# EricLBuehler/diffusion-rs

Hardware: AMD Instinct MI355X
Metric: images/sec, FLUX.1-dev 1024x1024 50-step (higher is better)
Workload: dtype bf16; 1 GPU; FLUX.1-dev bf16 1024x1024 50-step, batch=1 per GPU, S=4096 img + T=512 txt tokens, step = one image (50x Flux::forward + Euler, unpack, VAE decode, u8); global_batch=1, parallelism=single GPU

## Files before the change

### diffusion-rs_amd/_lib.py

```python
import ctypes as C
import os

_HERE = os.path.dirname(os.path.abspath(__file__))
LIB_PATH = os.environ.get("FMI_LIB") or os.path.join(_HERE, "libflux_mi355x.so")
ALT_LIB_PATH = os.path.join(_HERE, "libflux_mi355x_alt.so")


class FmiError(RuntimeError):

    def __init__(self, msg, code=None):
        super().__init__(msg)
        self.code = code


ERR_INVALID, ERR_HIP, ERR_STATE, ERR_UNSUPPORTED, ERR_NOMEM = -1, -2, -3, -4, -5


class FluxConfig(C.Structure):
    _fields_ = [("in_channels", C.c_int), ("pooled_projection_dim", C.c_int), ("joint_attention_dim", C.c_int),
                ("num_attention_heads", C.c_int), ("num_layers", C.c_int), ("num_single_layers", C.c_int),
                ("guidance_embeds", C.c_int), ("axes_dim", C.c_int * 3), ("theta", C.c_int)]


ALL_TO_ALL_FN = C.CFUNCTYPE(C.c_int, C.c_void_p, C.c_void_p, C.c_void_p, C.c_size_t, C.c_void_p)
# ... 13 lines not shown
    _fields_ = [("threshold", C.c_float), ("force", C.POINTER(C.c_int8)), ("decisions_out", C.POINTER(C.c_int32)), ("distances_out", C.POINTER(C.c_float))]


class FluxTrueCfg(C.Structure):
    _fields_ = [("neg_txt", C.c_void_p), ("neg_txt_dtype", C.c_int), ("neg_y", C.c_void_p), ("neg_y_dtype", C.c_int), ("scale", C.c_float)]


class FluxControl(C.Structure):
    _fields_ = [("cond", C.c_void_p), ("cond_dtype", C.c_int)]


class FluxControlNet(C.Structure):
    _fields_ = [("net", C.c_void_p), ("cond", C.c_void_p), ("cond_dtype", C.c_int), ("scale", C.c_float), ("step_scales", C.POINTER(C.c_float))]


class FluxIp(C.Structure):
    _fields_ = [("adapter", C.c_void_p), ("embeds", C.c_void_p), ("embeds_dtype", C.c_int), ("neg_embeds", C.c_void_p), ("scale", C.c_float),
                ("step_scales", C.POINTER(C.c_float))]


class FluxDenoiseOptions(C.Structure):
    _fields_ = [("ctx", C.POINTER(FluxContext)), ("ctl", C.POINTER(FluxControl)), ("cfg", C.POINTER(FluxTrueCfg)), ("cache", C.POINTER(FluxStepCache)),
                ("x0", C.c_void_p), ("noise", C.c_void_p), ("mask", C.c_void_p)]


class VaeConfig(C.Structure):
    _fields_ = [("in_channels", C.c_int), ("out_channels", C.c_int), ("block_out_channels", C.c_int * 4), ("n_blocks", C.c_int),
                ("layers_per_block", C.c_int), ("latent_channels", C.c_int), ("norm_num_groups", C.c_int),
                ("mid_block_add_attention", C.c_int), ("use_post_quant_conv", C.c_int), ("scaling_factor", C.c_double),
                ("shift_factor", C.c_double), ("use_quant_conv", C.c_int)]


class SchedulerConfigC(C.Structure):
    _fields_ = [("base_image_seq_len", C.c_int), ("base_shift", C.c_double), ("max_image_seq_len", C.c_int), ("max_shift", C.c_double),
                ("shift", C.c_double), ("use_dynamic_shifting", C.c_int)]


class T5Config(C.Structure):
    _fields_ = [("vocab_size", C.c_int), ("d_model", C.c_int), ("d_kv", C.c_int), ("d_ff", C.c_int), ("num_layers", C.c_int), ("num_heads", C.c_int),
                ("relative_attention_num_buckets", C.c_int), ("relative_attention_max_distance", C.c_int), ("layer_norm_epsilon", C.c_float),
                ("feed_forward_act", C.c_int)]


class ClipConfig(C.Structure):
    _fields_ = [("vocab_size", C.c_int), ("projection_dim", C.c_int), ("intermediate_size", C.c_int), ("max_position_embeddings", C.c_int),
                ("num_hidden_layers", C.c_int), ("num_attention_heads", C.c_int)]


class GemmDesc(C.Structure):
    _fields_ = [("a", C.c_void_p), ("w", C.c_void_p), ("bias", C.c_void_p), ("out", C.c_void_p), ("gate", C.c_void_p), ("resid", C.c_void_p),
                ("M", C.c_int), ("N", C.c_int), ("K", C.c_int), ("lda", C.c_int), ("ldw", C.c_int), ("ldo", C.c_int), ("epi", C.c_int),
                ("gelu_from", C.c_int), ("alpha", C.c_float), ("rows_per_batch", C.c_int), ("gate_bstride", C.c_int), ("q8", C.c_int),
                ("a_scale", C.c_void_p), ("w_scale", C.c_void_p), ("a_off", C.c_void_p), ("w_sum", C.c_void_p)]


GEMM_STORE_BF16, GEMM_GELU_BF16, GEMM_RESID_GATE_F32, GEMM_GELU_FROM_COL, GEMM_STORE_F32, GEMM_SCALE_BF16, GEMM_RESID_ADD_BF16, GEMM_SILU_BF16 = range(8)

F32, F16, BF16, U8, I8 = 0, 1, 2, 3, 4
MODEL_AUTO, MODEL_BF16, MODEL_F16, MODEL_F32 = 0, 1, 2, 3

_lib = None
_product = None
_alt = None


def load():
    global _lib, _product
    if _lib is not None:
        return _lib
    if not os.path.exists(LIB_PATH):
        raise FmiError(f"{LIB_PATH} not found — build it with `make lib` (hipcc --offload-arch=gfx950); there is no CPU fallback")
    try:
        import torch
    except Exception:
        pass
    _lib = _product = _declare(C.CDLL(LIB_PATH, mode=C.RTLD_GLOBAL))
    return _lib


def load_alt():
    global _alt
    if _alt is None:
        load()
        if not os.path.exists(ALT_LIB_PATH):
            raise FmiError(f"{ALT_LIB_PATH} not found — build it with `make alt`")
        _alt = _declare(C.CDLL(ALT_LIB_PATH, mode=C.RTLD_LOCAL))
        if not _alt.fmi_has_alt_kernels():
            raise FmiError(f"{ALT_LIB_PATH} was not compiled with -DFMI_ALT_KERNELS=1")
    return _alt


class use_alt:

    def __enter__(self):
        global _lib
        alt = load_alt()
        self.prev, _lib = _lib, alt
        return alt

    def __exit__(self, *exc):
        global _lib
        _lib = self.prev
        return False


def _declare(lib):
# ... 67 lines not shown
    lib.fmi_t5_forward.argtypes = [C.c_void_p, C.c_void_p, C.c_int, C.c_int, C.c_void_p, C.c_int, C.c_void_p]
    lib.fmi_clip_forward.argtypes = [C.c_void_p, C.c_void_p, C.c_int, C.c_int, C.c_void_p, C.c_int, C.c_void_p, C.c_void_p]
    lib.fmi_flux_forward_context.argtypes = [C.c_void_p, C.POINTER(FluxInputs), C.POINTER(FluxContext), C.c_void_p, C.c_void_p]
    head, loop, blend = [C.c_void_p, C.POINTER(FluxInputs)], [C.c_void_p, C.POINTER(C.c_double), C.c_int], [C.c_void_p] * 3
    lib.fmi_flux_denoise_with.argtypes = head + [C.POINTER(FluxDenoiseOptions)] + loop + [C.c_void_p]
    lib.fmi_flux_denoise.argtypes = head + loop + [C.c_void_p]
    lib.fmi_flux_denoise_inpaint.argtypes = head + loop + blend + [C.c_void_p]
    lib.fmi_flux_denoise_context.argtypes = head + [C.POINTER(FluxContext)] + loop + blend + [C.c_void_p]
    lib.fmi_flux_denoise_cached.argtypes = head + [C.POINTER(FluxContext)] + loop + blend + [C.POINTER(FluxStepCache), C.c_void_p]
    lib.fmi_flux_denoise_cfg.argtypes = head + [C.POINTER(FluxContext), C.POINTER(FluxTrueCfg)] + loop + blend + [C.c_void_p]
    lib.fmi_flux_denoise_control.argtypes = head + [C.POINTER(FluxControl), C.POINTER(FluxTrueCfg)] + loop + blend + [C.c_void_p]
    lib.fmi_cfg_euler_step.argtypes = [C.c_void_p, C.c_void_p, C.c_void_p, C.c_float, C.c_float, C.c_int64, C.c_void_p, C.c_void_p, C.c_void_p, C.c_float, C.c_void_p]
    lib.fmi_flux_create_cond.argtypes = [C.POINTER(FluxConfig), C.c_int, C.c_int, C.POINTER(C.c_void_p)]
    lib.fmi_flux_cond_channels.argtypes = [C.c_void_p]
    lib.fmi_flux_forward_control.argtypes = [C.c_void_p, C.POINTER(FluxInputs), C.POINTER(FluxControl), C.c_void_p, C.c_void_p]
    lib.fmi_flux_create_controlnet.argtypes = [C.POINTER(FluxConfig), C.c_int, C.POINTER(C.c_void_p)]
    lib.fmi_flux_is_controlnet.argtypes = [C.c_void_p]
    lib.fmi_flux_forward_controlnet.argtypes = [C.c_void_p, C.POINTER(FluxInputs), C.POINTER(FluxControlNet), C.c_void_p, C.c_void_p]
    lib.fmi_flux_denoise_controlnet.argtypes = head + [C.POINTER(FluxDenoiseOptions), C.POINTER(FluxControlNet)] + loop + [C.c_void_p]
    lib.fmi_flux_controlnet_eval.argtypes = [C.c_void_p, C.POINTER(FluxInputs), C.c_void_p, C.c_int, C.c_void_p]
    lib.fmi_flux_controlnet_sample.argtypes = [C.c_void_p, C.c_int, C.c_int, C.c_void_p]
    lib.fmi_add_scaled_rows_bf16.argtypes = [C.c_void_p, C.c_int64, C.c_void_p, C.c_int, C.c_int64, C.c_int, C.c_float, C.c_void_p]
    lib.fmi_ip_adapter_create.argtypes = [C.POINTER(FluxConfig), C.c_int, C.c_int, C.POINTER(C.c_void_p)]
    lib.fmi_ip_adapter_destroy.argtypes = [C.c_void_p]
    lib.fmi_ip_adapter_destroy.restype = None
    lib.fmi_ip_adapter_set_tensor.argtypes = [C.c_void_p, C.c_char_p, C.c_void_p, C.c_int, C.POINTER(C.c_int64), C.c_int]
    lib.fmi_ip_adapter_missing_count.argtypes = [C.c_void_p]
    lib.fmi_ip_adapter_missing_name.argtypes = [C.c_void_p, C.c_int]
    lib.fmi_ip_adapter_missing_name.restype = C.c_char_p
    lib.fmi_ip_adapter_size_in_bytes.argtypes = [C.c_void_p]
    lib.fmi_ip_adapter_size_in_bytes.restype = C.c_size_t
    lib.fmi_flux_forward_ip.argtypes = [C.c_void_p, C.POINTER(FluxInputs), C.POINTER(FluxControl), C.POINTER(FluxControlNet), C.POINTER(FluxIp), C.c_void_p, C.c_void_p]
    lib.fmi_flux_denoise_ip.argtypes = head + [C.POINTER(FluxDenoiseOptions), C.POINTER(FluxControlNet), C.POINTER(FluxIp)] + loop + [C.c_void_p]
    lib.fmi_ip_attention.argtypes = [C.c_void_p, C.c_int, C.c_int64, C.c_void_p, C.c_void_p, C.c_void_p, C.c_void_p, C.c_int64, C.c_int, C.c_int, C.c_int, C.c_int, C.c_float,
                                     C.c_int, C.c_void_p]
    lib.fmi_cast_cols_bf16.argtypes = [C.c_void_p, C.c_int, C.c_int64, C.c_int64, C.c_int, C.c_void_p, C.c_int, C.c_int, C.c_void_p]
    lib.fmi_mask_image.argtypes = [C.c_void_p, C.c_void_p, C.c_int, C.c_int, C.c_int, C.c_int, C.c_void_p, C.c_void_p]
    lib.fmi_fill_condition.argtypes = [C.c_void_p, C.c_void_p, C.c_int, C.c_int, C.c_int, C.c_void_p, C.c_void_p]
    lib.fmi_flux_step_cache_bytes.argtypes = [C.c_void_p]
    lib.fmi_flux_step_cache_bytes.restype = C.c_size_t
    lib.fmi_latent_ids.argtypes =[C.c_int, C.c_int, C.c_int, C.c_float, C.c_float, C.c_float, C.c_void_p, C.c_void_p]
    lib.fmi_preprocess_u8.argtypes = [C.c_void_p, C.c_int, C.c_int, C.c_int, C.c_int, C.c_int, C.c_void_p, C.c_void_p]
    lib.fmi_latent_mask.argtypes = [C.c_void_p, C.c_int, C.c_int, C.c_int, C.c_int, C.c_void_p, C.c_void_p]
    lib.fmi_encode_latents.argtypes = [C.c_void_p, C.c_int, C.c_int, C.c_int, C.c_int, C.c_double, C.c_double, C.c_void_p, C.c_void_p, C.c_void_p]
    lib.fmi_scale_noise.argtypes = [C.c_void_p, C.c_void_p, C.c_double, C.c_int64, C.c_void_p, C.c_void_p]
    lib.fmi_vae_decode.argtypes = [C.c_void_p, C.c_void_p, C.c_int, C.c_int, C.c_int, C.c_void_p, C.c_void_p]
    lib.fmi_vae_encode.argtypes = [C.c_void_p, C.c_void_p, C.c_int, C.c_int, C.c_int, C.c_void_p, C.c_void_p, C.c_void_p, C.c_void_p]
    lib.fmi_vae_mid_attention.argtypes = [C.c_void_p, C.c_void_p, C.c_int, C.c_int, C.c_int, C.c_void_p, C.c_void_p]
    lib.fmi_pack_latents.argtypes = [C.c_void_p, C.c_int, C.c_int, C.c_int, C.c_int, C.c_void_p, C.c_void_p, C.c_void_p]
    lib.fmi_postprocess_u8.argtypes = [C.c_void_p, C.c_int, C.c_int, C.c_int, C.c_int, C.c_int, C.c_void_p, C.c_void_p]
    lib.fmi_linear_bf16.argtypes = [C.c_void_p, C.c_void_p, C.c_void_p, C.c_void_p, C.c_int, C.c_int, C.c_int, C.c_int, C.c_void_p]
    lib.fmi_quantize_rows_fp8.argtypes = [C.c_void_p, C.c_int, C.c_int, C.c_void_p, C.c_void_p, C.c_void_p]
    lib.fmi_gemm_group.argtypes = [C.POINTER(GemmDesc), C.c_int, C.c_void_p]
    lib.fmi_splitk_resid_gate.argtypes = [C.c_void_p, C.c_int, C.c_void_p, C.c_void_p, C.c_int, C.c_int, C.c_void_p, C.c_int, C.c_int, C.c_int, C.c_void_p]
    lib.fmi_set_gemm_kernel.argtypes = [C.c_int, C.c_int]
    lib.fmi_linear_fp8.argtypes = [C.c_void_p, C.c_void_p, C.c_void_p, C.c_void_p, C.c_void_p, C.c_int, C.c_int, C.c_int, C.c_int, C.c_void_p]
    lib.fmi_quantize_rows_i8.argtypes = lib.fmi_quantize_rows_fp8.argtypes
    lib.fmi_linear_i8.argtypes = lib.fmi_linear_fp8.argtypes
    lib.fmi_gemm_q8.argtypes = [C.c_void_p] * 6 + [C.c_int] * 5 + [C.c_void_p]
    lib.fmi_quantize_rows_i8_asym.argtypes = [C.c_void_p, C.c_int, C.c_int, C.c_int, C.c_void_p, C.c_void_p, C.c_void_p, C.c_void_p]
    lib.fmi_rowsum_i8.argtypes = [C.c_void_p, C.c_void_p, C.c_int, C.c_int, C.c_int, C.c_void_p, C.c_void_p]
    lib.fmi_quantize_rows_i8_scaled.argtypes = [C.c_void_p, C.c_int, C.c_int, C.c_int, C.c_void_p, C.c_void_p, C.c_void_p, C.c_void_p, C.c_void_p]
    lib.fmi_col_absmax.argtypes = [C.c_void_p, C.c_int, C.c_int, C.c_int, C.c_void_p, C.c_void_p]
    lib.fmi_flux_calibrate_int8.argtypes = [C.c_void_p, C.c_int]
    lib.fmi_gemm_i8_asym.argtypes = [C.c_void_p] * 8 + [C.c_int] * 4 + [C.c_void_p]
    lib.fmi_flux_quantize_fp8.argtypes = [C.c_void_p, C.c_void_p]
    lib.fmi_flux_quantize_int8.argtypes = [C.c_void_p, C.c_uint, C.c_void_p]
    lib.fmi_flux_set_fp8_attention.argtypes = [C.c_void_p, C.c_int]
    lib.fmi_flux_set_modulation_gemm.argtypes = [C.c_void_p, C.c_int]
    lib.fmi_linear_bnb4_bf16.argtypes = [C.c_void_p, C.c_void_p, C.c_void_p, C.c_int, C.c_int, C.c_void_p, C.c_void_p, C.c_int, C.c_int, C.c_int,
                                         C.c_int, C.c_void_p]
    lib.fmi_linear_int8_bf16.argtypes = [C.c_void_p, C.c_void_p, C.c_void_p, C.c_void_p, C.c_void_p, C.c_int, C.c_int, C.c_int, C.c_int, C.c_void_p]
    lib.fmi_sdpa_bf16.argtypes = [C.c_void_p, C.c_void_p, C.c_void_p, C.c_void_p, C.c_int, C.c_int, C.c_int, C.c_int, C.c_int, C.c_float, C.c_int,
                                  C.c_void_p]
    lib.fmi_sdpa_fp8qk.argtypes = lib.fmi_sdpa_bf16.argtypes
    lib.fmi_sdpa_workspace_bytes.argtypes = [C.c_int, C.c_int, C.c_int]
    lib.fmi_sdpa_workspace_bytes.restype = C.c_size_t
    lib.fmi_sdpa_bf16_ws.argtypes = [C.c_void_p] * 4 + [C.c_int] * 5 + [C.c_float, C.c_int, C.c_void_p, C.c_size_t, C.c_void_p]
    lib.fmi_sdpa_fp8qk_ws.argtypes = [C.c_void_p] * 4 + [C.c_int] * 5 + [C.c_float, C.c_int, C.c_int, C.c_void_p, C.c_size_t, C.c_void_p]
    lib.fmi_sdpa_fp8.argtypes = [C.c_void_p] * 4 + [C.c_int] * 5 + [C.c_float, C.c_int, C.c_float, C.c_int, C.c_void_p]
    lib.fmi_sdpa_fp8_ws.argtypes = [C.c_void_p] * 4 + [C.c_int] * 5 + [C.c_float, C.c_int, C.c_float, C.c_int, C.c_void_p, C.c_size_t, C.c_void_p]
    lib.fmi_linear_q8_workspace_bytes.argtypes = [C.c_int, C.c_int]
    lib.fmi_linear_q8_workspace_bytes.restype = C.c_size_t
    lib.fmi_linear_fp8_ws.argtypes = list(lib.fmi_linear_fp8.argtypes[:-1]) + [C.c_void_p, C.c_size_t, C.c_void_p]
    lib.fmi_linear_i8_ws.argtypes = lib.fmi_linear_fp8_ws.argtypes
    lib.fmi_layernorm_mod.argtypes = [C.c_void_p, C.c_void_p, C.c_void_p, C.c_void_p, C.c_int, C.c_int, C.c_float, C.c_void_p]
    lib.fmi_groupnorm_nhwc.argtypes = [C.c_void_p, C.c_void_p, C.c_void_p, C.c_void_p, C.c_int, C.c_int, C.c_int, C.c_int, C.c_float, C.c_int,
                                       C.c_void_p]
    lib.fmi_conv2d_nhwc.argtypes = [C.c_void_p, C.c_void_p, C.c_void_p, C.c_void_p, C.c_void_p, C.c_int, C.c_int, C.c_int, C.c_int, C.c_int,
                                    C.c_int, C.c_int, C.c_void_p]
    for name in ("f32", "f16", "bf16"):
        for q in ("int8", "fp4", "nf4"):
            getattr(lib, f"dequantize_blockwise_{name}_{q}").argtypes = [C.c_void_p, C.c_void_p, C.c_void_p, C.c_void_p, C.c_int, C.c_int, C.c_void_p]
            getattr(lib, f"dequantize_blockwise_{name}_{q}").restype = None
        getattr(lib, f"dequantize_8bit_kernel_{name}").argtypes = [C.c_void_p, C.c_void_p, C.c_void_p, C.c_int, C.c_int, C.c_int]
        getattr(lib, f"dequantize_8bit_kernel_{name}").restype = None
    lib.fmi_event_create.argtypes = [C.POINTER(C.c_void_p)]
    lib.fmi_event_record.argtypes = [C.c_void_p, C.c_void_p]
    lib.fmi_event_elapsed_ms.argtypes = [C.c_void_p, C.c_void_p, C.POINTER(C.c_float)]
    lib.fmi_event_destroy.argtypes = [C.c_void_p]
    lib.fmi_stream_synchronize.argtypes = [C.c_void_p]
    return lib


SDPA_NO_EXP2 = 1 << 30


def tree_build_id(root=None):
    import glob
    import hashlib
    root = root or os.path.dirname(_HERE)
    files = sorted(glob.glob(os.path.join(root, "diffusion-rs_amd", "csrc", "*")) + glob.glob(os.path.join(root, "include", "*.h")) +
                   [os.path.join(root, "Makefile")], key=lambda p: os.path.relpath(p, root))
    h = hashlib.sha256()
    for f in files:
        with open(f, "rb") as fh:
            h.update(fh.read())
    return h.hexdigest()[:16]


def check(rc, lib=None):
    if rc != 0:
        raise FmiError(f"fmi status {rc}: {(lib or load()).fmi_last_error().decode(errors='replace')}", code=int(rc))


EXPORTED = [
    "fmi_last_error", "fmi_abi_version", "fmi_init", "fmi_device_info", "fmi_build_id", "fmi_has_alt_kernels", "fmi_flux_default_config", "fmi_flux_create", "fmi_flux_destroy",
    "fmi_flux_set_tensor", "fmi_flux_set_linear_bnb4", "fmi_flux_set_linear_int8", "fmi_flux_set_linear_gguf", "fmi_gguf_block_info", "fmi_gguf_dequantize", "fmi_flux_get_tensor", "fmi_flux_lora_add", "fmi_flux_lora_set_weight", "fmi_flux_lora_remove", "fmi_flux_lora_count", "fmi_flux_lora_name", "fmi_flux_set_quant_dense_cache", "fmi_flux_set_sequence_parallel", "fmi_flux_set_split_k", "fmi_set_bnb4_onewave_min_rows", "fmi_flux_set_attention_rescale_threshold", "fmi_flux_set_attention_kernel", "fmi_flux_state_buffer_count", "fmi_flux_state_export", "fmi_flux_state_adopt", "fmi_flux_state_buffer", "fmi_flux_set_modulation_gemm", "fmi_flux_quantize_fp8", "fmi_flux_quantize_int8", "fmi_flux_calibrate_int8", "fmi_flux_set_fp8_attention", "fmi_flux_missing_count", "fmi_flux_missing_name", "fmi_flux_size_in_bytes",
    "fmi_flux_forward", "fmi_flux_denoise", "fmi_flux_denoise_inpaint", "fmi_flux_forward_context", "fmi_flux_denoise_context", "fmi_flux_denoise_cached", "fmi_flux_step_cache_bytes", "fmi_flux_denoise_cfg", "fmi_flux_create_cond", "fmi_flux_cond_channels", "fmi_flux_forward_control", "fmi_flux_denoise_control", "fmi_flux_denoise_with",
    "fmi_flux_create_controlnet", "fmi_flux_is_controlnet", "fmi_flux_forward_controlnet", "fmi_flux_denoise_controlnet", "fmi_flux_controlnet_eval", "fmi_flux_controlnet_sample", "fmi_add_scaled_rows_bf16",
    "fmi_ip_adapter_create", "fmi_ip_adapter_destroy", "fmi_ip_adapter_set_tensor", "fmi_ip_adapter_missing_count", "fmi_ip_adapter_missing_name", "fmi_ip_adapter_size_in_bytes",
    "fmi_flux_forward_ip", "fmi_flux_denoise_ip", "fmi_ip_attention",
    "fmi_flux_set_profiling", "fmi_flux_set_fused_qkv_relayout", "fmi_flux_phase_count", "fmi_flux_phase_name", "fmi_flux_phase_ms",
    "fmi_vae_default_config", "fmi_vae_create", "fmi_vae_destroy", "fmi_vae_set_tensor", "fmi_vae_missing_count", "fmi_vae_missing_name",
    "fmi_vae_scale_factor", "fmi_vae_shift_factor", "fmi_vae_decode", "fmi_vae_encode", "fmi_vae_mid_attention",
    "fmi_t5_default_config", "fmi_t5_create", "fmi_t5_destroy", "fmi_t5_set_tensor", "fmi_t5_set_linear_bnb4", "fmi_t5_set_linear_int8", "fmi_t5_missing_count", "fmi_t5_missing_name",
    "fmi_t5_size_in_bytes", "fmi_t5_forward", "fmi_clip_default_config", "fmi_clip_create", "fmi_clip_destroy", "fmi_clip_set_tensor",
    "fmi_clip_missing_count", "fmi_clip_missing_name", "fmi_clip_size_in_bytes", "fmi_clip_forward", "fmi_pack_latents", "fmi_unpack_latents", "fmi_postprocess_u8",
    "fmi_preprocess_u8", "fmi_latent_mask", "fmi_encode_latents", "fmi_scale_noise", "fmi_latent_ids", "fmi_cfg_euler_step", "fmi_cast_cols_bf16", "fmi_mask_image", "fmi_fill_condition",
    "fmi_randn", "fmi_philox_u32", "fmi_calculate_shift", "fmi_get_timesteps", "fmi_linear_bf16", "fmi_linear_bnb4_bf16", "fmi_linear_int8_bf16", "fmi_quantize_rows_fp8", "fmi_linear_fp8", "fmi_quantize_rows_i8", "fmi_linear_i8", "fmi_gemm_q8", "fmi_quantize_rows_i8_asym", "fmi_rowsum_i8", "fmi_quantize_rows_i8_scaled", "fmi_col_absmax", "fmi_gemm_i8_asym", "fmi_gemm_group", "fmi_splitk_resid_gate", "fmi_set_gemm_kernel", "fmi_linear_q8_workspace_bytes", "fmi_linear_fp8_ws", "fmi_linear_i8_ws", "fmi_sdpa_bf16", "fmi_sdpa_fp8qk", "fmi_sdpa_workspace_bytes", "fmi_sdpa_bf16_ws", "fmi_sdpa_fp8qk_ws", "fmi_sdpa_fp8", "fmi_sdpa_fp8_ws", "fmi_set_attention_kernel", "fmi_layernorm_mod",
    "fmi_release_scratch", "fmi_timestep_embedding", "fmi_rope_table", "fmi_rmsnorm_rope",
    "fmi_groupnorm_nhwc", "fmi_conv2d_nhwc",
    "fmi_comm_probe", "fmi_comm_unique_id", "fmi_comm_create", "fmi_comm_destroy", "fmi_comm_rank", "fmi_comm_world_size", "fmi_comm_stats", "fmi_comm_all_to_all",
    "fmi_comm_broadcast", "fmi_comm_gather",
    "dequantize_blockwise_f32_int8", "dequantize_blockwise_f32_fp4", "dequantize_blockwise_f32_nf4", "dequantize_blockwise_f16_int8",
    "dequantize_blockwise_f16_fp4", "dequantize_blockwise_f16_nf4", "dequantize_blockwise_bf16_int8", "dequantize_blockwise_bf16_fp4",
    "dequantize_blockwise_bf16_nf4", "dequantize_8bit_kernel_f32", "dequantize_8bit_kernel_f16", "dequantize_8bit_kernel_bf16",
    "fmi_malloc", "fmi_free", "fmi_memcpy", "fmi_memset", "fmi_stream_synchronize", "fmi_event_create", "fmi_event_record",
    "fmi_event_elapsed_ms", "fmi_event_destroy",
]
```

### diffusion-rs_amd/csrc/capi.hip

```cpp
#include <algorithm>
#include <cmath>
#include <cstring>
#include <map>
#include <mutex>
#include <set>
#include <thread>
#include <tuple>
#include <utility>
#include <vector>

#include "common.h"

namespace fmi {
static thread_local std::string g_err;
void set_error(const std::string& msg) { g_err = msg; }
int fail(fmi_status st, const std::string& msg) {
  g_err = msg;
  return (int)st;
}
}
using namespace fmi;

extern "C" const char* fmi_last_error(void) { return g_err.c_str(); }
extern "C" int fmi_abi_version(void) { return FMI_ABI_VERSION; }
// ... 276 lines not shown
  const size_t bytes = fmi_linear_q8_workspace_bytes(M, K);
  FMI_TRY(ws.get(bytes));
  return linear_q8_ws(x, wq, w_scale, bias, y, M, N, K, epi, ws.p, bytes, stream, kind);
}
extern "C" int fmi_gemm_q8(const void* xq, const float* x_scale, const void* wq, const float* w_scale, const void* bias, void* y, int M, int N, int K,
                           int kind, fmi_epilogue epi, void* stream) {
  if (!xq || !x_scale || !wq || !w_scale || !y) return fail(FMI_ERR_INVALID, "gemm_q8: null pointer");
  if (kind != 1 && kind != 2) return fail(FMI_ERR_INVALID, "gemm_q8: kind must be 1 (e4m3) or 2 (int8)");
  if (M == 0 || N == 0) return FMI_OK;
  if (N % 4 || N <= 128) return fail(FMI_ERR_INVALID, "gemm_q8: N must be a multiple of 4 and > 128");
  GemmProblem p{};
  p.A = (const bf16_t*)xq, p.W = (const bf16_t*)wq, p.bias = (const bf16_t*)bias, p.out = y;
  p.M = M, p.N = N, p.K = K, p.lda = K, p.ldw = K, p.ldo = N, p.epi = epi_of(epi), p.alpha = 1.f;
  p.fp8 = kind, p.a_scale = x_scale, p.w_scale = w_scale;
  return launch_gemm(&p, 1, (hipStream_t)stream);
}

extern "C" int fmi_quantize_rows_i8_asym(const void* x, int rows, int K, int d0, int8_t* out, float* scale, float* offset, void* stream) {
  if (rows == 0) return FMI_OK;
  if (!x || !out || !scale || !offset) return fail(FMI_ERR_INVALID, "quantize_rows_i8_asym: null pointer");
  return launch_quantize_rows_i8_asym((const bf16_t*)x, K, rows, K, d0, reinterpret_cast<uint8_t*>(out), scale, offset, (hipStream_t)stream);
}
extern "C" int fmi_quantize_rows_i8_scaled(const void* x, int rows, int K, int d0, const float* col_scale, int8_t* out, float* scale, float* offset, void* stream) {
  if (rows == 0) return FMI_OK;
  if (!x || !out || !scale || !col_scale) return fail(FMI_ERR_INVALID, "quantize_rows_i8_scaled: null pointer");
  if (d0 < 0) return launch_quantize_rows_fp8((const bf16_t*)x, K, rows, K, reinterpret_cast<uint8_t*>(out), scale, (hipStream_t)stream, 2, col_scale);
  if (!offset) return fail(FMI_ERR_INVALID, "quantize_rows_i8_scaled: the offset form (d0 >= 0) needs `offset`");
  return launch_quantize_rows_i8_asym((const bf16_t*)x, K, rows, K, d0, reinterpret_cast<uint8_t*>(out), scale, offset, (hipStream_t)stream, col_scale);
}
extern "C" int fmi_col_absmax(const void* x, int rows, int K, int ld, float* amax_inout, void* stream) {
  if (rows == 0) return FMI_OK;
  if (!x || !amax_inout) return fail(FMI_ERR_INVALID, "col_absmax: null pointer");
  if (ld < K) return fail(FMI_ERR_INVALID, "col_absmax: ld must be >= K");
  return launch_col_absmax((const bf16_t*)x, ld, rows, K, amax_inout, (hipStream_t)stream);
}
extern "C" int fmi_rowsum_i8(const int8_t* wq, const float* w_scale, int N, int K, int d0, float* w_sum, void* stream) {
  if (N == 0) return FMI_OK;
  if (!wq || !w_scale || !w_sum) return fail(FMI_ERR_INVALID, "rowsum_i8: null pointer");
  if (reinterpret_cast<uintptr_t>(wq) & 15) return fail(FMI_ERR_INVALID, "rowsum_i8: wq must be 16-byte aligned");
  return launch_rowsum_i8(wq, w_scale, N, K, d0, w_sum, (hipStream_t)stream);
}
extern "C" int fmi_gemm_i8_asym(const void* xq, const float* x_scale, const float* x_offset, const void* wq, const float* w_scale, const float* w_sum,
                                const void* bias, void* y, int M, int N, int K, fmi_epilogue epi, void* stream) {
  if (!xq || !x_scale || !x_offset || !wq || !w_scale || !w_sum || !y) return fail(FMI_ERR_INVALID, "gemm_i8_asym: null pointer");
  if (M == 0 || N == 0) return FMI_OK;
  if (N % 4 || N <= 128) return fail(FMI_ERR_INVALID, "gemm_i8_asym: N must be a multiple of 4 and > 128");
  GemmProblem p{};
  p.A = (const bf16_t*)xq, p.W = (const bf16_t*)wq, p.bias = (const bf16_t*)bias, p.out = y;
  p.M = M, p.N = N, p.K = K, p.lda = K, p.ldw = K, p.ldo = N, p.epi = epi_of(epi), p.alpha = 1.f;
  p.fp8 = 2, p.a_scale = x_scale, p.w_scale = w_scale, p.a_off = x_offset, p.w_sum = w_sum;
  return launch_gemm(&p, 1, (hipStream_t)stream);
}

extern "C" int fmi_gemm_group(const fmi_gemm_desc* probs, int nprob, void* stream) {
  if (nprob <= 0) return FMI_OK;
  if (!probs) return fail(FMI_ERR_INVALID, "gemm_group: null descriptor array");
  if (nprob > 8) return fail(FMI_ERR_INVALID, "gemm_group: too many grouped problems (at most 8), got " + std::to_string(nprob));
  auto misaligned = [](const void* p, uintptr_t a) { return (reinterpret_cast<uintptr_t>(p) & (a - 1)) != 0; };
  GemmProblem gp[8];
  for (int i = 0; i < nprob; ++i) {
    const fmi_gemm_desc& d = probs[i];
    const std::string who = "gemm_group: problem " + std::to_string(i) + ": ";
    if (!d.a || !d.w || !d.out) return fail(FMI_ERR_INVALID, who + "null a / w / out");
    if (d.epi < EPI_STORE_BF16 || d.epi > EPI_SILU_BF16) return fail(FMI_ERR_INVALID, who + "epi must be 0 .. 7");
    if (d.q8 < 0 || d.q8 > 2) return fail(FMI_ERR_INVALID, who + "q8 must be 0, 1 or 2");
    if (d.M <= 0 || d.N <= 0 || d.K <= 0) return fail(FMI_ERR_INVALID, who + "empty problem");
    if (d.lda < d.K || d.ldw < d.K || d.ldo < d.N || d.gate_bstride < 0) return fail(FMI_ERR_INVALID, who + "lda / ldw must be >= K, ldo >= N and gate_bstride >= 0");
    if (misaligned(d.a, 16) || misaligned(d.w, 16)) return fail(FMI_ERR_INVALID, who + "a and w must be 16-byte aligned");
    const bool f32_out = d.epi == EPI_RESID_GATE_F32 || d.epi == EPI_STORE_F32;
    if (misaligned(d.out, f32_out ? 4 : 2) || misaligned(d.bias, 2) || misaligned(d.resid, 2) || misaligned(d.gate, 4) || misaligned(d.a_scale, 4) ||
        misaligned(d.w_scale, 4) || misaligned(d.a_off, 4) || misaligned(d.w_sum, 4))
      return fail(FMI_ERR_INVALID, who + "a pointer is not aligned to its element type");
    if (d.epi != EPI_STORE_F32 && d.epi != EPI_SCALE_BF16 && d.alpha != 1.0f)
      return fail(FMI_ERR_INVALID, who + "alpha belongs to STORE_F32 / SCALE_BF16 and must be 1 elsewhere");
    GemmProblem& p = gp[i];
    p = GemmProblem{};
    p.A = (const bf16_t*)d.a, p.W = (const bf16_t*)d.w, p.bias = (const bf16_t*)d.bias, p.out = d.out, p.gate = d.gate, p.resid = d.resid;
    p.M = d.M, p.N = d.N, p.K = d.K, p.lda = d.lda, p.ldw = d.ldw, p.ldo = d.ldo;
    p.epi = d.epi, p.gelu_from = d.gelu_from, p.alpha = d.alpha, p.rows_per_batch = d.rows_per_batch, p.gate_bstride = d.gate_bstride;
    p.fp8 = d.q8, p.a_scale = d.a_scale, p.w_scale = d.w_scale, p.a_off = d.a_off, p.w_sum = d.w_sum;
  }
  return launch_gemm(gp, nprob, (hipStream_t)stream);
}
extern "C" int fmi_splitk_resid_gate(const float* parts, int S, const void* bias, const float* gate, int rows_per_batch, int gate_bstride, float* out, int ldo,
                                     int M, int N, void* stream) {
  if (M == 0 || N == 0) return FMI_OK;
  if (!parts || !out) return fail(FMI_ERR_INVALID, "splitk_resid_gate: null pointer");
  if (S < 1 || M < 0 || N < 0 || ldo < N) return fail(FMI_ERR_INVALID, "splitk_resid_gate: S >= 1, M, N >= 0 and ldo >= N required");
  if ((reinterpret_cast<uintptr_t>(parts) | reinterpret_cast<uintptr_t>(out)) & 15) return fail(FMI_ERR_INVALID, "splitk_resid_gate: parts and out must be 16-byte aligned");
  if ((reinterpret_cast<uintptr_t>(gate) & 3) || (reinterpret_cast<uintptr_t>(bias) & 1)) return fail(FMI_ERR_INVALID, "splitk_resid_gate: gate / bias not aligned to their element type");
  return launch_splitk_resid_gate(parts, S, (const bf16_t*)bias, gate, rows_per_batch, gate_bstride, out, ldo, M, N, (hipStream_t)stream);
}
extern "C" int fmi_set_gemm_kernel(int pingpong, int w4) {
  set_gemm_pingpong(pingpong != 0);
  set_gemm_w4(w4 != 0);
  return FMI_OK;
}

extern "C" int fmi_linear_fp8(const void* x, const uint8_t* wq, const float* w_scale, const void* bias, void* y, int M, int N, int K,
                              fmi_epilogue epi, void* stream) {
  return linear_q8(x, wq, w_scale, bias, y, M, N, K, epi, stream, 1);
}
extern "C" int fmi_linear_i8(const void* x, const int8_t* wq, const float* w_scale, const void* bias, void* y, int M, int N, int K,
                             fmi_epilogue epi, void* stream) {
  return linear_q8(x, reinterpret_cast<const uint8_t*>(wq), w_scale, bias, y, M, N, K, epi, stream, 2);
}

extern "C" int fmi_linear_fp8_ws(const void* x, const uint8_t* wq, const float* w_scale, const void* bias, void* y, int M, int N, int K,
                                 fmi_epilogue epi, void* workspace, size_t workspace_bytes, void* stream) {
  return linear_q8_ws(x, wq, w_scale, bias, y, M, N, K, epi, workspace, workspace_bytes, stream, 1);
}
extern "C" int fmi_linear_i8_ws(const void* x, const int8_t* wq, const float* w_scale, const void* bias, void* y, int M, int N, int K,
                                fmi_epilogue epi, void* workspace, size_t workspace_bytes, void* stream) {
  return linear_q8_ws(x, reinterpret_cast<const uint8_t*>(wq), w_scale, bias, y, M, N, K, epi, workspace, workspace_bytes, stream, 2);
}

extern "C" size_t fmi_sdpa_workspace_bytes(int B, int H, int Lk) {
  if (B <= 0 || H <= 0 || Lk <= 0) return 0;
  return (size_t)B * H * 128 * ((size_t)(Lk + 63) / 64 * 64) * 2;
}
static int sdpa_ws(const void* q, const void* k, const void* v, void* o, int B, int H, int Lq, int Lk, int d, float scale, int score_exp2,
                   int out_token_major, void* workspace, size_t workspace_bytes, void* stream, int qk_fp8) {
  if (!q || !k || !v || !o) return fail(FMI_ERR_INVALID, "sdpa: null pointer");
  if (d != 128) return fail(FMI_ERR_UNSUPPORTED, "sdpa: head dim must be 128");
  if (B <= 0 || H <= 0 || Lq <= 0 || Lk <= 0) return fail(FMI_ERR_INVALID, "sdpa: empty problem");
  if (!workspace || workspace_bytes < fmi_sdpa_workspace_bytes(B, H, Lk))
    return fail(FMI_ERR_INVALID, "sdpa: workspace smaller than fmi_sdpa_workspace_bytes(B, H, Lk)");
  if (reinterpret_cast<uintptr_t>(workspace) & 15) return fail(FMI_ERR_INVALID, "sdpa: workspace must be 16-byte aligned");
  hipStream_t s = (hipStream_t)stream;
  const int Lpad = (Lk + 63) / 64 * 64;
  bf16_t* vt = static_cast<bf16_t*>(workspace);
  FMI_TRY(launch_v_transpose((const bf16_t*)v, 128, (int64_t)Lk * 128, vt, B * H, 1, Lk, 0, Lpad, s));
  FMI_TRY(launch_vt_zero_pad(vt, B * H, Lk, Lpad, s));
  AttnOut ao{};
// ... 105 lines not shown
```

### diffusion-rs_amd/csrc/common.h

```cpp
#pragma once
#ifndef FMI_ALT_KERNELS
#define FMI_ALT_KERNELS 0
#endif
#include <type_traits>
#include <hip/hip_runtime.h>
#include <stdint.h>

#include <set>
#include <string>
#include <vector>

#include "../../include/flux_mi355x.h"

namespace fmi {

void set_error(const std::string& msg);
int fail(fmi_status st, const std::string& msg);
#define FMI_HIP_TRY(expr)                                                                       \
  do {                                                                                          \
    hipError_t _e = (expr);                                                                     \
    if (_e != hipSuccess)                                                                       \
      return ::fmi::fail(FMI_ERR_HIP, std::string(#expr) + ": " + hipGetErrorString(_e) + " @" + \
                                          __FILE__ + ":" + std::to_string(__LINE__));           \
  } while (0)
// ... 195 lines not shown

constexpr int NUM_XCD = 8;
__device__ __forceinline__ int xcd_remap(int bid, int nwg) {
  int xcd = bid % NUM_XCD, idx = bid / NUM_XCD;
  int q = nwg / NUM_XCD, r = nwg % NUM_XCD;
  int base = xcd < r ? xcd * (q + 1) : r * (q + 1) + (xcd - r) * q;
  return base + idx;
}

inline int cdiv(int a, int b) { return (a + b - 1) / b; }
inline int64_t cdiv64(int64_t a, int64_t b) { return (a + b - 1) / b; }

enum GemmEpi : int {
  EPI_STORE_BF16 = 0,
  EPI_GELU_BF16 = 1,
  EPI_RESID_GATE_F32 = 2,
  EPI_GELU_FROM_COL = 3,
  EPI_STORE_F32 = 4,
  EPI_SCALE_BF16 = 5,
  EPI_RESID_ADD_BF16 = 6,
  EPI_SILU_BF16 = 7
};
struct GemmProblem {
  const bf16_t* A;
  const bf16_t* W;
  const bf16_t* bias;
  void* out;
  const float* gate;
  const void* resid;
  int M, N, K;
  int lda, ldw, ldo;
  int epi;
  int gelu_from;
  float alpha;
  int rows_per_batch;
  int gate_bstride;
  const uint8_t* Wq;
  const float* absmax;
  int q_blocksize;
  int q_type;
  int cv_ks, cv_h, cv_w, cv_cin, cv_up;
  const bf16_t* cv_zero;
  bf16_t *qk_qh, *qk_kh, *qk_vt;
  const bf16_t *qk_wq, *qk_wk;
  const float* qk_pe;
  int64_t qk_pe_bstride;
  int qk_H, qk_D, qk_rows, qk_row_off, qk_Ltot, qk_Lpad;
  float qk_q8, qk_k8;
  int fp8;
  const float* a_scale;
  const float* w_scale;
  const float* a_off;
  const float* w_sum;
};
int launch_gemm(const GemmProblem* probs, int nprob, hipStream_t stream);
void set_gemm_w4(bool on);
void set_gemm_pingpong(bool on);
void set_gemm_w4q_min_rows(int rows);
void set_gemm_w4_qkv_min_n(int n);

struct AttnOut {
  bf16_t* p0;
  int rows0;
  int ld0;
  int64_t bstride0;
  bf16_t* p1;
  int ld1;
  int64_t bstride1;
  int head_major;
};
constexpr int ATT_NO_EXP2 = 1 << 30;
int launch_attention_ex(const bf16_t* q, const bf16_t* k, const bf16_t* vt, const AttnOut& out, int B, int H, int Lq, int Lk,
                        int Lkpad, float scale, int rescale_thr_x16, hipStream_t stream, int qk_fp8 = 0, float* lse = nullptr, int nsplit = 0,
                        int score_exp2 = ATT_NO_EXP2, int kind = -1, float v_inv = 1.f);
unsigned long long attention_fp8_fallbacks();
struct OpScratch {
  explicit OpScratch(hipStream_t stream);
  ~OpScratch();
  OpScratch(const OpScratch&) = delete;
  OpScratch& operator=(const OpScratch&) = delete;
  int get(size_t bytes);
  void* p = nullptr;

 private:
  hipStream_t s_;
  bool locked_ = false;
};
bool alt_kernels_built();
enum AttnKind {
  SINGLE_BARRIER = 0,
  PINGPONG = 1,
  W4 = 2,
  W16 = 3,
  W32 = 4,
  W16L = 5,
};
void set_attention_kind(int kind);
int launch_attention(const bf16_t* q, const bf16_t* k, const bf16_t* vt, bf16_t* out, int B, int H,
                     int Lq, int Lk, int Lkpad, float scale, int out_token_major, hipStream_t stream);
int launch_v_transpose(const bf16_t* v, int ldv, int64_t v_bstride, bf16_t* vt, int B, int H, int rows,
                       int row_off, int Lpad, hipStream_t stream);
int launch_vt_zero_pad(bf16_t* vt, int BH, int L, int Lpad, hipStream_t stream);
int launch_v_transpose_fp8(const bf16_t* v, uint8_t* vt8, int BH, int Lk, int Lpad, float v_scale, hipStream_t stream);
size_t sp_qkv_bytes_per_peer(int Hr, int Ll);
size_t sp_o_bytes_per_peer(int Hr, int Ll);
int launch_sp_pack_qkv(const bf16_t* q, const bf16_t* k, const bf16_t* vt, void* send, int H, int Tl, int Sl, int N, hipStream_t s);
int launch_sp_unpack_qkv(const void* recv, bf16_t* qf, bf16_t* kf, bf16_t* vtf, int H, int Tl, int Sl, int N, hipStream_t s);
int launch_sp_pack_o(const bf16_t* o, void* send, int H, int Tl, int Sl, int N, hipStream_t s);
int launch_sp_unpack_o(const void* recv, const AttnOut& out, int H, int Ll, int N, hipStream_t s);
int launch_sp_merge_splits(const bf16_t* parts, const float* lse, int S, bf16_t* out, int heads, int L, hipStream_t s);
int launch_qk_norm_rope(const bf16_t* q, const bf16_t* k, int ld, int64_t in_bstride, const bf16_t* wq,
                        const bf16_t* wk, const float* pe, int64_t pe_bstride, bf16_t* qo, bf16_t* ko,
                        int B, int H, int rows, int row_off, int Ltot, hipStream_t stream);
int launch_qk_norm_rope_f32(const bf16_t* q, const bf16_t* k, int ld, int64_t in_bstride, const bf16_t* wq, const bf16_t* wk, const float* pe,
                            int64_t pe_bstride, float* qo, float* ko, int B, int H, int rows, int row_off, int Ltot, hipStream_t stream);
int launch_rope_table(const float* txt_ids, const float* img_ids, int B, int T, int S, const int* axes,
                      int theta, float* pe, hipStream_t stream, const float* ctx_ids = nullptr, int R = 0);
int launch_layernorm_mod2(const float* x, const float* scale, const float* shift, int mod_bstride, int rows_per_batch, bf16_t* out, int rows,
                          const float* x2, const float* scale2, const float* shift2, int rows_per_batch2, bf16_t* out2, int rows2, int D, float eps,
                          hipStream_t stream);
int launch_layernorm_mod_fp8_2(const float* x, const float* scale, const float* shift, int mod_bstride, int rows_per_batch, uint8_t* out,
                               float* out_scale, int rows, const float* x2, const float* scale2, const float* shift2, int rows_per_batch2, uint8_t* out2,
                               float* out_scale2, int rows2, int D, float eps, hipStream_t stream, int kind = 1, const float* smooth = nullptr,
                               const float* smooth2 = nullptr);
int launch_layernorm_mod(const float* x, const float* scale, const float* shift, int mod_bstride,
                         int rows_per_batch, bf16_t* out, int rows, int D, float eps, hipStream_t stream);
int launch_quantize_rows_fp8(const bf16_t* x, int ld, int rows, int K, uint8_t* out, float* scale, hipStream_t stream, int kind = 1, const float* vec = nullptr);
int launch_quantize_rows_i8_asym(const bf16_t* x, int ld, int rows, int K, int d0, uint8_t* out, float* scale, float* offset, hipStream_t stream, const float* vec = nullptr);
int launch_rowsum_i8(const int8_t* wq, const float* w_scale, int N, int K, int d0, float* w_sum, hipStream_t stream);
int launch_layernorm_mod_fp8(const float* x, const float* scale, const float* shift, int mod_bstride, int rows_per_batch,
                             uint8_t* out, float* out_scale, int rows, int D, float eps, hipStream_t stream, int kind = 1, const float* smooth = nullptr);
int launch_col_absmax(const bf16_t* x, int ld, int rows, int K, float* amax, hipStream_t stream);
void smooth_factors_host(const float* act_amax, const float* w_amax, int K, float* s_out, float* inv_out);
int launch_gemv(const float* x, const bf16_t* W, const bf16_t* bias, float* y, int M, int N, int K,
                int silu_in, int accumulate, hipStream_t stream);
int launch_dequant_int8_scb_bf16(const int8_t* w, const float* scb, bf16_t* out, int col, int64_t n, hipStream_t stream);
constexpr int LORA_TILE_ROWS = 64, LORA_RANK_CHUNK = 16;
int launch_lora_pack(const float* A, const float* B, int rows, int K, int r, double coef, float* Acat, double* Bt, int rows_pad, int off, hipStream_t stream);
int launch_lora_merge(const bf16_t* w0, bf16_t* w, int rows, int K, const float* A, const double* Bt, int rows_pad, int Rpad, hipStream_t stream);
int launch_timestep_embedding(const float* t, int B, int dim, float* out, hipStream_t stream);
int launch_cast_to_bf16(const void* src, fmi_dtype dt, bf16_t* dst, int64_t n, hipStream_t stream);
int launch_cast_to_f32(const void* src, fmi_dtype dt, float* dst, int64_t n, hipStream_t stream);
int launch_cast_rows_bf16(const void* src, fmi_dtype dt, int64_t src_bs, bf16_t* dst, int64_t dst_bs, int B, int64_t n, hipStream_t stream, int B_src = 0);
int launch_cast_cols_bf16(const void* src, fmi_dtype dt, int64_t rows, int64_t rows_src, int cols, bf16_t* dst, int dst_ld, int col0, hipStream_t stream);
int launch_add_scaled_rows_bf16(float* x, int64_t x_bs, const bf16_t* src, int B, int64_t rows, int D, float c, hipStream_t stream);
int launch_add_scaled_rows_f32(float* x, int64_t x_bs, const float* src, int B, int64_t rows, int D, float c, hipStream_t stream);
int launch_silu_to_bf16(const float* src, bf16_t* dst, int64_t n, hipStream_t stream);
int launch_euler_update(float* img, const float* pred, float dt, int64_t n, hipStream_t stream);
int launch_euler_blend(float* img, const float* pred, const float* x0, const float* noise, const float* mask, float dt, float s, int64_t n, hipStream_t stream);
int launch_euler_cfg(float* img, const float* pos, const float* neg, float scale, float dt, int64_t n, hipStream_t stream, const float* x0 = nullptr,
                     const float* noise = nullptr, const float* mask = nullptr, float s = 0.f);
int launch_scale_noise(const float* x0, const float* noise, float t, int64_t n, float* out, hipStream_t stream);
int launch_add2_rows(float* y, const float* g, const float* v, int R, int B, int N, hipStream_t stream);
int launch_splitk_resid_gate(const float* parts, int S, const bf16_t* bias, const float* gate, int rows_per_batch, int gate_bstride, float* out, int ldo,
                             int M, int N, hipStream_t stream);
int launch_split_rows_f32(const float* src, float* dst, int B, int rows_src_per_b, int row_off, int rows, int D, hipStream_t stream);
int step_cache_groups(int64_t n);
int launch_step_cache_residual(const float* x1, int64_t x1_bs, float* x0, const float* r_ref, float* r, float* part, double* sums, int B, int64_t n, hipStream_t stream);
int launch_step_cache_delta(const float* xf, int64_t xf_bs, const float* x1copy, float* delta, int B, int64_t n, hipStream_t stream);
int launch_step_cache_apply(const float* x1, int64_t x1_bs, const float* delta, float* xf, int64_t xf_bs, int B, int64_t n, hipStream_t stream);

}
```

### diffusion-rs_amd/csrc/flux_model.hip

```cpp
#include <algorithm>
#include <cstring>
#include <map>
#include <set>
#include <cmath>
#include <cstring>
#include <vector>

#include <dlfcn.h>

#include "common.h"
#include "ip_adapter.h"

using namespace fmi;

namespace {

enum ArenaId { AR_BASE = 0, AR_MOD, AR_BLOCKS, AR_Q4, AR_COUNT };
struct Arena {
  DeviceBuffer base;
  size_t bytes = 0;
};
enum PartState : uint8_t { PS_UNSET = 0, PS_FP4 = 1, PS_NF4 = 2, PS_INT8 = 3, PS_GGUF0 = 16, PS_GGUF_END = 48, PS_DENSE = 100 };
inline bool is_gguf(int state) { return state >= PS_GGUF0 && state < PS_GGUF_END; }

// ... 25 lines not shown
};

struct Dest {
  Dense* d;
  int part;
  bool bias;
  void* ptr;
  int64_t numel;
  int rows, cols;
};

enum Phase { PH_EMBED = 0, PH_MOD, PH_LN, PH_GEMM_QKV, PH_RELAYOUT, PH_ATTN, PH_GEMM_PROJ, PH_GEMM_MLP, PH_FINAL, PH_COUNT };
const char* kPhaseNames[PH_COUNT] = {"embed", "modulation", "layernorm_mod", "gemm_qkv", "qk_norm_rope_vT", "attention",
                                     "gemm_proj", "gemm_mlp", "final_layer"};

}

struct fmi_flux {
  fmi_flux_config cfg;
  int cond = 0;
  int D, M, H;
  int device = 0;
  Arena arena[AR_COUNT];
  size_t cursor[AR_COUNT] = {0, 0, 0, 0};
  std::vector<Dense*> fused;
  bool finalized = false;
  Dense img_in, txt_in, time1, time2, guid1, guid2, vecin1, vecin2, final_proj;
  Dense mod_all;
  struct DoubleW {
    Dense qkv[2], proj[2], mlp1[2], mlp2[2];
    bf16_t* nq[2];
    bf16_t* nk[2];
    int64_t mod_off[2];
  };
  struct SingleW {
    Dense w1, w2;
    bf16_t* nq;
    bf16_t* nk;
    int64_t mod_off;
  };
  std::vector<DoubleW> dbl;
  std::vector<SingleW> sgl;
  int64_t mod_final_off = 0, n_mod = 0;
  std::map<std::string, Dest> names;
  MissingSet missing;
  struct WS {
    int B = 0, S = 0, T = 0;
    DeviceBuffer base;
    float *x_img, *x_txt, *x_txt0, *x, *vec, *mod, *temb, *h1, *yf, *pe, *img_f32, *pred_tmp, *tv;
    bf16_t *img_bf, *txt_bf, *xm, *qkv_img, *qkv_txt, *big, *Qh, *Kh, *Vt, *attn_img, *attn_txt, *hid, *vec_bf;
    uint8_t* a8 = nullptr;
    float* a8s = nullptr;
    float* a8o = nullptr;
    int Lpad = 0;
  } ws;
  bool profiling = false;
  hipStream_t side = nullptr;
  hipEvent_t ev_fork = nullptr, ev_join = nullptr;
  bool two_streams = false;
  hipEvent_t ev0 = nullptr, ev1 = nullptr;
  float phase_ms[PH_COUNT] = {0};
  int attn_thr = 96;
  int attn_kind = -1;
  DeviceBuffer mod_steps, vec_steps, temb_steps, h1_steps;
  DeviceBuffer vec_steps_bf;
  size_t mod_steps_rows = 0;
  int mod_gemm = 1;
  DeviceBuffer sc_x0, sc_r[2], sc_delta, sc_part, sc_sums;
  DeviceBuffer cfg_gd;
  size_t sc_elems = 0, sc_part_floats = 0;
  double* sc_host = nullptr;
  bool fuse_qkv_relayout = true;
  bool dense_cache = false;
  int quant_mode = -1;
  bool quant_auto = true;
  std::set<const void*> dense_ready;
  DeviceBuffer wscratch[2];
  int sp_rank = 0, sp_world = 1;
  fmi_all_to_all_fn sp_a2a = nullptr;
  void* sp_user = nullptr;
  DeviceBuffer sp_base;
  int sp_Tl = 0, sp_Sl = 0, sp_Nw = 0;
  void *sp_send = nullptr, *sp_recv = nullptr;
  bf16_t *sp_Qf = nullptr, *sp_Kf = nullptr, *sp_Vtf = nullptr, *sp_O = nullptr;
  float* sp_lse = nullptr;
  static constexpr int SP_SPLITS = 4;
  bool split_k = false;
  DeviceBuffer splitk_scratch;
  bool fp8 = false;
  int q8_kind = 0;
  unsigned q8_mask = 0;
  DeviceBuffer fp8_arena;
  bool calib = false;
  int calib_evals = 0;
  DeviceBuffer calib_arena;
  float* calib_wmax = nullptr;
  int fp8_attn = 1;
  std::vector<float> q8_dbl, k8_dbl, q8_sgl, k8_sgl;
  bool attn_scales_valid = false;
  std::vector<int> n8_dbl, n8_sgl;
  struct LoraPair {
    DeviceBuffer A;
    DeviceBuffer B;
    int r = 0;
    float scale = 1.f;
  };
  struct LoraAdapter {
    float weight = 1.f;
    std::map<std::string, LoraPair> pairs;
  };
  std::map<std::string, LoraAdapter> loras;
  std::map<std::string, DeviceBuffer> lora_backup;
  DeviceBuffer lora_scratch;
  std::vector<DeviceBuffer> lora_dead;
  bool is_cn = false;
  Dense cn_x;
  std::vector<Dense> cn_dbl, cn_sgl;
  DeviceBuffer cn_samples;
  DeviceBuffer cn_cx;
  DeviceBuffer cn_cond_bf;
  size_t cn_elems = 0;
  int cn_B = 0, cn_S = 0;
};

static int compute_attention_scales(fmi_flux* m);
static void lora_release_storage(fmi_flux* m);

namespace {

size_t align_up(size_t v, size_t a) { return (v + a - 1) / a * a; }

size_t arena_take(fmi_flux* m, int ar, size_t bytes) {
  const size_t off = align_up(m->cursor[ar], 256);
  m->cursor[ar] = off + bytes;
  return off;
}
int ensure_arena(fmi_flux* m, int ar) {
  Arena& a = m->arena[ar];
  if (a.base || a.bytes == 0) return FMI_OK;
  hipError_t e = a.base.alloc(a.bytes);
  if (e != hipSuccess) return fail(FMI_ERR_NOMEM, "flux: hipMalloc of " + std::to_string(a.bytes) + " bytes (weight arena " + std::to_string(ar) + ") failed: " + hipGetErrorString(e));
// ... 220 lines not shown
  m->dense_ready.clear();
  m->finalized = true;
  return FMI_OK;
}

constexpr int PE_ROW_FLOATS = 128;
int ensure_workspace(fmi_flux* m, int B, int S, int T) {
  auto& w = m->ws;
  if (w.base && w.B == B && w.S == S && w.T == T) return FMI_OK;
  const int D = m->D, M = m->M, H = m->H, L = S + T;
  const int Lpad = (L + 63) / 64 * 64;
  const int C = m->cfg.in_channels, J = m->cfg.joint_attention_dim, P = m->cfg.pooled_projection_dim;
  const int ldbig = 3 * D + M;
  size_t off = 0;
  auto take = [&](size_t bytes) {
    off = align_up(off, 256);
    size_t o = off;
    off += bytes;
    return o;
  };
  struct Item {
    void** p;
    size_t bytes;
    size_t o;
  };
  std::vector<Item> items;
  auto add = [&](void** p, size_t bytes) { items.push_back({p, bytes, take(bytes)}); };
  add((void**)&w.x_img, (size_t)B * S * D * 4);
  add((void**)&w.x_txt, (size_t)B * T * D * 4);
  add((void**)&w.x_txt0, (size_t)B * T * D * 4);
  add((void**)&w.x, (size_t)B * L * D * 4);
  add((void**)&w.vec, (size_t)B * D * 4);
  add((void**)&w.mod, (size_t)B * m->n_mod * 4);
  add((void**)&w.temb, (size_t)B * 256 * 4);
  add((void**)&w.h1, (size_t)B * D * 4);
  add((void**)&w.yf, (size_t)B * P * 4);
  add((void**)&w.pe, (size_t)B * L * PE_ROW_FLOATS * 4);
  add((void**)&w.img_f32, (size_t)B * S * C * 4);
  add((void**)&w.pred_tmp, (size_t)B * S * C * 4);
  add((void**)&w.tv, 4096 * 4);
  add((void**)&w.img_bf, (size_t)B * S * (C + m->cond) * 2);
  add((void**)&w.txt_bf, (size_t)B * T * J * 2);
  add((void**)&w.xm, (size_t)B * L * D * 2);
  add((void**)&w.qkv_img, (size_t)B * S * 3 * D * 2);
  add((void**)&w.qkv_txt, (size_t)B * T * 3 * D * 2);
  add((void**)&w.big, (size_t)B * L * ldbig * 2);
  add((void**)&w.Qh, (size_t)B * H * L * 128 * 2);
  add((void**)&w.Kh, (size_t)B * H * L * 128 * 2);
  add((void**)&w.Vt, (size_t)B * H * 128 * Lpad * 2);
  add((void**)&w.attn_img, (size_t)B * S * D * 2);
  add((void**)&w.attn_txt, (size_t)B * T * D * 2);
  add((void**)&w.hid, (size_t)B * L * M * 2);
  add((void**)&w.vec_bf, (size_t)B * D * 2);
  if (m->fp8) {
    add((void**)&w.a8, (size_t)B * L * (D + M));
    add((void**)&w.a8s, (size_t)B * L * 4);
    add((void**)&w.a8o, (size_t)B * L * 4);
  }
  const size_t total = align_up(off, 256);
  if (w.base) FMI_HIP_TRY(hipDeviceSynchronize());
  FMI_HIP_TRY(w.base.alloc(total));
  FMI_HIP_TRY(hipMemset(w.base.ptr, 0, total));
  for (auto& it : items) *it.p = w.base.as<char>() + it.o;
  if (B == 1) {
    w.x_txt = w.x;
    w.x_img = w.x + (size_t)T * D;
  }
  w.B = B, w.S = S, w.T = T, w.Lpad = Lpad;
  return FMI_OK;
}

GemmProblem make_problem_fp8(const fmi_flux* m, const Dense& d, int row0, int Mrows, void* out, int ldo, int epi) {
  GemmProblem p{};
  p.A = reinterpret_cast<const bf16_t*>(m->ws.a8 + (size_t)row0 * d.K);
  p.W = reinterpret_cast<const bf16_t*>(d.w8);
  p.bias = d.b;
  p.out = out;
  p.M = Mrows, p.N = d.N, p.K = d.K;
  p.lda = d.K, p.ldw = d.K, p.ldo = ldo;
  p.epi = epi;
  p.alpha = 1.0f;
  p.fp8 = m->q8_kind;
  p.a_scale = m->ws.a8s + row0;
  p.w_scale = d.w8_scale;
  if (d.w8_d0 >= 0) p.a_off = m->ws.a8o + row0, p.w_sum = d.w8_sum;
  return p;
}
int quantize_act(fmi_flux* m, const Dense& d, const bf16_t* x, int ld, int rows, int row0, hipStream_t s) {
  uint8_t* out = m->ws.a8 + (size_t)row0 * d.K;
  if (d.w8_d0 >= 0) return launch_quantize_rows_i8_asym(x, ld, rows, d.K, d.w8_d0, out, m->ws.a8s + row0, m->ws.a8o + row0, s, d.sm_inv);
  return launch_quantize_rows_fp8(x, ld, rows, d.K, out, m->ws.a8s + row0, s, m->q8_kind, d.sm_inv);
}
int calib_rec(fmi_flux* m, const Dense& d, const bf16_t* x, int ld, int rows, hipStream_t s) {
  if (!m->calib || !d.sm_amax) return FMI_OK;
  return launch_col_absmax(x, ld, rows, d.K, d.sm_amax, s);
}
GemmProblem make_problem(const Dense& d, const bf16_t* A, int lda, int Mrows, void* out, int ldo, int epi) {
  GemmProblem p{};
  p.A = A;
  p.W = d.w;
  p.bias = d.b;
  p.out = out;
  p.M = Mrows;
  p.N = d.N;
  p.K = d.K;
  p.lda = lda;
// ... 325 lines not shown
}

int compute_vec_steps(fmi_flux* m, const fmi_flux_inputs* in, const float* tv_dev, int n_steps, float* vec_steps, float* temb_steps, float* h1_steps, hipStream_t s) {
  auto& w = m->ws;
  const fmi_flux_config& c = m->cfg;
  const int B = in->B, D = m->D, R = n_steps * B;
  FMI_TRY(launch_timestep_embedding(tv_dev, R, 256, temb_steps, s));
  FMI_TRY(launch_gemv(temb_steps, m->time1.w, m->time1.b, h1_steps, R, D, 256, 0, 0, s));
  FMI_TRY(launch_gemv(h1_steps, m->time2.w, m->time2.b, vec_steps, R, D, D, 1, 0, s));
  float* gterm = nullptr;
  if (c.guidance_embeds) {
    if (!in->guidance) return fail(FMI_ERR_INVALID, "flux: guidance_embeds model needs a guidance vector");
    gterm = h1_steps;
    FMI_TRY(launch_timestep_embedding(in->guidance, B, 256, w.temb, s));
    FMI_TRY(launch_gemv(w.temb, m->guid1.w, m->guid1.b, w.h1, B, D, 256, 0, 0, s));
    FMI_TRY(launch_gemv(w.h1, m->guid2.w, m->guid2.b, gterm, B, D, D, 1, 0, s));
  }
  float* vterm = h1_steps + (size_t)B * D;
  FMI_TRY(launch_gemv(w.yf, m->vecin1.w, m->vecin1.b, w.h1, B, D, c.pooled_projection_dim, 0, 0, s));
  FMI_TRY(launch_gemv(w.h1, m->vecin2.w, m->vecin2.b, vterm, B, D, D, 1, 0, s));
  return launch_add2_rows(vec_steps, gterm, vterm, R, B, D, s);
}

struct StepCacheRun {
  const fmi_flux_step_cache* o;
  int step = 0;
  bool valid = false;
  int ref = 0;
};

int step_cache_decide(fmi_flux* m, StepCacheRun* sc, int B, int S, int T, hipStream_t s, bool* reuse) {
  auto& w = m->ws;
  const int64_t n = (int64_t)S * m->D, L = S + T;
  PhaseTimer pt(m, s, PH_EMBED);
  const int i = sc->step;
  float* const r_ref = m->sc_r[sc->ref].as<float>();
  FMI_TRY(launch_step_cache_residual(w.x_img, n, m->sc_x0.as<float>(), sc->valid ? r_ref : nullptr, m->sc_r[sc->ref ^ 1].as<float>(), m->sc_part.as<float>(),
                                     m->sc_sums.as<double>(), B, n, s));
  bool below = true;
  if (sc->valid) {
    FMI_HIP_TRY(hipMemcpyAsync(m->sc_host, m->sc_sums.ptr, (size_t)2 * B * sizeof(double), hipMemcpyDeviceToHost, s));
    FMI_HIP_TRY(hipStreamSynchronize(s));
  }
  for (int b = 0; b < B; ++b) {
    float d = -1.f;
    if (sc->valid) d = m->sc_host[2 * b + 1] == 0.0 ? INFINITY : (float)(m->sc_host[2 * b] / m->sc_host[2 * b + 1]);
    if (sc->o->distances_out) sc->o->distances_out[(size_t)i * B + b] = d;
    below = below && d < sc->o->threshold;
  }
  const int f = sc->o->force ? sc->o->force[i] : -1;
  *reuse = sc->valid && (f == 1 || (f < 0 && sc->o->threshold > 0.f && below));
  if (sc->o->decisions_out) sc->o->decisions_out[i] = *reuse ? 1 : 0;
  if (*reuse) FMI_TRY(launch_step_cache_apply(w.x_img, n, m->sc_delta.as<float>(), w.x + (size_t)T * m->D, L * m->D, B, n, s));
  return FMI_OK;
}

int forward_core(fmi_flux* m, const fmi_flux_inputs* in, const EvalPlan& p, const float* img_f32, const float* timesteps_dev, float* pred, const float* mod_pre,
                 const float* txt_pre, StepCacheRun* sc, const CnInject* inj, const IpInject* ipj, hipStream_t s) {
  auto& w = m->ws;
  const fmi_flux_config& c = m->cfg;
  const int B = in->B, Bs = p.Bs, R = p.R, Ss = in->S, S = Ss + R, T = in->T, L = S + T;
  const int D = m->D, Mh = m->M, H = m->H, C = c.in_channels;
  const int nmod = (int)m->n_mod;
  const int64_t pe_bs = in->ids_per_sample ? (int64_t)L * PE_ROW_FLOATS : 0;
  const float att_scale = 1.0f / sqrtf(128.0f);
  const bool fp8 = m->fp8;
  const int qk = m->q8_kind;
  const bool sp = m->sp_world > 1 && m->sp_a2a;
  if (sp && (B != 1 || fp8)) return fail(FMI_ERR_UNSUPPORTED, "flux: sequence parallelism runs one image (B = 1) in bf16 mode");
  if (m->calib) {
    if (sp || fp8) return fail(FMI_ERR_STATE, "flux: int8 calibration runs on one device in bf16 mode");
    ++m->calib_evals;
  }
  if (m->fp8_attn == 2 && !sp && !m->attn_scales_valid) FMI_TRY(compute_attention_scales(m));
  const bool qk8_any = m->fp8_attn == 2 && !sp;
  const int BT = B * T;
  const auto cn_hook = [&](bool single, int i, float* rows, int64_t bs) -> int {
    if (m->is_cn) {
      PhaseTimer pt(m, s, PH_EMBED);
      FMI_TRY(launch_cast_rows_bf16(rows, FMI_F32, bs, w.xm, (int64_t)S * D, B, (int64_t)S * D, s));
      Dense& zl = single ? m->cn_sgl[i] : m->cn_dbl[i];
      GemmProblem q = make_problem(zl, w.xm, D, B * S, m->cn_samples.as<bf16_t>() + ((single ? m->cn_dbl.size() : 0) + i) * m->cn_elems, D, EPI_STORE_BF16);
      return gemm1(m, q, zl, s);
    }
    if (!inj) return FMI_OK;
    const int n_net = (int)(single ? inj->net->cn_sgl.size() : inj->net->cn_dbl.size()), n_main = single ? c.num_single_layers : c.num_layers;
    if (!n_net) return FMI_OK;
    const int k = i / ((n_main + n_net - 1) / n_net);
    PhaseTimer pt(m, s, PH_EMBED);
    return launch_add_scaled_rows_bf16(rows, bs, inj->net->cn_samples.as<bf16_t>() + ((single ? inj->net->cn_dbl.size() : 0) + k) * inj->net->cn_elems, B, S, D, inj->c, s);
  };
  const auto ip_hook = [&](int i) -> int {
    if (!ipj) return FMI_OK;
    PhaseTimer pt(m, s, PH_ATTN);
    return launch_ip_attention(w.qkv_img, 3 * D, (int64_t)S * 3 * D, m->dbl[i].nq[0], ipj->a->k_of(i), ipj->a->v_of(i), w.x_img, (int64_t)S * D, B, H, S, ipj->a->N, ipj->c,
                               0, s);
  };
  {
    PhaseTimer pt(m, s, PH_EMBED);
    if (m->cond)
      FMI_TRY(launch_cast_cols_bf16(img_f32, FMI_F32, (int64_t)B * S, (int64_t)Bs * S, C, w.img_bf, m->img_in.K, 0, s));
    else if (R || Bs != B) FMI_TRY(launch_cast_rows_bf16(img_f32, FMI_F32, (int64_t)Ss * C, w.img_bf, (int64_t)S * C, B, (int64_t)Ss * C, s, Bs));
    else FMI_TRY(launch_cast_to_bf16(img_f32, FMI_F32, w.img_bf, (int64_t)B * S * C, s));
    if (!mod_pre) FMI_TRY(compute_vec(m, in, timesteps_dev, w.vec, s));
    GemmProblem p[2];
    p[0] = make_problem(m->img_in, w.img_bf, m->img_in.K, B * S, w.x_img, D, EPI_STORE_F32);
    p[1] = make_problem(m->txt_in, w.txt_bf, c.joint_attention_dim, B * T, w.x_txt, D, EPI_STORE_F32);
    Dense* dn[2] = {&m->img_in, &m->txt_in};
    if (txt_pre) {
      FMI_HIP_TRY(hipMemcpyAsync(w.x_txt, txt_pre, (size_t)B * T * D * 4, hipMemcpyDeviceToDevice, s));
      FMI_TRY(gemm1(m, p[0], m->img_in, s));
    } else {
      FMI_TRY(gemm2(m, p, dn, 2, s));
    }
    if (m->is_cn)
      FMI_TRY(launch_add_scaled_rows_f32(w.x_img, (int64_t)S * D, m->cn_cx.as<float>(), B, S, D, 1.0f, s));
    if (sc) FMI_HIP_TRY(hipMemcpyAsync(m->sc_x0.ptr, w.x_img, (size_t)B * S * D * 4, hipMemcpyDeviceToDevice, s));
  }
  if (!mod_pre) {
    PhaseTimer pt(m, s, PH_MOD);
    if (m->mod_all.q_type) {
      FMI_TRY(launch_silu_to_bf16(w.vec, w.vec_bf, (int64_t)B * D, s));
      GemmProblem p = make_problem(m->mod_all, w.vec_bf, D, B, w.mod, nmod, EPI_STORE_F32);
      FMI_TRY(gemm1(m, p, m->mod_all, s));
    } else {
      FMI_TRY(launch_gemv(w.vec, m->mod_all.w, m->mod_all.b, w.mod, B, nmod, D, 1, 0, s));
    }
  }
  const float* const mod = mod_pre ? mod_pre : w.mod;

  bool reuse = false;
  for (int i = 0; i < c.num_layers; ++i) {
    if (sc && i == 1) {
      FMI_TRY(step_cache_decide(m, sc, B, S, T, s, &reuse));
      if (reuse) break;
    }
    auto& bw = m->dbl[i];
    const float* mi = mod + bw.mod_off[0];
    const float* mt = mod + bw.mod_off[1];
    bf16_t* xm_txt = w.xm;
    bf16_t* xm_img = w.xm + (size_t)B * T * D;
    bool fused_img = false, fused_txt = false, qk8 = false;
    const bool q_qkv = fp8 && bw.qkv[0].w8, q_out = fp8 && bw.proj[0].w8, q_m1 = fp8 && bw.mlp1[0].w8, q_m2 = fp8 && bw.mlp2[0].w8;
    {
      PhaseTimer pt(m, s, PH_LN);
      if (q_qkv) {
        FMI_TRY(launch_layernorm_mod_fp8_2(w.x_img, mi + D, mi, nmod, S, w.a8 + (size_t)BT * D, w.a8s + BT, B * S, w.x_txt, mt + D, mt, T, w.a8, w.a8s,
                                           B * T, D, 1e-6f, s, qk, bw.qkv[0].sm_inv, bw.qkv[1].sm_inv));
      } else {
        FMI_TRY(launch_layernorm_mod2(w.x_img, mi + D, mi, nmod, S, xm_img, B * S, w.x_txt, mt + D, mt, T, xm_txt, B * T, D, 1e-6f, s));
        FMI_TRY(calib_rec(m, bw.qkv[0], xm_img, D, B * S, s));
        FMI_TRY(calib_rec(m, bw.qkv[1], xm_txt, D, B * T, s));
      }
    }
    {
      PhaseTimer pt(m, s, PH_GEMM_QKV);
      GemmProblem p[2];
      p[0] = q_qkv ? make_problem_fp8(m, bw.qkv[0], BT, B * S, w.qkv_img, 3 * D, EPI_STORE_BF16)
                   : make_problem(bw.qkv[0], xm_img, D, B * S, w.qkv_img, 3 * D, EPI_STORE_BF16);
      p[1] = q_qkv ? make_problem_fp8(m, bw.qkv[1], 0, B * T, w.qkv_txt, 3 * D, EPI_STORE_BF16)
                   : make_problem(bw.qkv[1], xm_txt, D, B * T, w.qkv_txt, 3 * D, EPI_STORE_BF16);
      qk8 = ((q_qkv && m->fp8_attn) || (qk8_any && !bw.qkv[0].q_type && !bw.qkv[1].q_type)) && can_fuse_relayout(m, B * S, S, T) && can_fuse_relayout(m, B * T, T, 0);
      const float q8 = qk8 ? m->q8_dbl[i] : 0.f, k8 = qk8 ? m->k8_dbl[i] : 0.f;
      fused_img = !ipj && with_qkv_relayout(m, p[0], bw.nq[0], bw.nk[0], pe_bs, S, T, L, q8, k8);
      fused_txt = with_qkv_relayout(m, p[1], bw.nq[1], bw.nk[1], pe_bs, T, 0, L, q8, k8);
      Dense* dn[2] = {&bw.qkv[0], &bw.qkv[1]};
      FMI_TRY(gemm2(m, p, dn, 2, s));
    }
    if (!(fused_img && fused_txt)) {
      PhaseTimer pt(m, s, PH_RELAYOUT);
      if (!fused_txt) {
        FMI_TRY(launch_qk_norm_rope(w.qkv_txt, w.qkv_txt + D, 3 * D, (int64_t)T * 3 * D, bw.nq[1], bw.nk[1], w.pe, pe_bs, w.Qh, w.Kh, B, H, T, 0, L, s));
        FMI_TRY(launch_v_transpose(w.qkv_txt + 2 * D, 3 * D, (int64_t)T * 3 * D, w.Vt, B, H, T, 0, w.Lpad, s));
      }
      if (!fused_img) {
        FMI_TRY(launch_qk_norm_rope(w.qkv_img, w.qkv_img + D, 3 * D, (int64_t)S * 3 * D, bw.nq[0], bw.nk[0], w.pe, pe_bs, w.Qh, w.Kh, B, H, S, T, L, s));
        FMI_TRY(launch_v_transpose(w.qkv_img + 2 * D, 3 * D, (int64_t)S * 3 * D, w.Vt, B, H, S, T, w.Lpad, s));
      }
    }
    {
      PhaseTimer pt(m, s, PH_ATTN);
      AttnOut o{};
      o.p0 = w.attn_txt, o.rows0 = T, o.ld0 = D, o.bstride0 = (int64_t)T * D;
      o.p1 = w.attn_img, o.ld1 = D, o.bstride1 = (int64_t)S * D;
      const float sc = qk8 ? att_scale / (m->q8_dbl[i] * m->k8_dbl[i]) : att_scale;
      if (sp) FMI_TRY(attention_sp(m, o, T, S, sc, s));
      else FMI_TRY(launch_attention_ex(w.Qh, w.Kh, w.Vt, o, B, H, L, L, w.Lpad, sc, m->attn_thr, s, qk8 ? 1 : 0, nullptr, 0, qk8 ? -m->n8_dbl[i] : ATT_NO_EXP2, m->attn_kind));
    }
    if (m->two_streams && !fp8 && !sp && !m->profiling && !m->calib && !bw.proj[0].q_type && !bw.proj[1].q_type && !bw.mlp1[0].q_type && !bw.mlp1[1].q_type &&
        !bw.mlp2[0].q_type && !bw.mlp2[1].q_type && !m->split_k) {
      bf16_t* hid_txt = w.hid;
      bf16_t* hid_img = w.hid + (size_t)B * T * Mh;
      FMI_HIP_TRY(hipEventRecord(m->ev_fork, s));
      FMI_HIP_TRY(hipStreamWaitEvent(m->side, m->ev_fork, 0));
      for (int st = 0; st < 2; ++st) {
        hipStream_t q = st ? m->side : s;
        const int rows = st ? B * T : B * S, rpb = st ? T : S;
        const float* mo = st ? mt : mi;
        float* x = st ? w.x_txt : w.x_img;
        bf16_t* xm_ = st ? xm_txt : xm_img;
        bf16_t* hid_ = st ? hid_txt : hid_img;
        GemmProblem p = make_problem(bw.proj[st], st ? w.attn_txt : w.attn_img, D, rows, x, D, EPI_RESID_GATE_F32);
        with_gate(p, mo + 2 * D, rpb, nmod);
        FMI_TRY(gemm1(m, p, bw.proj[st], q));
        FMI_TRY(launch_layernorm_mod(x, mo + 4 * D, mo + 3 * D, nmod, rpb, xm_, rows, D, 1e-6f, q));
        p = make_problem(bw.mlp1[st], xm_, D, rows, hid_, Mh, EPI_GELU_BF16);
        FMI_TRY(gemm1(m, p, bw.mlp1[st], q));
        p = make_problem(bw.mlp2[st], hid_, Mh, rows, x, D, EPI_RESID_GATE_F32);
        with_gate(p, mo + 5 * D, rpb, nmod);
        FMI_TRY(gemm1(m, p, bw.mlp2[st], q));
      }
      FMI_HIP_TRY(hipEventRecord(m->ev_join, m->side));
      FMI_HIP_TRY(hipStreamWaitEvent(s, m->ev_join, 0));
      FMI_TRY(ip_hook(i));
      FMI_TRY(cn_hook(false, i, w.x_img, (int64_t)S * D));
      continue;
    }
    {
      PhaseTimer pt(m, s, PH_GEMM_PROJ);
      GemmProblem p[2];
      if (q_out) {
        FMI_TRY(quantize_act(m, bw.proj[0], w.attn_img, D, B * S, BT, s));
        FMI_TRY(quantize_act(m, bw.proj[1], w.attn_txt, D, B * T, 0, s));
      } else {
        FMI_TRY(calib_rec(m, bw.proj[0], w.attn_img, D, B * S, s));
        FMI_TRY(calib_rec(m, bw.proj[1], w.attn_txt, D, B * T, s));
      }
      p[0] = q_out ? make_problem_fp8(m, bw.proj[0], BT, B * S, w.x_img, D, EPI_RESID_GATE_F32)
                   : make_problem(bw.proj[0], w.attn_img, D, B * S, w.x_img, D, EPI_RESID_GATE_F32);
      with_gate(p[0], mi + 2 * D, S, nmod);
      p[1] = q_out ? make_problem_fp8(m, bw.proj[1], 0, B * T, w.x_txt, D, EPI_RESID_GATE_F32)
                   : make_problem(bw.proj[1], w.attn_txt, D, B * T, w.x_txt, D, EPI_RESID_GATE_F32);
      with_gate(p[1], mt + 2 * D, T, nmod);
      Dense* dn[2] = {&bw.proj[0], &bw.proj[1]};
      FMI_TRY(gemm2(m, p, dn, 2, s));
    }
    {
      PhaseTimer pt(m, s, PH_LN);
      if (q_m1) {
        FMI_TRY(launch_layernorm_mod_fp8_2(w.x_img, mi + 4 * D, mi + 3 * D, nmod, S, w.a8 + (size_t)BT * D, w.a8s + BT, B * S, w.x_txt, mt + 4 * D,
                                           mt + 3 * D, T, w.a8, w.a8s, B * T, D, 1e-6f, s, qk, bw.mlp1[0].sm_inv, bw.mlp1[1].sm_inv));
      } else {
        FMI_TRY(launch_layernorm_mod2(w.x_img, mi + 4 * D, mi + 3 * D, nmod, S, xm_img, B * S, w.x_txt, mt + 4 * D, mt + 3 * D, T, xm_txt, B * T, D,
                                      1e-6f, s));
        FMI_TRY(calib_rec(m, bw.mlp1[0], xm_img, D, B * S, s));
        FMI_TRY(calib_rec(m, bw.mlp1[1], xm_txt, D, B * T, s));
      }
    }
    {
      PhaseTimer pt(m, s, PH_GEMM_MLP);
      bf16_t* hid_txt = w.hid;
      bf16_t* hid_img = w.hid + (size_t)B * T * Mh;
      GemmProblem p[2];
      p[0] = q_m1 ? make_problem_fp8(m, bw.mlp1[0], BT, B * S, hid_img, Mh, EPI_GELU_BF16) : make_problem(bw.mlp1[0], xm_img, D, B * S, hid_img, Mh, EPI_GELU_BF16);
      p[1] = q_m1 ? make_problem_fp8(m, bw.mlp1[1], 0, B * T, hid_txt, Mh, EPI_GELU_BF16) : make_problem(bw.mlp1[1], xm_txt, D, B * T, hid_txt, Mh, EPI_GELU_BF16);
      Dense* dn1[2] = {&bw.mlp1[0], &bw.mlp1[1]};
      FMI_TRY(gemm2(m, p, dn1, 2, s));
      if (q_m2) {
        if (bw.mlp2[0].sm_inv || bw.mlp2[1].sm_inv) {
          FMI_TRY(quantize_act(m, bw.mlp2[1], hid_txt, Mh, B * T, 0, s));
          FMI_TRY(quantize_act(m, bw.mlp2[0], hid_img, Mh, B * S, BT, s));
        } else {
          FMI_TRY(quantize_act(m, bw.mlp2[0], w.hid, Mh, B * L, 0, s));
        }
      } else {
        FMI_TRY(calib_rec(m, bw.mlp2[0], hid_img, Mh, B * S, s));
        FMI_TRY(calib_rec(m, bw.mlp2[1], hid_txt, Mh, B * T, s));
      }
      p[0] = q_m2 ? make_problem_fp8(m, bw.mlp2[0], BT, B * S, w.x_img, D, EPI_RESID_GATE_F32)
                  : make_problem(bw.mlp2[0], hid_img, Mh, B * S, w.x_img, D, EPI_RESID_GATE_F32);
      with_gate(p[0], mi + 5 * D, S, nmod);
      p[1] = q_m2 ? make_problem_fp8(m, bw.mlp2[1], 0, B * T, w.x_txt, D, EPI_RESID_GATE_F32)
                  : make_problem(bw.mlp2[1], hid_txt, Mh, B * T, w.x_txt, D, EPI_RESID_GATE_F32);
      with_gate(p[1], mt + 5 * D, T, nmod);
      Dense* dn2[2] = {&bw.mlp2[0], &bw.mlp2[1]};
      FMI_TRY(gemm2(m, p, dn2, 2, s));
    }
    FMI_TRY(ip_hook(i));
    FMI_TRY(cn_hook(false, i, w.x_img, (int64_t)S * D));
  }

  if (sc && c.num_layers == 1) FMI_TRY(step_cache_decide(m, sc, B, S, T, s, &reuse));
  for (int b = 0; b < B && w.x_txt != w.x && !reuse; ++b) {
    FMI_HIP_TRY(hipMemcpyAsync(w.x + (size_t)b * L * D, w.x_txt + (size_t)b * T * D, (size_t)T * D * 4, hipMemcpyDeviceToDevice, s));
    FMI_HIP_TRY(hipMemcpyAsync(w.x + ((size_t)b * L + T) * D, w.x_img + (size_t)b * S * D, (size_t)S * D * 4, hipMemcpyDeviceToDevice, s));
  }
  const int ldbig = 3 * D + Mh;
  for (int i = 0; i < (reuse ? 0 : c.num_single_layers); ++i) {
    auto& bw = m->sgl[i];
    const float* mo = mod + bw.mod_off;
    bool fused = false;
    const bool q_w1 = fp8 && bw.w1.w8, q_w2 = fp8 && bw.w2.w8;
    const bool qk8 = ((q_w1 && m->fp8_attn) || (qk8_any && !bw.w1.q_type)) && can_fuse_relayout(m, B * L, L, 0);
    {
      PhaseTimer pt(m, s, PH_LN);
      if (q_w1) {
        FMI_TRY(launch_layernorm_mod_fp8(w.x, mo + D, mo, nmod, L, w.a8, w.a8s, B * L, D, 1e-6f, s, qk, bw.w1.sm_inv));
      } else {
        FMI_TRY(launch_layernorm_mod(w.x, mo + D, mo, nmod, L, w.xm, B * L, D, 1e-6f, s));
        FMI_TRY(calib_rec(m, bw.w1, w.xm, D, B * L, s));
      }
    }
    {
      PhaseTimer pt(m, s, PH_GEMM_QKV);
      GemmProblem p = q_w1 ? make_problem_fp8(m, bw.w1, 0, B * L, w.big, ldbig, EPI_GELU_FROM_COL)
                           : make_problem(bw.w1, w.xm, D, B * L, w.big, ldbig, EPI_GELU_FROM_COL);
      p.gelu_from = 3 * D;
      fused = with_qkv_relayout(m, p, bw.nq, bw.nk, pe_bs, L, 0, L, qk8 ? m->q8_sgl[i] : 0.f, qk8 ? m->k8_sgl[i] : 0.f);
      FMI_TRY(gemm1(m, p, bw.w1, s));
    }
    if (!fused) {
      PhaseTimer pt(m, s, PH_RELAYOUT);
      FMI_TRY(launch_qk_norm_rope(w.big, w.big + D, ldbig, (int64_t)L * ldbig, bw.nq, bw.nk, w.pe, pe_bs, w.Qh, w.Kh, B, H, L, 0, L, s));
      FMI_TRY(launch_v_transpose(w.big + 2 * D, ldbig, (int64_t)L * ldbig, w.Vt, B, H, L, 0, w.Lpad, s));
    }
    {
      PhaseTimer pt(m, s, PH_ATTN);
      AttnOut o{};
      o.p0 = nullptr, o.rows0 = 0;
      o.p1 = w.big + 2 * D, o.ld1 = ldbig, o.bstride1 = (int64_t)L * ldbig;
      const float sc = qk8 ? att_scale / (m->q8_sgl[i] * m->k8_sgl[i]) : att_scale;
      if (sp) FMI_TRY(attention_sp(m, o, T, S, sc, s));
      else FMI_TRY(launch_attention_ex(w.Qh, w.Kh, w.Vt, o, B, H, L, L, w.Lpad, sc, m->attn_thr, s, qk8 ? 1 : 0, nullptr, 0, qk8 ? -m->n8_sgl[i] : ATT_NO_EXP2, m->attn_kind));
    }
    {
      PhaseTimer pt(m, s, PH_GEMM_PROJ);
      if (q_w2) FMI_TRY(quantize_act(m, bw.w2, w.big + 2 * D, ldbig, B * L, 0, s));
      else FMI_TRY(calib_rec(m, bw.w2, w.big + 2 * D, ldbig, B * L, s));
      GemmProblem p = q_w2 ? make_problem_fp8(m, bw.w2, 0, B * L, w.x, D, EPI_RESID_GATE_F32)
                           : make_problem(bw.w2, w.big + 2 * D, ldbig, B * L, w.x, D, EPI_RESID_GATE_F32);
      with_gate(p, mo + 2 * D, L, nmod);
      FMI_TRY(gemm1(m, p, bw.w2, s));
    }
    FMI_TRY(cn_hook(true, i, w.x + (size_t)T * D, (int64_t)L * D));
  }
  if (m->is_cn) return FMI_OK;
  if (sc) {
    if (!reuse) {
      PhaseTimer pt(m, s, PH_EMBED);
      FMI_TRY(launch_step_cache_delta(w.x + (size_t)T * D, (int64_t)L * D, m->sc_x0.as<float>(), m->sc_delta.as<float>(), B, (int64_t)S * D, s));
      sc->ref ^= 1, sc->valid = true;
    }
    ++sc->step;
  }

  {
    PhaseTimer pt(m, s, PH_FINAL);
    const float* mf = mod + m->mod_final_off;
    for (int b = 0; b < B; ++b)
      FMI_TRY(launch_layernorm_mod(w.x + ((size_t)b * L + T) * D, mf + (size_t)b * nmod, mf + (size_t)b * nmod + D, 0, 0,
                                   w.xm + (size_t)b * Ss * D, Ss, D, 1e-6f, s));
    GemmProblem p = make_problem(m->final_proj, w.xm, D, B * Ss, pred, C, EPI_STORE_F32);
    FMI_TRY(gemm1(m, p, m->final_proj, s));
  }
  return FMI_OK;
}

int check_inputs(fmi_flux* m, const fmi_flux_inputs* in) {
  if (!m || !in) return fail(FMI_ERR_INVALID, "flux: null handle or inputs");
  if (in->B <= 0 || in->S <= 0 || in->T <= 0) return fail(FMI_ERR_INVALID, "flux: B, S, T must be positive");
  if (in->B > 8) return fail(FMI_ERR_UNSUPPORTED, "flux: batch > 8 per device not supported (shard across GPUs)");
  if (!in->img_ids || !in->txt || !in->txt_ids || !in->y) return fail(FMI_ERR_INVALID, "flux: null input tensor");
  FMI_TRY(use_device(m));
  return check_ready(m);
}

int validate(fmi_flux* m, const fmi_flux_inputs* in, const fmi_flux_denoise_options& o, const fmi_flux_controlnet* cn, const fmi_flux_ip* ip, int n_steps, const char* bad_io,
             EvalPlan* p) {
  if (m && m->is_cn) return fail(FMI_ERR_UNSUPPORTED, "flux: a ControlNet handle is evaluated through the main model (fmi_flux_forward_controlnet / fmi_flux_denoise_controlnet) or fmi_flux_controlnet_eval");
  if ((o.x0 || o.noise || o.mask) && !(o.x0 && o.noise && o.mask)) return fail(FMI_ERR_INVALID, "flux_denoise: x0, noise and mask go together (all three or none)");
  FMI_TRY(check_inputs(m, in));
  if (bad_io) return fail(FMI_ERR_INVALID, bad_io);
  const bool sp = m->sp_world > 1 && m->sp_a2a;
  const auto f32_or_bf16 = [](fmi_dtype t) { return t == FMI_F32 || t == FMI_BF16; };
  *p = EvalPlan{o, 0, in->B};
  if (const fmi_flux_context* ctx = o.ctx; ctx && ctx->R != 0) {
    if (ctx->R < 0) return fail(FMI_ERR_INVALID, "flux: context R must not be negative");
    if (!ctx->ctx || !ctx->ctx_ids) return fail(FMI_ERR_INVALID, "flux: a context of R > 0 rows needs ctx and ctx_ids");
    if (!f32_or_bf16(ctx->ctx_dtype)) return fail(FMI_ERR_INVALID, "flux: ctx_dtype must be F32 or BF16");
    if (sp) return fail(FMI_ERR_UNSUPPORTED, "flux: a context is not supported under sequence parallelism");
    p->R = ctx->R;
  }
  if (!m->cond && o.ctl) return fail(FMI_ERR_INVALID, "flux: a control was given to a model without conditioning channels (fmi_flux_create_cond)");
  if (m->cond) {
    if (!o.ctl || !o.ctl->cond)
      return fail(FMI_ERR_INVALID, "flux: this model has " + std::to_string(m->cond) + " conditioning channels: every evaluation needs a control (fmi_flux_forward_control, fmi_flux_denoise_with)");
    if (!f32_or_bf16(o.ctl->cond_dtype)) return fail(FMI_ERR_INVALID, "flux: cond_dtype must be F32 or BF16");
// ... 453 lines not shown
static int step_cache_ensure(fmi_flux* m, int B, int rows, hipStream_t s) {
  const size_t per = (size_t)rows * m->D, elems = (size_t)B * per, part = (size_t)B * step_cache_groups((int64_t)per) * 2;
  if (m->sc_elems < elems || m->sc_part_floats < part) {
    FMI_HIP_TRY(hipStreamSynchronize(s));
    m->sc_x0.reset(), m->sc_r[0].reset(), m->sc_r[1].reset(), m->sc_delta.reset(), m->sc_part.reset(), m->sc_elems = 0, m->sc_part_floats = 0;
    for (DeviceBuffer* b : {&m->sc_x0, &m->sc_r[0], &m->sc_r[1], &m->sc_delta})
      if (b->alloc(elems * 4) != hipSuccess) return fail(FMI_ERR_NOMEM, "flux_denoise: hipMalloc of a step-cache buffer (" + std::to_string(elems * 4) + " bytes) failed");
    if (m->sc_part.alloc(part * 4) != hipSuccess) return fail(FMI_ERR_NOMEM, "flux_denoise: hipMalloc of the step cache's partial sums failed");
    m->sc_elems = elems, m->sc_part_floats = part;
  }
  if (!m->sc_sums) FMI_HIP_TRY(m->sc_sums.alloc(2 * 8 * sizeof(double)));
  if (!m->sc_host) FMI_HIP_TRY(hipHostMalloc((void**)&m->sc_host, 2 * 8 * sizeof(double), hipHostMallocDefault));
  return FMI_OK;
}

static int hoist_steps(fmi_flux* m, const fmi_flux_inputs* in, const double* timesteps_host, int n_steps, hipStream_t s, const float** mod_steps, const float** txt_pre) {
  const int B = in->B;
  std::vector<float> tv((size_t)(n_steps > 0 ? n_steps : 1) * B);
  for (int i = 0; i < n_steps; ++i)
    for (int b = 0; b < B; ++b) tv[(size_t)i * B + b] = 1.0f * (float)timesteps_host[i];
  FMI_HIP_TRY(hipMemcpyAsync(m->ws.tv, tv.data(), tv.size() * 4, hipMemcpyHostToDevice, s));
  FMI_HIP_TRY(hipStreamSynchronize(s));
  *mod_steps = nullptr;
  const size_t R = (size_t)n_steps * B, nmod = (size_t)m->n_mod;
  if (n_steps > 1 && R * nmod * 4 <= (2ull << 30)) {
    if (m->mod_steps_rows < R) {
      FMI_HIP_TRY(hipStreamSynchronize(s));
      m->mod_steps.reset(), m->vec_steps.reset(), m->vec_steps_bf.reset(), m->temb_steps.reset(), m->h1_steps.reset(), m->mod_steps_rows = 0;
      FMI_HIP_TRY(m->mod_steps.alloc(R * nmod * 4));
      FMI_HIP_TRY(m->vec_steps.alloc(R * (size_t)m->D * 4));
      FMI_HIP_TRY(m->vec_steps_bf.alloc(R * (size_t)m->D * 2));
      FMI_HIP_TRY(m->temb_steps.alloc(R * (size_t)256 * 4));
      FMI_HIP_TRY(m->h1_steps.alloc(std::max<size_t>(R, 2 * (size_t)B) * (size_t)m->D * 4));
      m->mod_steps_rows = R;
    }
    {
      PhaseTimer pt(m, s, PH_EMBED);
      FMI_TRY(compute_vec_steps(m, in, m->ws.tv, n_steps, m->vec_steps.as<float>(), m->temb_steps.as<float>(), m->h1_steps.as<float>(), s));
    }
    {
      PhaseTimer pt(m, s, PH_MOD);
      constexpr int GEMV_MAXROWS = 4;
      if (m->mod_all.q_type || (m->mod_gemm && (R > GEMV_MAXROWS || m->mod_gemm == 2) && m->D % 64 == 0 && nmod % 8 == 0 && R * nmod < (1ull << 31))) {
        FMI_TRY(launch_silu_to_bf16(m->vec_steps.as<float>(), m->vec_steps_bf.as<bf16_t>(), (int64_t)R * m->D, s));
        GemmProblem p = make_problem(m->mod_all, m->vec_steps_bf.as<bf16_t>(), m->D, (int)R, m->mod_steps.as<float>(), (int)nmod, EPI_STORE_F32);
        FMI_TRY(gemm1(m, p, m->mod_all, s));
      } else {
        for (size_t r0 = 0; r0 < R; r0 += GEMV_MAXROWS)
          FMI_TRY(launch_gemv(m->vec_steps.as<float>() + r0 * m->D, m->mod_all.w, m->mod_all.b, m->mod_steps.as<float>() + r0 * nmod, (int)std::min<size_t>(GEMV_MAXROWS, R - r0),
                              (int)nmod, m->D, 1, 0, s));
      }
    }
    *mod_steps = m->mod_steps.as<float>();
  }
  *txt_pre = nullptr;
  if (n_steps > 1) {
    PhaseTimer pt(m, s, PH_EMBED);
    GemmProblem p = make_problem(m->txt_in, m->ws.txt_bf, m->cfg.joint_attention_dim, B * in->T, m->ws.x_txt0, m->D, EPI_STORE_F32);
    FMI_TRY(gemm1(m, p, m->txt_in, s));
    *txt_pre = m->ws.x_txt0;
  }
  return FMI_OK;
}

struct CnRun {
  fmi_flux* net;
  const float *mod_steps, *txt_pre;
  std::vector<float> c;
};
struct IpRun {
  const fmi_ip_adapter* a;
  std::vector<float> c;
};
static int run_steps(fmi_flux* m, const fmi_flux_inputs* in, const EvalPlan& p, float* img_inout, const double* timesteps_host, int n_steps, const float* mod_steps,
                     const float* txt_pre, StepCacheRun* sc, const CnRun* cn, const IpRun* ip, hipStream_t s) {
  const fmi_flux_denoise_options& o = p.o;
  const size_t B = in->B, nmod = m->n_mod;
  const int64_t n = (int64_t)p.Bs * in->S * m->cfg.in_channels;
  for (int i = 0; i < n_steps; ++i) {
    CnInject inj{};
    const IpInject ipj{ip && ip->c[i] != 0.f ? ip->a : nullptr, ip ? ip->c[i] : 0.f};
    if (cn && cn->c[i] != 0.f) {
      fmi_flux* net = cn->net;
      FMI_TRY(forward_core(net, in, cn_plan(p), img_inout, net->ws.tv + i * B, nullptr, cn->mod_steps ? cn->mod_steps + i * B * (size_t)net->n_mod : nullptr, cn->txt_pre,
                           nullptr, nullptr, nullptr, s));
      inj = CnInject{net, cn->c[i]};
    }
    FMI_TRY(forward_core(m, in, p, img_inout, m->ws.tv + i * B, m->ws.pred_tmp, mod_steps ? mod_steps + i * B * nmod : nullptr, txt_pre, sc, inj.net ? &inj : nullptr,
                         ipj.a ? &ipj : nullptr, s));
    const float dt = (float)(timesteps_host[i + 1] - timesteps_host[i]);
    if (o.cfg)
      FMI_TRY(launch_euler_cfg(img_inout, m->ws.pred_tmp, m->ws.pred_tmp + n, o.cfg->scale, dt, n, s, o.x0, o.noise, o.mask, (float)timesteps_host[i + 1]));
    else if (o.mask)
      FMI_TRY(launch_euler_blend(img_inout, m->ws.pred_tmp, o.x0, o.noise, o.mask, dt, (float)timesteps_host[i + 1], n, s));
    else
      FMI_TRY(launch_euler_update(img_inout, m->ws.pred_tmp, dt, n, s));
  }
  return FMI_OK;
}

static int denoise_loop(fmi_flux* m, const fmi_flux_inputs* in_caller, const fmi_flux_denoise_options& o, const fmi_flux_controlnet* cn, const fmi_flux_ip* ip,
                        float* img_inout, const double* timesteps_host, int n_steps, void* stream) {
  EvalPlan p;
  FMI_TRY(validate(m, in_caller, o, cn, ip, n_steps, img_inout && timesteps_host && n_steps >= 0 ? nullptr : "flux_denoise: null img/timesteps or negative n_steps", &p));
  hipStream_t s = (hipStream_t)stream;
  fmi_flux_inputs in = *in_caller;
// ... 559 lines not shown
```

### diffusion-rs_amd/csrc/gemm_bf16.hip

```cpp
#include <cstdlib>
#include <type_traits>

#include <atomic>

#include "common.h"

namespace fmi {

constexpr int TILE_BAND = 8;
constexpr int BM = 256, BK = 64;
constexpr int GEMM_THREADS = 512;
constexpr int A_TILE_BYTES = BM * BK * 2;
constexpr int MAX_PROBLEMS = 8;

struct GemmBatch {
  GemmProblem p[MAX_PROBLEMS];
  int tile_start[MAX_PROBLEMS + 1];
  int band[MAX_PROBLEMS];
  int nprob;
};

}
#include "gemm_frame.h"
namespace fmi {
// ... 220 lines not shown
          const float4 c01 = pc01[u], c23 = pc23[u];
          const float cs[4] = {c01.x, c01.z, c23.x, c23.z};
          const float sn[4] = {c01.y, c01.w, c23.y, c23.w};
          const float inv = rms_inv128(ss);
          float rr8[8];
#pragma unroll
          for (int p = 0; p < 4; ++p) {
            const float x0 = v[2 * p] * inv * bf16_to_f32(we[2 * p]);
            const float x1 = v[2 * p + 1] * inv * bf16_to_f32(we[2 * p + 1]);
            rr8[2 * p] = cs[p] * x0 - sn[p] * x1;
            rr8[2 * p + 1] = sn[p] * x0 + cs[p] * x1;
          }
          const int64_t row = ((int64_t)b * P.qk_H + head0 + hh) * P.qk_Ltot + pos;
          if (P.qk_q8 > 0.f) {
            const float sc8 = part == 0 ? P.qk_q8 : P.qk_k8;
            int lo = 0, hi = 0;
            lo = __builtin_amdgcn_cvt_pk_fp8_f32(rr8[0] * sc8, rr8[1] * sc8, lo, false);
            lo = __builtin_amdgcn_cvt_pk_fp8_f32(rr8[2] * sc8, rr8[3] * sc8, lo, true);
            hi = __builtin_amdgcn_cvt_pk_fp8_f32(rr8[4] * sc8, rr8[5] * sc8, hi, false);
            hi = __builtin_amdgcn_cvt_pk_fp8_f32(rr8[6] * sc8, rr8[7] * sc8, hi, true);
            *reinterpret_cast<uint2*>(reinterpret_cast<uint8_t*>(osel) + row * 128 + sub * 8) = make_uint2((uint32_t)lo, (uint32_t)hi);
          } else {
            bf16_t* dst = osel + row * 128 + sub * 8;
            *reinterpret_cast<uint4*>(dst) = make_uint4(pack_bf16x2(rr8[0], rr8[1]), pack_bf16x2(rr8[2], rr8[3]), pack_bf16x2(rr8[4], rr8[5]), pack_bf16x2(rr8[6], rr8[7]));
          }
        }
      }
    }
  } else {
    const bf16_t* tp = reinterpret_cast<const bf16_t*>(smem);
    const int g8 = lane & 31;
#pragma unroll 4
    for (int it = 0; it < 16; ++it) {
      const int dc = wave * 32 + it * 2 + hl;
      const int m16 = m0 + 16 * (g8 >> 1);
      if (m16 < P.M) {
        const uint4 x = *reinterpret_cast<const uint4*>(tp + dc * 256 + g8 * 8);
        const int b = m16 / P.qk_rows, kv16 = P.qk_row_off + (m16 - b * P.qk_rows);
        bf16_t* dst = P.qk_vt + (((int64_t)b * P.qk_H + head0 + (dc >> 7)) * 128 + (dc & 127)) * P.qk_Lpad + kv16 + (g8 & 1) * 8;
        *reinterpret_cast<uint4*>(dst) = x;
      }
    }
  }
}

template <class ACC>
__device__ __forceinline__ void qkv_relayout_epilogue(const GemmProblem& P, const ACC& acc, char* smem, int m0, int n0, int wave, int lane) {
  __syncthreads();
  qkv_relayout_stage(P, acc, smem, n0, wave, lane);
  __syncthreads();
  qkv_relayout_emit(P, smem, m0, n0, wave, lane);
}

template <int NJ, int WN, int ACT, class ACC>
__device__ __forceinline__ void gemm_epilogue_impl(const GemmProblem& P, const ACC& acc, char* smem, int m0, int n0, int wave, int lane) {
  constexpr int BN = WN * 32 * NJ;
  const int wm = wave / WN, wn = wave % WN;
  const int epi = P.epi;
  const float alpha = P.alpha;
  auto add_bias = [](const uint2 b, float (&v)[4]) {
    v[0] += bf16_to_f32((bf16_t)(b.x & 0xffff));
    v[1] += bf16_to_f32((bf16_t)(b.x >> 16));
    v[2] += bf16_to_f32((bf16_t)(b.y & 0xffff));
    v[3] += bf16_to_f32((bf16_t)(b.y >> 16));
  };
  auto scale = [&](float (&v)[4]) {
    if constexpr (ACT == 3 || ACT == -1) {
      if (epi == EPI_STORE_F32 || epi == EPI_SCALE_BF16) {
#pragma unroll
        for (int e = 0; e < 4; ++e) v[e] *= alpha;
      }
    }
  };
  const int tile_gelu = n0 >= P.gelu_from ? 1 : (n0 + BN <= P.gelu_from ? -1 : 0);
  auto activate = [&](int n, float (&v)[4]) {
    if constexpr (ACT == -1) {
      if (epi == EPI_GELU_BF16 || (epi == EPI_GELU_FROM_COL && n >= P.gelu_from)) {
        gelu_tanh4(v);
      } else if (epi == EPI_SILU_BF16) {
#pragma unroll
        for (int e = 0; e < 4; ++e) v[e] = silu(v[e]);
      }
    } else if constexpr (ACT == 1) {
      gelu_tanh4(v);
    } else if constexpr (ACT == 2) {
      if (tile_gelu > 0 || (tile_gelu == 0 && n >= P.gelu_from)) gelu_tanh4(v);
    } else if constexpr (ACT == 3) {
      if (epi == EPI_SILU_BF16) {
#pragma unroll
        for (int e = 0; e < 4; ++e) v[e] = silu(v[e]);
      }
    }
  };
  auto finish = [&](int n, float (&v)[4], bool full) {
    scale(v);
    if (P.bias) {
      if (full) {
        add_bias(*reinterpret_cast<const uint2*>(P.bias + n), v);
      } else {
        for (int e = 0; e < 4 && n + e < P.N; ++e) v[e] += bf16_to_f32(P.bias[n + e]);
      }
    }
    activate(n, v);
  };
  const bool f32_out = (epi == EPI_RESID_GATE_F32 || epi == EPI_STORE_F32);
  const bool staged = (P.ldo % 8 == 0) && (n0 + BN <= P.N) && ((reinterpret_cast<uintptr_t>(P.out) & 15) == 0) && epi != EPI_RESID_ADD_BF16 &&
                      (P.bias == nullptr || (reinterpret_cast<uintptr_t>(P.bias) & 7) == 0);
// ... 1 lines not shown
    __syncthreads();
    char* cw = smem + wave * (8192 * NJ);
    const int ncol0 = n0 + wn * 32 * NJ;
    constexpr bool WIDE = ACC::kSlots <= 4;
    uint2 bc[WIDE ? 1 : ACC::kSlots];
    float bf[WIDE ? ACC::kSlots : 1][4];
    acc.cols([&](int slot, int c) {
      uint2 b = make_uint2(0u, 0u);
      if (P.bias) b = *reinterpret_cast<const uint2*>(P.bias + ncol0 + 4 * c);
      if constexpr (WIDE) {
        bf[slot][0] = bf16_to_f32((bf16_t)(b.x & 0xffff)), bf[slot][1] = bf16_to_f32((bf16_t)(b.x >> 16));
        bf[slot][2] = bf16_to_f32((bf16_t)(b.y & 0xffff)), bf[slot][3] = bf16_to_f32((bf16_t)(b.y >> 16));
      } else {
        bc[slot] = b;
      }
    });
    auto finish_s = [&](int slot, int n, float (&v)[4]) {
      scale(v);
      if constexpr (WIDE) {
#pragma unroll
        for (int e = 0; e < 4; ++e) v[e] += bf[slot][e];
      } else {
        add_bias(bc[slot], v);
      }
      activate(n, v);
    };
    if (!f32_out) {
      constexpr int RB = 64 * NJ;
      constexpr int NS8 = 8 * NJ;
      acc.template each<-1>([&](int r, int c, float (&v)[4], int slot) {
        finish_s(slot, ncol0 + 4 * c, v);
        *reinterpret_cast<uint2*>(cw + r * RB + ((c ^ (r & (NS8 - 1))) << 3)) = make_uint2(pack_bf16x2(v[0], v[1]), pack_bf16x2(v[2], v[3]));
      });
      asm volatile("s_waitcnt lgkmcnt(0)" ::: "memory");
      constexpr int LPR = RB / 16, RPI = 64 / LPR;
      bf16_t* ob = reinterpret_cast<bf16_t*>(P.out);
#pragma unroll
      for (int it = 0; it < 128 / RPI; ++it) {
        const int r = it * RPI + lane / LPR, ch = lane % LPR;
        const int sp = ((2 * ch) ^ (r & (NS8 - 1))) & ~1;
        uint4 d = *reinterpret_cast<const uint4*>(cw + r * RB + (sp << 3));
        if (r & 1) d = make_uint4(d.z, d.w, d.x, d.y);
        const int m = m0 + wm * 128 + r;
        if (m < P.M) __builtin_nontemporal_store(*reinterpret_cast<const i32x4_nt*>(&d), reinterpret_cast<i32x4_nt*>(ob + (int64_t)m * P.ldo + ncol0 + ch * 8));
        if constexpr (NJ == 4) {
          if ((it & 3) == 3) __builtin_amdgcn_sched_barrier(0);
        }
      }
    } else {
      constexpr int RBF = 128 * NJ;
      constexpr int NS16 = 8 * NJ;
      constexpr int LPR = RBF / 16, RPI = 64 / LPR;
      float* of = reinterpret_cast<float*>(P.out);
      auto f32_pass = [&](auto pass_tag) {
        constexpr int pass = decltype(pass_tag)::value;
        asm volatile("s_waitcnt lgkmcnt(0)" ::: "memory");
        acc.template each<pass>([&](int rg, int c, float (&v)[4], int slot) {
          finish_s(slot, ncol0 + 4 * c, v);
          const int r = rg - pass * 64;
          *reinterpret_cast<float4*>(cw + r * RBF + ((c ^ (r & (NS16 - 1))) << 4)) = make_float4(v[0], v[1], v[2], v[3]);
        });
        asm volatile("s_waitcnt lgkmcnt(0)" ::: "memory");
        constexpr int NIT = 64 / RPI;
        const int ch = lane % LPR, n = ncol0 + ch * 4;
        if (epi == EPI_RESID_GATE_F32) {
          constexpr int GRP = NIT < 8 ? NIT : 8;
#pragma unroll
          for (int g0 = 0; g0 < NIT; g0 += GRP) {
            float4 xr[GRP], gg[GRP];
#pragma unroll
            for (int u = 0; u < GRP; ++u) {
              const int r = (g0 + u) * RPI + lane / LPR;
              const int m = min(m0 + wm * 128 + pass * 64 + r, P.M - 1);
              const float* gate = P.gate + (P.rows_per_batch > 0 ? (int64_t)(m / P.rows_per_batch) * P.gate_bstride : 0);
              gg[u] = *reinterpret_cast<const float4*>(gate + n);
              xr[u] = *reinterpret_cast<const float4*>(of + (int64_t)m * P.ldo + n);
            }
#pragma unroll
            for (int u = 0; u < GRP; ++u) {
              const int r = (g0 + u) * RPI + lane / LPR;
              const int m = m0 + wm * 128 + pass * 64 + r;
              const float4 v = *reinterpret_cast<const float4*>(cw + r * RBF + ((ch ^ (r & (NS16 - 1))) << 4));
              if (m < P.M) {
                float4 x = xr[u];
                x.x += gg[u].x * v.x;
                x.y += gg[u].y * v.y;
                x.z += gg[u].z * v.z;
                x.w += gg[u].w * v.w;
                *reinterpret_cast<float4*>(of + (int64_t)m * P.ldo + n) = x;
              }
            }
          }
        } else {
#pragma unroll
          for (int it = 0; it < NIT; ++it) {
            const int r = it * RPI + lane / LPR;
            const float4 v = *reinterpret_cast<const float4*>(cw + r * RBF + ((ch ^ (r & (NS16 - 1))) << 4));
            const int m = m0 + wm * 128 + pass * 64 + r;
            if (m < P.M) *reinterpret_cast<float4*>(of + (int64_t)m * P.ldo + n) = v;
          }
        }
      };
      f32_pass(std::integral_constant<int, 0>{});
      f32_pass(std::integral_constant<int, 1>{});
    }
    return;
  }
  acc.template each<-1>([&](int r, int c, float (&v)[4], int) {
    const int m = m0 + wm * 128 + r;
    const int n = n0 + wn * 32 * NJ + 4 * c;
    if (m >= P.M || n >= P.N) return;
    const float* gate = P.gate;
    if (epi == EPI_RESID_GATE_F32 && P.rows_per_batch > 0) gate += (int64_t)(m / P.rows_per_batch) * P.gate_bstride;
    const bool full = (n + 3 < P.N) && (P.bias == nullptr || (reinterpret_cast<uintptr_t>(P.bias + n) & 7) == 0);
    finish(n, v, full);
    if (epi == EPI_RESID_GATE_F32) {
      float* o = reinterpret_cast<float*>(P.out) + (int64_t)m * P.ldo + n;
      for (int e = 0; e < 4 && n + e < P.N; ++e) o[e] += gate[n + e] * v[e];
    } else if (epi == EPI_STORE_F32) {
      float* o = reinterpret_cast<float*>(P.out) + (int64_t)m * P.ldo + n;
      for (int e = 0; e < 4 && n + e < P.N; ++e) o[e] = v[e];
    } else {
      bf16_t* o = reinterpret_cast<bf16_t*>(P.out) + (int64_t)m * P.ldo + n;
      if (epi == EPI_RESID_ADD_BF16) {
        const bf16_t* rs = reinterpret_cast<const bf16_t*>(P.resid) + (int64_t)m * P.ldo + n;
        for (int e = 0; e < 4 && n + e < P.N; ++e) v[e] += bf16_to_f32(rs[e]);
      }
      for (int e = 0; e < 4 && n + e < P.N; ++e) o[e] = f32_to_bf16(v[e]);
    }
  });
}

template <int NJ, int WN = 4, int ACT = -1, class ACC>
__device__ __forceinline__ void gemm_epilogue(const GemmProblem& P, const ACC& acc, char* smem, int m0, int n0, int wave, int lane) {
  if constexpr (NJ == 2 && WN == 4) {
    if (P.qk_qh != nullptr && n0 < 3 * P.qk_D) {
      qkv_relayout_epilogue(P, acc, smem, m0, n0, wave, lane);
      return;
    }
  }
  gemm_epilogue_impl<NJ, WN, ACT>(P, acc, smem, m0, n0, wave, lane);
}
inline int epilogue_kind(const GemmProblem* p, int n) {
  auto kind = [](int epi) { return (epi == EPI_STORE_BF16 || epi == EPI_RESID_GATE_F32) ? 0 : epi == EPI_GELU_BF16 ? 1 : epi == EPI_GELU_FROM_COL ? 2 : 3; };
  const int k = kind(p[0].epi);
  for (int i = 1; i < n; ++i)
    if (kind(p[i].epi) != k) return -1;
  return k;
}

template <int MODE, int NJ>
__global__ __launch_bounds__(GEMM_THREADS, 2) void gemm_bf16_kernel(const GemmBatch batch) {
  constexpr int BN = 128 * NJ;
  constexpr int W_TILE_BYTES = BN * BK * 2;
  constexpr int BUF_BYTES = A_TILE_BYTES + W_TILE_BYTES;
  __shared__ __attribute__((aligned(16))) char smem[2 * BUF_BYTES];
  const int tid = threadIdx.x;
  const int lane = tid & 63;
  const int wave = __builtin_amdgcn_readfirstlane(tid >> 6);
  const int wm = wave >> 2, wn = wave & 3;

  const GemmTile tile = gemm_tile<BN>(batch, 2);
  const GemmProblem& P = tile.P;
  const int m0 = tile.m0, n0 = tile.n0, nk = tile.nk;

  auto bufA = [&](int b) -> char* { return smem + b * BUF_BYTES; };
  auto bufW = [&](int b) -> char* { return smem + b * BUF_BYTES + A_TILE_BYTES; };

  f32x4 acc[8][2 * NJ];
  zero(acc);

  const FragSlots<16> frag = frag_slots<16>(lane);
  const int (&koff)[2] = frag.koff;
  const int a_row_off = frag.row_off(wm * 128);
  const int w_row_off = frag.row_off(wn * 32 * NJ);

  int cv_y[4], cv_x[4], cv_pix[4];
  const int cv_sh = MODE == 2 && P.cv_up > 0 ? P.cv_up : 0;
  const int cv_half = MODE == 2 && P.cv_up >= 0 ? P.cv_ks >> 1 : 0;
  const int cv_ow = P.cv_w << cv_sh, cv_oh = P.cv_h << cv_sh;
  const uint32_t cv_cin2 = (uint32_t)P.cv_cin * 2;
  if (MODE == 2) {
#pragma unroll
    for (int i = 0; i < 4; ++i) {
      int m = m0 + (wave * 4 + i) * 8 + (lane >> 3);
      m = m > P.M - 1 ? P.M - 1 : m;
      const bool down = P.cv_up < 0;
      const int ow = down ? P.cv_w >> 1 : cv_ow, oh = down ? P.cv_h >> 1 : cv_oh;
      const int x = m % ow, y = (m / ow) % oh, b = m / (ow * oh);
      cv_x[i] = down ? 2 * x : x;
      cv_y[i] = down ? 2 * y : y;
      cv_pix[i] = b * P.cv_h * P.cv_w;
    }
  }
  const int cv_slot[2] = {((lane & 7) ^ ((lane >> 4) & 7)) << 4, ((lane & 7) ^ ((4 + (lane >> 4)) & 7)) << 4};
  auto conv_src = [&](int i, int dy, int dx, int c0) -> const char* {
    const int yy = cv_y[i] + dy, xx = cv_x[i] + dx;
    const bool in = (unsigned)yy < (unsigned)cv_oh && (unsigned)xx < (unsigned)cv_ow;
    const uint32_t pix = (uint32_t)(cv_pix[i] + (yy >> cv_sh) * P.cv_w + (xx >> cv_sh));
    const char* src = reinterpret_cast<const char*>(P.A) + ((uint64_t)pix * cv_cin2 + (uint32_t)(c0 * 2 + cv_slot[i & 1]));
// ... 252 lines not shown
    }
    slot_barrier();
    wr = wr == 2 ? 0 : wr + 1;
    wi = wi == 2 ? 0 : wi + 1;
  };
  const int nmain = nk > 2 ? nk - 2 : 0;
  for (int t = 0; t < nmain; ++t) ktile(t, std::true_type{});
  for (int t = nmain; t < nk; ++t) ktile(t, std::false_type{});
  if (g == 0) slot_barrier();

  if constexpr (I8) {
#pragma unroll
    for (int i = 0; i < 4; ++i)
#pragma unroll
      for (int j = 0; j < NJ; ++j)
#pragma unroll
        for (int r = 0; r < 16; ++r) acc[i][j][r] = (float)acci[i][j][r];
  }
  if constexpr (FP8) {
    float sa[4], oa[4];
    const bool off = I8 && P.a_off != nullptr;
#pragma unroll
    for (int i = 0; i < 4; ++i) {
      const int r = min(m0 + g * 128 + i * 32 + (lane & 31), P.M - 1);
      sa[i] = P.a_scale[r];
      oa[i] = off ? P.a_off[r] : 0.f;
    }
#pragma unroll
    for (int j = 0; j < NJ; ++j)
#pragma unroll
      for (int q = 0; q < 4; ++q) {
        const int n = n0 + wn * 64 + j * 32 + 8 * q + 4 * (lane >> 5);
        float sn[4], wsn[4];
#pragma unroll
        for (int c = 0; c < 4; ++c) {
          sn[c] = P.w_scale[min(n + c, P.N - 1)];
          wsn[c] = off ? P.w_sum[min(n + c, P.N - 1)] : 0.f;
        }
        if (off) {
#pragma unroll
          for (int i = 0; i < 4; ++i)
#pragma unroll
            for (int c = 0; c < 4; ++c) acc[i][j][4 * q + c] = acc[i][j][4 * q + c] * (sa[i] * sn[c]) + oa[i] * wsn[c];
        } else {
#pragma unroll
          for (int i = 0; i < 4; ++i)
#pragma unroll
            for (int c = 0; c < 4; ++c) acc[i][j][4 * q + c] *= sa[i] * sn[c];
        }
      }
  }
  int lane_e = lane;
  asm volatile("" : "+v"(lane_e));
  if constexpr (FP8) gemm_epilogue<NJ, 4, ACT>(P, Acc32<NJ>{acc, lane_e}, smem, m0, n0, wave, lane_e);
  else gemm_epilogue<NJ, 4, ACT>(P, Acc16<NJ>{acc16, lane_e}, smem, m0, n0, wave, lane_e);
}


constexpr int W4_THREADS = 256;
template <int ACT, class V, int I, int J>
__device__ __forceinline__ void w4_epilogue(const GemmProblem& P, V (&acc)[I][J], char* smem, int m0, int n0, int wave, int wm, int wn, int lane) {
  using View = std::conditional_t<std::is_same<V, f32x16>::value, Acc32<2>, Acc16<2>>;
  constexpr int H = J / 2;
  int lane_e = lane;
  asm volatile("" : "+v"(lane_e));
  if (P.qk_qh != nullptr && n0 < 3 * P.qk_D) {
    __syncthreads();
    {
      V hacc[I][H];
#pragma unroll
      for (int i = 0; i < I; ++i)
#pragma unroll
        for (int j = 0; j < H; ++j) hacc[i][j] = acc[i][j];
#pragma clang loop unroll(disable)
      for (int r = 0; r < 2; ++r) {
        qkv_relayout_stage(P, View{hacc, lane_e}, smem, n0, wm * 4 + wn * 2 + r, lane_e);
#pragma unroll
        for (int i = 0; i < I; ++i)
#pragma unroll
          for (int j = 0; j < H; ++j) hacc[i][j] = acc[i][H + j];
        asm volatile("" : "+v"(lane_e));
      }
    }
    __syncthreads();
#pragma clang loop unroll(disable)
    for (int r = 0; r < 2; ++r) {
      qkv_relayout_emit(P, smem, m0, n0, wave * 2 + r, lane_e);
      asm volatile("" : "+v"(lane_e));
    }
    return;
  }
  V hacc[I][H];
#pragma unroll
  for (int i = 0; i < I; ++i)
#pragma unroll
    for (int j = 0; j < H; ++j) hacc[i][j] = acc[i][j];
#pragma clang loop unroll(disable)
  for (int r = 0; r < 2; ++r) {
    gemm_epilogue_impl<2, 4, ACT>(P, View{hacc, lane_e}, smem, m0, n0, wm * 4 + wn * 2 + r, lane_e);
#pragma unroll
    for (int i = 0; i < I; ++i)
#pragma unroll
      for (int j = 0; j < H; ++j) hacc[i][j] = acc[i][H + j];
    asm volatile("" : "+v"(lane_e));
  }
}

#if FMI_ALT_KERNELS
template <int ACT>
__global__ __launch_bounds__(W4_THREADS, 1) void gemm_w4_kernel(const GemmBatch batch) {
  constexpr int NJ = 4, BN = 256;
  constexpr int A_RING = 0, W_RING = 2 * A_TILE_BYTES, TILE = A_TILE_BYTES;
  constexpr int ES = 2;
  __shared__ __attribute__((aligned(16))) char smem[5 * TILE];
  const int tid = threadIdx.x;
  const int lane = tid & 63;
  const int wave = __builtin_amdgcn_readfirstlane(tid >> 6);
  const int wm = wave >> 1, wn = wave & 1;

  const GemmTile tile = gemm_tile<BN>(batch, ES);
  const GemmProblem& P = tile.P;
  const int m0 = tile.m0, n0 = tile.n0, nk = tile.nk;

  f32x4 acc[8][8];
  zero(acc);

  const uint32_t lds0 = (uint32_t)(uintptr_t)(lds_void*)smem;
  const FragSlots<16> frag = frag_slots<16>(lane);
  const int (&koff)[2] = frag.koff;
  const uint32_t a_row = lds0 + A_RING + frag.row_off(wm * 128);
  const uint32_t w_row = lds0 + W_RING + frag.row_off(wn * 128);

  const TileDma<8> dma(P, m0, n0, ES, wave * 8, wave * 8, lane);
  auto dma_a = [&](int kt, int i) {
    const char* base = dma.a_base + (int64_t)kt * (BK * 2);
    const uint32_t l = lds0 + A_RING + (kt & 1) * TILE + (wave * 8 + i) * 1024;
    asm volatile("s_mov_b32 m0, %2\n\ts_nop 0\n\tglobal_load_lds_dwordx4 %0, %1" ::"v"(dma.a_off[i]), "s"(base), "s"(l) : "memory");
  };
  auto dma_w = [&](int kt, int slot, int i) {
    const char* base = dma.w_base + (int64_t)kt * (BK * 2);
    const uint32_t l = lds0 + W_RING + slot * TILE + (wave * 8 + i) * 1024;
    asm volatile("s_mov_b32 m0, %2\n\ts_nop 0\n\tglobal_load_lds_dwordx4 %0, %1" ::"v"(dma.w_off[i]), "s"(base), "s"(l) : "memory");
  };
  auto sync_all = [&]() {
    __builtin_amdgcn_sched_barrier(0);
    __builtin_amdgcn_s_barrier();
    __builtin_amdgcn_sched_barrier(0);
  };

  const int klast = nk - 1;
#pragma unroll
  for (int i = 0; i < 8; ++i) dma_a(0, i);
#pragma unroll
  for (int i = 0; i < 8; ++i) dma_w(0, 0, i);
#pragma unroll
  for (int i = 0; i < 8; ++i) dma_w(min(1, klast), 1, i);
#pragma unroll
// ... 27 lines not shown
      case 10: FMI_W4_RD(wf[s][2], w_ad[s], 4096); break;
      case 11: FMI_W4_RD(wf[s][3], w_ad[s], 6144); break;
      case 12: FMI_W4_RD(wf[s][4], w_ad[s], 8192); break;
      case 13: FMI_W4_RD(wf[s][5], w_ad[s], 10240); break;
      case 14: FMI_W4_RD(wf[s][6], w_ad[s], 12288); break;
      default: FMI_W4_RD(wf[s][7], w_ad[s], 14336); break;
    }
  };
#define FMI_W4_WAIT(N, s)                                                                                                                         \
  asm volatile("s_waitcnt lgkmcnt(" #N ")"                                                                                                        \
               : "+v"(xf[s][0]), "+v"(xf[s][1]), "+v"(xf[s][2]), "+v"(xf[s][3]), "+v"(xf[s][4]), "+v"(xf[s][5]), "+v"(xf[s][6]), "+v"(xf[s][7]), \
                 "+v"(wf[s][0]), "+v"(wf[s][1]), "+v"(wf[s][2]), "+v"(wf[s][3]), "+v"(wf[s][4]), "+v"(wf[s][5]), "+v"(wf[s][6]), "+v"(wf[s][7]))
  auto mfma = [&](int s, int i, int j) {
    asm volatile("v_mfma_f32_16x16x32_bf16 %0, %1, %2, %0" : "+a"(acc[i][j]) : "v"(wf[s][j]), "v"(xf[s][i]));
  };

  rebase(0, 0);
#pragma unroll
  for (int w = 0; w < 16; ++w) read_frag(0, w);
  int wslot = 0;
  for (int t = 0; t < nk; ++t) {
    const int wnext = wslot == 2 ? 0 : wslot + 1;
    const int wnn = wnext == 2 ? 0 : wnext + 1;
    const int kt2 = min(t + 2, klast);
    FMI_W4_WAIT(0, 0);
    __builtin_amdgcn_sched_barrier(0);
#pragma unroll
    for (int q = 0; q < 64; ++q) {
      mfma(0, q >> 3, q & 7);
      if (q % 3 == 1 && q / 3 < 16) read_frag(1, q / 3);
      if ((q & 7) == 3) dma_w(kt2, wnn, q >> 3);
      __builtin_amdgcn_sched_barrier(0);
    }
    FMI_W4_WAIT(0, 1);
    asm volatile("s_waitcnt vmcnt(8)" ::: "memory");
    sync_all();
    rebase((t + 1) & 1, wnext);
#pragma unroll
    for (int q = 0; q < 64; ++q) {
      mfma(1, q >> 3, q & 7);
      if (q % 3 == 1 && q / 3 < 16) read_frag(0, q / 3);
      if ((q & 7) == 5) dma_a(kt2, q >> 3);
      __builtin_amdgcn_sched_barrier(0);
    }
    wslot = wnext;
  }
  asm volatile("s_waitcnt vmcnt(0) lgkmcnt(0)\n\ts_nop 15\n\ts_nop 15" ::: "memory");
#pragma unroll
  for (int i = 0; i < 8; ++i)
#pragma unroll
    for (int j = 0; j < 8; ++j) asm volatile("" : "+a"(acc[i][j]));
#undef FMI_W4_RD
#undef FMI_W4_WAIT
  w4_epilogue<ACT>(P, acc, smem, m0, n0, wave, wm, wn, lane);
}

#endif

}
#include "gemm_w4q.h"
namespace fmi {

static std::atomic<bool> g_pingpong{true};
static std::atomic<bool> g_w4{[] {
  const char* e = getenv("FMI_GEMM_W4");
  return e ? atoi(e) != 0 : false;
}()};
static std::atomic<int> g_w4q_min_rows{256};
static std::atomic<int> g_w4_qkv_min_n{[]() { const char* e = getenv("FMI_GEMM_W4_QKV_MIN_N"); return e && atoi(e) > 0 ? atoi(e) : 1 << 30; }()};
void set_gemm_w4_qkv_min_n(int n) { g_w4_qkv_min_n = n; }
void set_gemm_w4q_min_rows(int rows) { g_w4q_min_rows = rows; }
void set_gemm_w4(bool on) { g_w4 = on; }
void set_gemm_pingpong(bool on) { g_pingpong = on; }

static int pick_tile_band(int tiles_m) {
  static const int pinned = [] {
    const char* e = getenv("FMI_GEMM_BAND");
    return e ? atoi(e) : 0;
  }();
  if (pinned > 0) return pinned;
  if (tiles_m <= TILE_BAND || tiles_m % TILE_BAND == 0) return TILE_BAND;
  auto panels = [](int r) { return (double)r + 32.0 / r; };
  int best = TILE_BAND;
  double best_cost = 1e30;
  for (int h = 5; h <= 10; ++h) {
    const int rag = tiles_m % h;
    const double cost = (tiles_m - rag) * panels(h) + (rag ? rag * panels(rag) : 0.0);
    if (cost < best_cost - 1e-9) best_cost = cost, best = h;
  }
  return best;
}

static int gemm_tile_width(const GemmProblem* probs, int nprob) {
  int max_n = 0;
  for (int i = 0; i < nprob; ++i) max_n = std::max(max_n, probs[i].N);
  int bn = max_n <= 128 ? 128 : 256;
  if (probs[0].cv_ks != 0 && bn == 256) {
    int64_t tiles = 0;
    for (int i = 0; i < nprob; ++i) tiles += (int64_t)cdiv(probs[i].M, BM) * cdiv(probs[i].N, 256);
    if (tiles <= 192) bn = 128;
  }
  return bn;
}
static bool gemm_w4_pays(const GemmProblem* probs, int nprob, int qkv_min_n) {
  if (probs[0].fp8 != 0 || probs[0].cv_ks != 0 || probs[0].q_type != 0) return false;
  for (int i = 0; i < nprob; ++i) {
    const GemmProblem& p = probs[i];
    if (p.epi != EPI_RESID_GATE_F32 && p.K < 8192 && !(p.qk_qh && p.N >= qkv_min_n)) return false;
  }
  return true;
}
static bool gemm_w4q_ok(const GemmProblem* probs, int nprob, int min_rows) {
  if (probs[0].q_type == 0) return false;
  for (int i = 0; i < nprob; ++i) {
    const GemmProblem& p = probs[i];
    const int kb = p.q_blocksize / BK;
    if (p.q_type == 3 || p.M < min_rows || p.K % p.q_blocksize || (kb & (kb - 1)) || (int64_t)p.N * p.K / 2 >= (1ll << 32)) return false;
  }
  return true;
}

static int validate_gemm_problems(const GemmProblem* probs, int nprob, int bn) {
  const bool quant = probs[0].q_type != 0, conv = probs[0].cv_ks != 0, fp8 = probs[0].fp8 != 0;
  for (int i = 0; i < nprob; ++i) {
    const GemmProblem& p = probs[i];
    if (p.M <= 0 || p.N <= 0) return fail(FMI_ERR_INVALID, "launch_gemm: empty problem");
    if (p.fp8 != probs[0].fp8 || p.fp8 < 0 || p.fp8 > 2) return fail(FMI_ERR_INVALID, "launch_gemm: cannot mix e4m3 / int8 / bf16 problems in one group");
    if (fp8 && (p.q_type || p.cv_ks || bn != 256 || p.K % 128 || p.lda % 16 || p.ldw % 16 || !p.a_scale || !p.w_scale))
      return fail(FMI_ERR_INVALID, "launch_gemm: fp8 needs dense operands, N > 128, K / lda / ldw multiples of 128 / 16 / 16 and both scale vectors");
    if ((p.a_off != nullptr) != (p.w_sum != nullptr) || (p.a_off && p.fp8 != 2))
      return fail(FMI_ERR_INVALID, "launch_gemm: the offset term (a_off, w_sum) belongs to int8 problems and needs both vectors");
    if (p.K <= 0 || p.K % BK != 0) return fail(FMI_ERR_INVALID, "launch_gemm: K must be a positive multiple of 64, got " + std::to_string(p.K));
    if ((p.q_type != 0) != quant || (p.cv_ks != 0) != conv) return fail(FMI_ERR_INVALID, "launch_gemm: cannot mix dense / 4-bit / conv problems in one group");
    if (quant && conv) return fail(FMI_ERR_UNSUPPORTED, "launch_gemm: quantised convolution");
    if ((!conv && p.lda % 8) || (!quant && p.ldw % 8)) return fail(FMI_ERR_INVALID, "launch_gemm: lda/ldw must be multiples of 8 elements (16-byte rows)");
    if (conv && (p.cv_cin % 64 || p.K != p.cv_ks * p.cv_ks * p.cv_cin || !p.cv_zero)) return fail(FMI_ERR_INVALID, "launch_gemm: bad conv descriptor (Cin % 64, K = k*k*Cin)");
    if (quant && p.q_type != 3 && (p.q_blocksize % 64 != 0 || p.q_blocksize <= 0)) return fail(FMI_ERR_INVALID, "launch_gemm: 4-bit blocksize must be a multiple of 64");
    if (p.epi == EPI_RESID_GATE_F32) {
      if (!p.gate) return fail(FMI_ERR_INVALID, "launch_gemm: the gated residual epilogue needs a gate vector");
      if ((reinterpret_cast<uintptr_t>(p.gate) & 15) || p.gate_bstride % 4)
        return fail(FMI_ERR_INVALID, "launch_gemm: gate must be 16-byte aligned and gate_bstride a multiple of 4 elements (read as float4)");
    }
    if (p.epi == EPI_RESID_ADD_BF16 && !p.resid) return fail(FMI_ERR_INVALID, "launch_gemm: the bf16 residual-add epilogue needs resid");
    if (p.epi == EPI_GELU_FROM_COL && p.gelu_from % 4) return fail(FMI_ERR_INVALID, "launch_gemm: gelu_from must be a multiple of 4 (decided per 4-column group), got " + std::to_string(p.gelu_from));
    if (p.rows_per_batch < 0) return fail(FMI_ERR_INVALID, "launch_gemm: rows_per_batch must be >= 0");
    if (p.qk_qh) {
      if (conv || bn != 256 || p.qk_D % 256 || p.qk_H * 128 != p.qk_D || 3 * p.qk_D > p.N || p.qk_rows <= 0 || p.qk_rows % 16 || p.qk_row_off % 16 || p.M % 16 ||
          p.qk_Lpad % 64 || !p.qk_kh || !p.qk_vt || !p.qk_wq || !p.qk_wk || !p.qk_pe || (p.bias && (reinterpret_cast<uintptr_t>(p.bias) & 7)))
        return fail(FMI_ERR_INVALID, "launch_gemm: bad fused qkv relayout descriptor (needs 256-wide tiles, D % 256 == 0, rows/row_off/M % 16 == 0)");
    }
  }
  if (epilogue_kind(probs, nprob) < 0) return fail(FMI_ERR_INVALID, "launch_gemm: the problems of a grouped launch must share the activation kind");
  return FMI_OK;
}

enum GemmKernel {
  GK_DB128,
  GK_DB256,
  GK_Q4_DB,
  GK_CONV,
  GK_PP,
  GK_PP_E4M3,
  GK_PP_I8,
  GK_W4,
  GK_W4Q,
};
enum GemmOperands { GO_DENSE, GO_Q4, GO_CONV };
struct GemmTraits {
  GemmOperands operands;
  int q8;
  int bn;
  bool w4_pays, w4q_ok;
};
struct GemmSwitches {
  bool pingpong, w4;
  int w4q_min_rows, w4_qkv_min_n;
};
struct GemmChoice {
  GemmKernel kernel;
  fmi_status err;
  const char* msg;
};
GemmChoice select_gemm_kernel(const GemmTraits& t, const GemmSwitches& sw, bool alt) {
  if (t.q8 == 2) return {GK_PP_I8, FMI_OK, nullptr};
  if (t.q8) return {GK_PP_E4M3, FMI_OK, nullptr};
  if (t.operands == GO_CONV) return {GK_CONV, FMI_OK, nullptr};
  if (t.operands == GO_Q4) return {t.bn == 256 && t.w4q_ok ? GK_W4Q : GK_Q4_DB, FMI_OK, nullptr};
  if (t.bn != 256) return {GK_DB128, FMI_OK, nullptr};
  const bool w4 = sw.w4 && t.w4_pays;
  if (!alt && (w4 || !sw.pingpong))
    return {GK_PP, FMI_ERR_UNSUPPORTED, "launch_gemm: the dense 4-wave / double-buffered 256-wide kernels live in the test build (libflux_mi355x_alt.so: make alt)"};
  return {w4 ? GK_W4 : !sw.pingpong ? GK_DB256 : GK_PP, FMI_OK, nullptr};
}

template <class F>
static int with_act(int act, F&& launch) {
  switch (act) {
    case 0: return launch(std::integral_constant<int, 0>{});
    case 1: return launch(std::integral_constant<int, 1>{});
    case 2: return launch(std::integral_constant<int, 2>{});
    default: return launch(std::integral_constant<int, 3>{});
  }
}

int launch_gemm(const GemmProblem* probs, int nprob, hipStream_t stream) {
  if (nprob <= 0) return FMI_OK;
  if (nprob > MAX_PROBLEMS) return fail(FMI_ERR_INVALID, "launch_gemm: too many grouped problems");
  const int bn = gemm_tile_width(probs, nprob);
  FMI_TRY(validate_gemm_problems(probs, nprob, bn));
  const GemmSwitches sw{g_pingpong, g_w4, g_w4q_min_rows, g_w4_qkv_min_n};
  const GemmTraits t{probs[0].cv_ks != 0 ? GO_CONV : probs[0].q_type != 0 ? GO_Q4 : GO_DENSE, probs[0].fp8, bn,
                     gemm_w4_pays(probs, nprob, sw.w4_qkv_min_n), gemm_w4q_ok(probs, nprob, sw.w4q_min_rows)};
  const GemmChoice c = select_gemm_kernel(t, sw, FMI_ALT_KERNELS != 0);
  if (c.err != FMI_OK) return fail(c.err, c.msg);
  GemmBatch b;
  b.nprob = nprob;
  int total = 0;
  for (int i = 0; i < nprob; ++i) {
    b.p[i] = probs[i];
    b.tile_start[i] = total;
    b.band[i] = pick_tile_band(cdiv(probs[i].M, BM));
    total += cdiv(probs[i].M, BM) * cdiv(probs[i].N, bn);
  }
  for (int i = nprob; i <= MAX_PROBLEMS; ++i) b.tile_start[i] = total;
  for (int i = nprob; i < MAX_PROBLEMS; ++i) b.band[i] = TILE_BAND;
  const bool wide = bn == 256;
  return with_act(epilogue_kind(probs, nprob), [&](auto act) -> int {
    constexpr int ACT = decltype(act)::value;
    auto launch = [&](auto kernel, int threads) { hipLaunchKernelGGL(kernel, dim3(total), dim3(threads), 0, stream, b); };
    switch (c.kernel) {
      case GK_DB128: launch(gemm_bf16_kernel<0, 1>, GEMM_THREADS); break;
      case GK_Q4_DB: wide ? launch(gemm_bf16_kernel<1, 2>, GEMM_THREADS) : launch(gemm_bf16_kernel<1, 1>, GEMM_THREADS); break;
      case GK_CONV: wide ? launch(gemm_bf16_kernel<2, 2>, GEMM_THREADS) : launch(gemm_bf16_kernel<2, 1>, GEMM_THREADS); break;
      case GK_PP: launch(gemm_pp_kernel<0, ACT>, GEMM_THREADS); break;
      case GK_PP_E4M3: launch(gemm_pp_kernel<1, ACT>, GEMM_THREADS); break;
      case GK_PP_I8: launch(gemm_pp_kernel<2, ACT>, GEMM_THREADS); break;
      case GK_W4Q:
        FMI_LDS_GUARD((gemm_w4q_kernel<ACT>), W4Q_LUT_BYTES + 4 * A_TILE_BYTES);
        launch(gemm_w4q_kernel<ACT>, W4_THREADS);
        break;
#if FMI_ALT_KERNELS
      case GK_DB256: launch(gemm_bf16_kernel<0, 2>, GEMM_THREADS); break;
      case GK_W4: launch(gemm_w4_kernel<ACT>, W4_THREADS); break;
#endif
      default: return fail(FMI_ERR_UNSUPPORTED, "launch_gemm: the selected kernel is not part of this build");
    }
    FMI_LAUNCH_CHECK();
    return FMI_OK;
  });
}

}
```

### diffusion-rs_amd/csrc/norm_rope.hip

```cpp
#include "common.h"

namespace fmi {

template <bool REG>
__global__ __launch_bounds__(256) void layernorm_mod_kernel(const float* __restrict x1, const float* __restrict scale1,
                                                            const float* __restrict shift1, int mod_bstride, int rows_per_batch1,
                                                            bf16_t* __restrict out1, int D, float eps, int rows1, const float* __restrict x2,
                                                            const float* __restrict scale2, const float* __restrict shift2, int rows_per_batch2,
                                                            bf16_t* __restrict out2) {
  __shared__ float red[2][4];
  const bool second = (int)blockIdx.x >= rows1;
  const int row = second ? blockIdx.x - rows1 : blockIdx.x;
  const float* x = second ? x2 : x1;
  const float* scale = second ? scale2 : scale1;
  const float* shift = second ? shift2 : shift1;
  const int rows_per_batch = second ? rows_per_batch2 : rows_per_batch1;
  bf16_t* out = second ? out2 : out1;
  const float4* xr = reinterpret_cast<const float4*>(x + (int64_t)row * D);
  const int nv = D >> 2;
  constexpr int MAXV = 4;
  float4 keep[MAXV], ksc[MAXV], ksh[MAXV];
  float s = 0.f, s2 = 0.f;
  const int batch = rows_per_batch > 0 ? row / rows_per_batch : 0;
  const float4* sc = scale ? reinterpret_cast<const float4*>(scale + (int64_t)batch * mod_bstride) : nullptr;
  const float4* sh = shift ? reinterpret_cast<const float4*>(shift + (int64_t)batch * mod_bstride) : nullptr;
  if constexpr (REG) {
#pragma unroll
    for (int c = 0; c < MAXV; ++c) {
      const int i = threadIdx.x + c * 256;
      if (i < nv) {
        const float4 v = xr[i];
        keep[c] = v;
        if (sc) ksc[c] = sc[i];
        if (sh) ksh[c] = sh[i];
        s += (v.x + v.y) + (v.z + v.w);
        s2 += (v.x * v.x + v.y * v.y) + (v.z * v.z + v.w * v.w);
      }
    }
  } else {
    for (int i = threadIdx.x; i < nv; i += 256) {
      const float4 v = xr[i];
      s += (v.x + v.y) + (v.z + v.w);
      s2 += (v.x * v.x + v.y * v.y) + (v.z * v.z + v.w * v.w);
    }
  }
  s = wave_sum(s);
  s2 = wave_sum(s2);
  const int w = threadIdx.x >> 6;
  if ((threadIdx.x & 63) == 0) {
    red[0][w] = s;
    red[1][w] = s2;
  }
  __syncthreads();
  s = (red[0][0] + red[0][1]) + (red[0][2] + red[0][3]);
  s2 = (red[1][0] + red[1][1]) + (red[1][2] + red[1][3]);
  const float mean = s / (float)D;
  const float var = s2 / (float)D - mean * mean;
  const float inv_std = 1.0f / sqrtf(var + eps);
  uint2* o = reinterpret_cast<uint2*>(out + (int64_t)row * D);
  auto emit = [&](int i, const float4 v, const float4 ksc_i, const float4 ksh_i) {
    float a = (v.x - mean) * inv_std, b = (v.y - mean) * inv_std, c = (v.z - mean) * inv_std, d = (v.w - mean) * inv_std;
    if (sc) {
      const float4 k = ksc_i;
      a *= (k.x + 1.0f);
      b *= (k.y + 1.0f);
      c *= (k.z + 1.0f);
      d *= (k.w + 1.0f);
    }
    if (sh) {
      const float4 k = ksh_i;
      a += k.x;
      b += k.y;
      c += k.z;
      d += k.w;
    }
    o[i] = make_uint2(pack_bf16x2(a, b), pack_bf16x2(c, d));
  };
  if constexpr (REG) {
#pragma unroll
    for (int c = 0; c < MAXV; ++c) {
      const int i = threadIdx.x + c * 256;
      if (i < nv) emit(i, keep[c], ksc[c], ksh[c]);
    }
  } else {
    const float4 z = make_float4(0.f, 0.f, 0.f, 0.f);
    for (int i = threadIdx.x; i < nv; i += 256) emit(i, xr[i], sc ? sc[i] : z, sh ? sh[i] : z);
  }
}

int launch_layernorm_mod2(const float* x, const float* scale, const float* shift, int mod_bstride, int rows_per_batch, bf16_t* out, int rows,
                          const float* x2, const float* scale2, const float* shift2, int rows_per_batch2, bf16_t* out2, int rows2, int D, float eps,
                          hipStream_t stream) {
  if (rows + rows2 <= 0) return FMI_OK;
  if (D % 4) return fail(FMI_ERR_INVALID, "layernorm_mod: D must be a multiple of 4");
  if (D <= 4096)
    hipLaunchKernelGGL(layernorm_mod_kernel<true>, dim3(rows + rows2), dim3(256), 0, stream, x, scale, shift, mod_bstride, rows_per_batch, out, D, eps, rows,
                       x2, scale2, shift2, rows_per_batch2, out2);
  else
    hipLaunchKernelGGL(layernorm_mod_kernel<false>, dim3(rows + rows2), dim3(256), 0, stream, x, scale, shift, mod_bstride, rows_per_batch, out, D, eps, rows,
                       x2, scale2, shift2, rows_per_batch2, out2);
  FMI_LAUNCH_CHECK();
  return FMI_OK;
}
int launch_layernorm_mod(const float* x, const float* scale, const float* shift, int mod_bstride, int rows_per_batch, bf16_t* out,
                         int rows, int D, float eps, hipStream_t stream) {
  return launch_layernorm_mod2(x, scale, shift, mod_bstride, rows_per_batch, out, rows, nullptr, nullptr, nullptr, 0, nullptr, 0, D, eps, stream);
}

template <bool F32OUT>
__global__ __launch_bounds__(256) void qk_norm_rope_kernel(const bf16_t* __restrict q, const bf16_t* __restrict k, int ld,
                                                           int64_t in_bstride, const bf16_t* __restrict wq,
                                                           const bf16_t* __restrict wk, const float* __restrict pe,
                                                           int64_t pe_bstride, void* __restrict qo, void* __restrict ko, int B,
                                                           int H, int rows, int row_off, int Ltot) {
  const int64_t gid = (int64_t)blockIdx.x * 16 + (threadIdx.x >> 4);
  const int sub = threadIdx.x & 15;
  const int64_t total = (int64_t)B * rows * H;
  if (gid >= total) return;
  const int h = (int)(gid % H);
  const int64_t br = gid / H;
  const int r = (int)(br % rows), b = (int)(br / rows);
  const int pos = row_off + r;
  const float4* pp = reinterpret_cast<const float4*>(pe + (int64_t)b * pe_bstride + ((int64_t)pos * 64 + 4 * sub) * 2);
  const float4 c01 = pp[0], c23 = pp[1];
  const float cs[4] = {c01.x, c01.z, c23.x, c23.z};
  const float sn[4] = {c01.y, c01.w, c23.y, c23.w};
#pragma unroll
  for (int which = 0; which < 2; ++which) {
    const bf16_t* src = (which ? k : q) + (int64_t)b * in_bstride + (int64_t)r * ld + h * 128 + sub * 8;
    const bf16_t* wv = (which ? wk : wq) + sub * 8;
    const int64_t doff = (((int64_t)b * H + h) * Ltot + pos) * 128 + sub * 8;
    const uint4 raw = *reinterpret_cast<const uint4*>(src);
    const uint4 wraw = *reinterpret_cast<const uint4*>(wv);
    const bf16_t* e = reinterpret_cast<const bf16_t*>(&raw);
    const bf16_t* we = reinterpret_cast<const bf16_t*>(&wraw);
    float v[8];
    float ss = 0.f;
#pragma unroll
    for (int i = 0; i < 8; ++i) {
      v[i] = bf16_to_f32(e[i]);
      ss += v[i] * v[i];
    }
    ss = row16_sum(ss);
    const float inv = rms_inv128(ss);
    uint32_t o[4];
    float of[8];
#pragma unroll
    for (int p = 0; p < 4; ++p) {
      const float x0 = v[2 * p] * inv * bf16_to_f32(we[2 * p]);
      const float x1 = v[2 * p + 1] * inv * bf16_to_f32(we[2 * p + 1]);
      of[2 * p] = cs[p] * x0 - sn[p] * x1, of[2 * p + 1] = sn[p] * x0 + cs[p] * x1;
      o[p] = pack_bf16x2(of[2 * p], of[2 * p + 1]);
    }
    if (F32OUT) {
      float4* d4 = reinterpret_cast<float4*>(static_cast<float*>(which ? ko : qo) + doff);
      d4[0] = make_float4(of[0], of[1], of[2], of[3]);
      d4[1] = make_float4(of[4], of[5], of[6], of[7]);
    } else {
      *reinterpret_cast<uint4*>(static_cast<bf16_t*>(which ? ko : qo) + doff) = make_uint4(o[0], o[1], o[2], o[3]);
// ... 65 lines not shown
```

### include/flux_mi355x.h

```cpp
#ifndef FLUX_MI355X_H
#define FLUX_MI355X_H

#include <stddef.h>
#include <stdint.h>

#ifdef __cplusplus
extern "C" {
#endif
#pragma GCC visibility push(default)

#define FMI_ABI_VERSION 6

typedef enum fmi_status {
  FMI_OK = 0,
  FMI_ERR_INVALID = -1,
  FMI_ERR_HIP = -2,
  FMI_ERR_STATE = -3,
  FMI_ERR_UNSUPPORTED = -4,
  FMI_ERR_NOMEM = -5
} fmi_status;

typedef enum fmi_dtype {
  FMI_F32 = 0,
  FMI_F16 = 1,
// ... 306 lines not shown
                         int N, int K, fmi_epilogue epi, void* stream);
int fmi_linear_int8_bf16(const void* x, const int8_t* weight, const float* scb, const void* bias, void* y,
                         int M, int N, int K, fmi_epilogue epi, void* stream);
int fmi_quantize_rows_fp8(const void* x, int rows, int K, uint8_t* out, float* scale, void* stream);
int fmi_linear_fp8(const void* x, const uint8_t* wq, const float* w_scale, const void* bias, void* y, int M, int N,
                   int K, fmi_epilogue epi, void* stream);
int fmi_quantize_rows_i8(const void* x, int rows, int K, int8_t* out, float* scale, void* stream);
int fmi_linear_i8(const void* x, const int8_t* wq, const float* w_scale, const void* bias, void* y, int M, int N,
                  int K, fmi_epilogue epi, void* stream);
size_t fmi_linear_q8_workspace_bytes(int M, int K);
int fmi_linear_fp8_ws(const void* x, const uint8_t* wq, const float* w_scale, const void* bias, void* y, int M, int N, int K,
                      fmi_epilogue epi, void* workspace, size_t workspace_bytes, void* stream);
int fmi_linear_i8_ws(const void* x, const int8_t* wq, const float* w_scale, const void* bias, void* y, int M, int N, int K,
                     fmi_epilogue epi, void* workspace, size_t workspace_bytes, void* stream);
int fmi_gemm_q8(const void* xq, const float* x_scale, const void* wq, const float* w_scale, const void* bias, void* y,
                int M, int N, int K, int kind, fmi_epilogue epi, void* stream);
int fmi_quantize_rows_i8_asym(const void* x, int rows, int K, int d0, int8_t* out, float* scale, float* offset, void* stream);
int fmi_rowsum_i8(const int8_t* wq, const float* w_scale, int N, int K, int d0, float* w_sum, void* stream);
int fmi_quantize_rows_i8_scaled(const void* x, int rows, int K, int d0, const float* col_scale, int8_t* out, float* scale, float* offset, void* stream);
int fmi_col_absmax(const void* x, int rows, int K, int ld, float* amax_inout, void* stream);
int fmi_gemm_i8_asym(const void* xq, const float* x_scale, const float* x_offset, const void* wq, const float* w_scale, const float* w_sum,
                     const void* bias, void* y, int M, int N, int K, fmi_epilogue epi, void* stream);
typedef enum fmi_gemm_epi {
  FMI_GEMM_STORE_BF16 = 0,
  FMI_GEMM_GELU_BF16 = 1,
  FMI_GEMM_RESID_GATE_F32 = 2,
  FMI_GEMM_GELU_FROM_COL = 3,
  FMI_GEMM_STORE_F32 = 4,
  FMI_GEMM_SCALE_BF16 = 5,
  FMI_GEMM_RESID_ADD_BF16 = 6,
  FMI_GEMM_SILU_BF16 = 7
} fmi_gemm_epi;
typedef struct fmi_gemm_desc {
  const void* a;
  const void* w;
  const void* bias;
  void* out;
  const float* gate;
  const void* resid;
  int M, N, K;
  int lda, ldw, ldo;
  int epi;
  int gelu_from;
  float alpha;
  int rows_per_batch;
  int gate_bstride;
  int q8;
  const float* a_scale;
  const float* w_scale;
  const float* a_off;
  const float* w_sum;
} fmi_gemm_desc;
int fmi_gemm_group(const fmi_gemm_desc* probs, int nprob, void* stream);
int fmi_splitk_resid_gate(const float* parts, int S, const void* bias, const float* gate, int rows_per_batch, int gate_bstride, float* out, int ldo,
                          int M, int N, void* stream);
int fmi_set_gemm_kernel(int pingpong, int w4);
int fmi_sdpa_bf16(const void* q, const void* k, const void* v, void* o, int B, int H, int Lq,
                  int Lk, int d, float scale, int out_token_major, void* stream);
size_t fmi_sdpa_workspace_bytes(int B, int H, int Lk);
int fmi_release_scratch(size_t* freed_bytes);
int fmi_sdpa_bf16_ws(const void* q, const void* k, const void* v, void* o, int B, int H, int Lq, int Lk, int d, float scale,
                     int out_token_major, void* workspace, size_t workspace_bytes, void* stream);
int fmi_set_attention_kernel(int kind);
int fmi_sdpa_fp8qk(const void* q, const void* k, const void* v, void* o, int B, int H, int Lq,
                  int Lk, int d, float scale, int out_token_major, void* stream);
#define FMI_SDPA_NO_EXP2 (1 << 30)
int fmi_sdpa_fp8qk_ws(const void* q, const void* k, const void* v, void* o, int B, int H, int Lq, int Lk, int d, float scale,
                      int score_exp2, int out_token_major, void* workspace, size_t workspace_bytes, void* stream);
int fmi_sdpa_fp8(const void* q, const void* k, const void* v, void* o, int B, int H, int Lq, int Lk, int d, float scale, int score_exp2,
                 float v_scale, int out_token_major, void* stream);
int fmi_sdpa_fp8_ws(const void* q, const void* k, const void* v, void* o, int B, int H, int Lq, int Lk, int d, float scale, int score_exp2,
                    float v_scale, int out_token_major, void* workspace, size_t workspace_bytes, void* stream);
int fmi_layernorm_mod(const float* x, const float* scale, const float* shift, void* out_bf16,
                      int rows, int D, float eps, void* stream);
int fmi_timestep_embedding(const float* t, int B, int dim, float* out, void* stream);
int fmi_rope_table(const float* txt_ids, const float* img_ids, int B, int T, int S, const int* axes_dim , int theta, float* pe, void* stream);
int fmi_rmsnorm_rope(const void* q, const void* k, int ld, const void* q_weight, const void* k_weight, const float* pe, void* q_out, void* k_out,
                     int B, int H, int L, int d, fmi_dtype out_dtype, void* stream);
int fmi_groupnorm_nhwc(const void* x_bf16, const float* weight, const float* bias, void* out_bf16,
                       int B, int HW, int C, int groups, float eps, int fuse_silu, void* stream);
int fmi_conv2d_nhwc(const void* x_bf16, const void* w_bf16, const void* bias_bf16,
                    const void* residual_bf16, void* out_bf16, int B, int in_h, int in_w, int Cin,
                    int Cout, int ksize, int upsample2x, void* stream);

void dequantize_blockwise_f32_int8(const float* code, const uint8_t* A, const float* absmax, float* out, int blocksize, int n, void* stream);
void dequantize_blockwise_f32_fp4(const float* code, const uint8_t* A, const float* absmax, float* out, int blocksize, int n, void* stream);
void dequantize_blockwise_f32_nf4(const float* code, const uint8_t* A, const float* absmax, float* out, int blocksize, int n, void* stream);
void dequantize_blockwise_f16_int8(const float* code, const uint8_t* A, const float* absmax, void* out, int blocksize, int n, void* stream);
void dequantize_blockwise_f16_fp4(const float* code, const uint8_t* A, const float* absmax, void* out, int blocksize, int n, void* stream);
void dequantize_blockwise_f16_nf4(const float* code, const uint8_t* A, const float* absmax, void* out, int blocksize, int n, void* stream);
void dequantize_blockwise_bf16_int8(const float* code, const uint8_t* A, const float* absmax, void* out, int blocksize, int n, void* stream);
void dequantize_blockwise_bf16_fp4(const float* code, const uint8_t* A, const float* absmax, void* out, int blocksize, int n, void* stream);
void dequantize_blockwise_bf16_nf4(const float* code, const uint8_t* A, const float* absmax, void* out, int blocksize, int n, void* stream);
void dequantize_8bit_kernel_f32(const int8_t* weight, const float* scb, float* out, int row, int col, int n);
void dequantize_8bit_kernel_f16(const int8_t* weight, const float* scb, void* out, int row, int col, int n);
void dequantize_8bit_kernel_bf16(const int8_t* weight, const float* scb, void* out, int row, int col, int n);

int fmi_malloc(void** dptr, size_t bytes);
int fmi_free(void* dptr);
int fmi_memcpy(void* dst, const void* src, size_t bytes, void* stream);
int fmi_memset(void* dst, int value, size_t bytes, void* stream);
int fmi_stream_synchronize(void* stream);
int fmi_event_create(void** ev);
int fmi_event_record(void* ev, void* stream);
int fmi_event_elapsed_ms(void* start, void* stop, float* ms);
int fmi_event_destroy(void* ev);
// ... 7 lines not shown
```

Baseline: 0.3238 images/s.

## Fold modulated LayerNorm into adjacent GEMM epilogues via precomputed column vectors

```diff
diff --git a/diffusion-rs_amd/_lib.py b/diffusion-rs_amd/_lib.py
--- a/diffusion-rs_amd/_lib.py
+++ b/diffusion-rs_amd/_lib.py
@@ -89,6 +89,13 @@
                 ("M", C.c_int), ("N", C.c_int), ("K", C.c_int), ("lda", C.c_int), ("ldw", C.c_int), ("ldo", C.c_int), ("epi", C.c_int),
                 ("gelu_from", C.c_int), ("alpha", C.c_float), ("rows_per_batch", C.c_int), ("gate_bstride", C.c_int), ("q8", C.c_int),
                 ("a_scale", C.c_void_p), ("w_scale", C.c_void_p), ("a_off", C.c_void_p), ("w_sum", C.c_void_p)]
+
+
+class GemmLnDesc(C.Structure):
+    _fields_ = [("scale", C.c_void_p), ("m0_prev", C.c_void_p), ("part_prev", C.c_void_p), ("m0", C.c_void_p), ("part", C.c_void_p), ("a", C.c_void_p),
+                ("stats", C.c_void_p), ("c1", C.c_void_p), ("c2", C.c_void_p), ("prev_tiles", C.c_int), ("lda", C.c_int), ("ld", C.c_int), ("tiles", C.c_int),
+                ("qh", C.c_void_p), ("kh", C.c_void_p), ("vt", C.c_void_p), ("wq", C.c_void_p), ("wk", C.c_void_p),
+                ("pe", C.c_void_p), ("qk_H", C.c_int), ("qk_rows", C.c_int), ("qk_row_off", C.c_int), ("qk_Ltot", C.c_int), ("qk_Lpad", C.c_int)]
 
 
 GEMM_STORE_BF16, GEMM_GELU_BF16, GEMM_RESID_GATE_F32, GEMM_GELU_FROM_COL, GEMM_STORE_F32, GEMM_SCALE_BF16, GEMM_RESID_ADD_BF16, GEMM_SILU_BF16 = range(8)
@@ -262,6 +269,7 @@
     lib.fmi_linear_bf16.argtypes = [C.c_void_p, C.c_void_p, C.c_void_p, C.c_void_p, C.c_int, C.c_int, C.c_int, C.c_int, C.c_void_p]
     lib.fmi_quantize_rows_fp8.argtypes = [C.c_void_p, C.c_int, C.c_int, C.c_void_p, C.c_void_p, C.c_void_p]
     lib.fmi_gemm_group.argtypes = [C.POINTER(GemmDesc), C.c_int, C.c_void_p]
+    lib.fmi_gemm_ln.argtypes = [C.POINTER(GemmDesc), C.POINTER(GemmLnDesc), C.c_void_p]
     lib.fmi_splitk_resid_gate.argtypes = [C.c_void_p, C.c_int, C.c_void_p, C.c_void_p, C.c_int, C.c_int, C.c_void_p, C.c_int, C.c_int, C.c_int, C.c_void_p]
     lib.fmi_set_gemm_kernel.argtypes = [C.c_int, C.c_int]
     lib.fmi_linear_fp8.argtypes = [C.c_void_p, C.c_void_p, C.c_void_p, C.c_void_p, C.c_void_p, C.c_int, C.c_int, C.c_int, C.c_int, C.c_void_p]
@@ -348,7 +356,7 @@
     "fmi_t5_size_in_bytes", "fmi_t5_forward", "fmi_clip_default_config", "fmi_clip_create", "fmi_clip_destroy", "fmi_clip_set_tensor",
     "fmi_clip_missing_count", "fmi_clip_missing_name", "fmi_clip_size_in_bytes", "fmi_clip_forward", "fmi_pack_latents", "fmi_unpack_latents", "fmi_postprocess_u8",
     "fmi_preprocess_u8", "fmi_latent_mask", "fmi_encode_latents", "fmi_scale_noise", "fmi_latent_ids", "fmi_cfg_euler_step", "fmi_cast_cols_bf16", "fmi_mask_image", "fmi_fill_condition",
-    "fmi_randn", "fmi_philox_u32", "fmi_calculate_shift", "fmi_get_timesteps", "fmi_linear_bf16", "fmi_linear_bnb4_bf16", "fmi_linear_int8_bf16", "fmi_quantize_rows_fp8", "fmi_linear_fp8", "fmi_quantize_rows_i8", "fmi_linear_i8", "fmi_gemm_q8", "fmi_quantize_rows_i8_asym", "fmi_rowsum_i8", "fmi_quantize_rows_i8_scaled", "fmi_col_absmax", "fmi_gemm_i8_asym", "fmi_gemm_group", "fmi_splitk_resid_gate", "fmi_set_gemm_kernel", "fmi_linear_q8_workspace_bytes", "fmi_linear_fp8_ws", "fmi_linear_i8_ws", "fmi_sdpa_bf16", "fmi_sdpa_fp8qk", "fmi_sdpa_workspace_bytes", "fmi_sdpa_bf16_ws", "fmi_sdpa_fp8qk_ws", "fmi_sdpa_fp8", "fmi_sdpa_fp8_ws", "fmi_set_attention_kernel", "fmi_layernorm_mod",
+    "fmi_randn", "fmi_philox_u32", "fmi_calculate_shift", "fmi_get_timesteps", "fmi_linear_bf16", "fmi_linear_bnb4_bf16", "fmi_linear_int8_bf16", "fmi_quantize_rows_fp8", "fmi_linear_fp8", "fmi_quantize_rows_i8", "fmi_linear_i8", "fmi_gemm_q8", "fmi_quantize_rows_i8_asym", "fmi_rowsum_i8", "fmi_quantize_rows_i8_scaled", "fmi_col_absmax", "fmi_gemm_i8_asym", "fmi_gemm_group", "fmi_gemm_ln", "fmi_splitk_resid_gate", "fmi_set_gemm_kernel", "fmi_linear_q8_workspace_bytes", "fmi_linear_fp8_ws", "fmi_linear_i8_ws", "fmi_sdpa_bf16", "fmi_sdpa_fp8qk", "fmi_sdpa_workspace_bytes", "fmi_sdpa_bf16_ws", "fmi_sdpa_fp8qk_ws", "fmi_sdpa_fp8", "fmi_sdpa_fp8_ws", "fmi_set_attention_kernel", "fmi_layernorm_mod",
     "fmi_release_scratch", "fmi_timestep_embedding", "fmi_rope_table", "fmi_rmsnorm_rope",
     "fmi_groupnorm_nhwc", "fmi_conv2d_nhwc",
     "fmi_comm_probe", "fmi_comm_unique_id", "fmi_comm_create", "fmi_comm_destroy", "fmi_comm_rank", "fmi_comm_world_size", "fmi_comm_stats", "fmi_comm_all_to_all",
diff --git a/diffusion-rs_amd/csrc/capi.hip b/diffusion-rs_amd/csrc/capi.hip
--- a/diffusion-rs_amd/csrc/capi.hip
+++ b/diffusion-rs_amd/csrc/capi.hip
@@ -352,7 +352,13 @@
   return launch_gemm(&p, 1, (hipStream_t)stream);
 }
 
-extern "C" int fmi_gemm_group(const fmi_gemm_desc* probs, int nprob, void* stream) {
+static int gemm_group_ln(const fmi_gemm_desc* probs, int nprob, const fmi_gemm_ln_desc* ln, void* stream);
+extern "C" int fmi_gemm_group(const fmi_gemm_desc* probs, int nprob, void* stream) { return gemm_group_ln(probs, nprob, nullptr, stream); }
+extern "C" int fmi_gemm_ln(const fmi_gemm_desc* prob, const fmi_gemm_ln_desc* ln, void* stream) {
+  if (!prob || !ln) return fail(FMI_ERR_INVALID, "gemm_ln: null descriptor");
+  return gemm_group_ln(prob, 1, ln, stream);
+}
+static int gemm_group_ln(const fmi_gemm_desc* probs, int nprob, const fmi_gemm_ln_desc* ln, void* stream) {
   if (nprob <= 0) return FMI_OK;
   if (!probs) return fail(FMI_ERR_INVALID, "gemm_group: null descriptor array");
   if (nprob > 8) return fail(FMI_ERR_INVALID, "gemm_group: too many grouped problems (at most 8), got " + std::to_string(nprob));
@@ -380,6 +386,23 @@
     p.epi = d.epi, p.gelu_from = d.gelu_from, p.alpha = d.alpha, p.rows_per_batch = d.rows_per_batch, p.gate_bstride = d.gate_bstride;
     p.fp8 = d.q8, p.a_scale = d.a_scale, p.w_scale = d.w_scale, p.a_off = d.a_off, p.w_sum = d.w_sum;
   }
+  if (ln) {
+    GemmProblem& p = gp[0];
+    if (ln->prev_tiles < 0 || ln->tiles < 0 || ln->ld < p.M) return fail(FMI_ERR_INVALID, "gemm_ln: prev_tiles, tiles >= 0 and ld >= M required");
+    if (misaligned(ln->m0_prev, 4) || misaligned(ln->m0, 4)) return fail(FMI_ERR_INVALID, "gemm_ln: m0 pointers must be 4-byte aligned");
+    p.ln_scale = ln->scale, p.ln_m0_prev = ln->m0_prev, p.ln_part_prev = ln->part_prev, p.ln_m0 = ln->m0, p.ln_part = ln->part, p.ln_a = (bf16_t*)ln->a;
+    p.ln_stats = ln->stats, p.ln_c1 = ln->c1, p.ln_c2 = ln->c2;
+    p.ln_prev_tiles = ln->prev_tiles, p.ln_lda = ln->lda, p.ln_ld = ln->ld, p.ln_tiles = ln->tiles;
+    if (ln->qh) {
+      if (misaligned(ln->qh, 16) || misaligned(ln->kh, 16) || misaligned(ln->vt, 16) || misaligned(ln->wq, 16) || misaligned(ln->wk, 16) || misaligned(ln->pe, 16))
+        return fail(FMI_ERR_INVALID, "gemm_ln: the relayout's buffers must be 16-byte aligned");
+      if (ln->qk_H <= 0 || ln->qk_row_off < 0 || ln->qk_rows <= 0 || ln->qk_Ltot < ln->qk_row_off + ln->qk_rows || ln->qk_Lpad < ln->qk_Ltot)
+        return fail(FMI_ERR_INVALID, "gemm_ln: bad relayout shape (H, rows > 0, row_off + rows <= Ltot <= Lpad)");
+      p.qk_qh = (bf16_t*)ln->qh, p.qk_kh = (bf16_t*)ln->kh, p.qk_vt = (bf16_t*)ln->vt, p.qk_wq = (const bf16_t*)ln->wq, p.qk_wk = (const bf16_t*)ln->wk;
+      p.qk_pe = ln->pe, p.qk_pe_bstride = 0;
+      p.qk_H = ln->qk_H, p.qk_D = ln->qk_H * 128, p.qk_rows = ln->qk_rows, p.qk_row_off = ln->qk_row_off, p.qk_Ltot = ln->qk_Ltot, p.qk_Lpad = ln->qk_Lpad;
+    }
+  }
   return launch_gemm(gp, nprob, (hipStream_t)stream);
 }
 extern "C" int fmi_splitk_resid_gate(const float* parts, int S, const void* bias, const float* gate, int rows_per_batch, int gate_bstride, float* out, int ldo,
diff --git a/diffusion-rs_amd/csrc/common.h b/diffusion-rs_amd/csrc/common.h
--- a/diffusion-rs_amd/csrc/common.h
+++ b/diffusion-rs_amd/csrc/common.h
@@ -271,7 +271,18 @@
   const float* w_scale;
   const float* a_off;
   const float* w_sum;
-};
+  const float* ln_scale;
+  const float* ln_m0_prev;
+  const float* ln_part_prev;
+  float* ln_m0;
+  float* ln_part;
+  bf16_t* ln_a;
+  const float* ln_stats;
+  const float* ln_c1;
+  const float* ln_c2;
+  int ln_prev_tiles, ln_lda, ln_ld, ln_tiles;
+};
+bool gemm_ln_fold_available(int K);
 int launch_gemm(const GemmProblem* probs, int nprob, hipStream_t stream);
 void set_gemm_w4(bool on);
 void set_gemm_pingpong(bool on);
@@ -337,13 +348,14 @@
                       int theta, float* pe, hipStream_t stream, const float* ctx_ids = nullptr, int R = 0);
 int launch_layernorm_mod2(const float* x, const float* scale, const float* shift, int mod_bstride, int rows_per_batch, bf16_t* out, int rows,
                           const float* x2, const float* scale2, const float* shift2, int rows_per_batch2, bf16_t* out2, int rows2, int D, float eps,
-                          hipStream_t stream);
+                          hipStream_t stream, float* mean = nullptr, float* mean2 = nullptr);
 int launch_layernorm_mod_fp8_2(const float* x, const float* scale, const float* shift, int mod_bstride, int rows_per_batch, uint8_t* out,
                                float* out_scale, int rows, const float* x2, const float* scale2, const float* shift2, int rows_per_batch2, uint8_t* out2,
                                float* out_scale2, int rows2, int D, float eps, hipStream_t stream, int kind = 1, const float* smooth = nullptr,
                                const float* smooth2 = nullptr);
 int launch_layernorm_mod(const float* x, const float* scale, const float* shift, int mod_bstride,
-                         int rows_per_batch, bf16_t* out, int rows, int D, float eps, hipStream_t stream);
+                         int rows_per_batch, bf16_t* out, int rows, int D, float eps, hipStream_t stream, float* mean = nullptr);
+int launch_ln_fold_operand(const float* mod, int64_t nmod, int R, const int64_t* offs_dev, int nlin, int D, bf16_t* out, hipStream_t stream);
 int launch_quantize_rows_fp8(const bf16_t* x, int ld, int rows, int K, uint8_t* out, float* scale, hipStream_t stream, int kind = 1, const float* vec = nullptr);
 int launch_quantize_rows_i8_asym(const bf16_t* x, int ld, int rows, int K, int d0, uint8_t* out, float* scale, float* offset, hipStream_t stream, const float* vec = nullptr);
 int launch_rowsum_i8(const int8_t* wq, const float* w_scale, int N, int K, int d0, float* w_sum, hipStream_t stream);
diff --git a/diffusion-rs_amd/csrc/flux_model.hip b/diffusion-rs_amd/csrc/flux_model.hip
--- a/diffusion-rs_amd/csrc/flux_model.hip
+++ b/diffusion-rs_amd/csrc/flux_model.hip
@@ -101,6 +101,7 @@
     uint8_t* a8 = nullptr;
     float* a8s = nullptr;
     float* a8o = nullptr;
+    float *ln_m0[2] = {nullptr, nullptr}, *ln_part[2] = {nullptr, nullptr};
     int Lpad = 0;
   } ws;
   bool profiling = false;
@@ -136,6 +137,8 @@
   static constexpr int SP_SPLITS = 4;
   bool split_k = false;
   DeviceBuffer splitk_scratch;
+  DeviceBuffer ln_c, ln_ops, ln_offs;
+  size_t ln_rows = 0;
   bool fp8 = false;
   int q8_kind = 0;
   unsigned q8_mask = 0;
@@ -462,6 +465,10 @@
   add((void**)&w.attn_txt, (size_t)B * T * D * 2);
   add((void**)&w.hid, (size_t)B * L * M * 2);
   add((void**)&w.vec_bf, (size_t)B * D * 2);
+  for (int k = 0; k < 2; ++k) {
+    add((void**)&w.ln_m0[k], (size_t)B * L * 4);
+    add((void**)&w.ln_part[k], (size_t)std::max(1, D / 256) * B * L * 8);
+  }
   if (m->fp8) {
     add((void**)&w.a8, (size_t)B * L * (D + M));
     add((void**)&w.a8s, (size_t)B * L * 4);
@@ -893,6 +900,63 @@
   *reuse = sc->valid && (f == 1 || (f < 0 && sc->o->threshold > 0.f && below));
   if (sc->o->decisions_out) sc->o->decisions_out[i] = *reuse ? 1 : 0;
   if (*reuse) FMI_TRY(launch_step_cache_apply(w.x_img, n, m->sc_delta.as<float>(), w.x + (size_t)T * m->D, L * m->D, B, n, s));
+  return FMI_OK;
+}
+
+static int64_t ln_dbl_cols(const fmi_flux* m) { return 6 * (int64_t)m->D + 2 * (int64_t)m->M; }
+static int64_t ln_dbl_col(const fmi_flux* m, int i, int mlp, int st) { return i * ln_dbl_cols(m) + (mlp ? 6 * (int64_t)m->D + st * (int64_t)m->M : st * 3 * (int64_t)m->D); }
+static int64_t ln_sgl_col(const fmi_flux* m, int i) { return m->cfg.num_layers * ln_dbl_cols(m) + i * (3 * (int64_t)m->D + m->M); }
+static int64_t ln_cols(const fmi_flux* m) { return ln_sgl_col(m, m->cfg.num_single_layers); }
+static bool ln_fold_enabled(const fmi_flux* m) {
+  if (m->fp8 || m->calib || m->split_k || m->is_cn || m->D < 256 || m->D % 256 || m->M % 4 || !gemm_ln_fold_available(m->D)) return false;
+  for (const auto& b : m->dbl)
+    for (int st = 0; st < 2; ++st)
+      if (b.qkv[st].q_type || b.proj[st].q_type || b.mlp1[st].q_type || b.mlp2[st].q_type) return false;
+  for (const auto& b : m->sgl)
+    if (b.w1.q_type || b.w2.q_type) return false;
+  return true;
+}
+static int ln_fold_precompute(fmi_flux* m, const float* mod, int R, hipStream_t s) {
+  const int D = m->D, nl = m->cfg.num_layers, ns = m->cfg.num_single_layers, nlin = 4 * nl + ns;
+  const int64_t cols = ln_cols(m);
+  if (nlin == 0 || R <= 0) return FMI_OK;
+  if (!m->ln_offs) {
+    std::vector<int64_t> offs;
+    for (int i = 0; i < nl; ++i)
+      for (int mlp = 0; mlp < 2; ++mlp)
+        for (int st = 0; st < 2; ++st) offs.push_back(m->dbl[i].mod_off[st] + (mlp ? 3 * D : 0)), offs.push_back(m->dbl[i].mod_off[st] + (mlp ? 4 * D : D));
+    for (int i = 0; i < ns; ++i) offs.push_back(m->sgl[i].mod_off), offs.push_back(m->sgl[i].mod_off + D);
+    FMI_HIP_TRY(m->ln_offs.alloc(offs.size() * 8));
+    FMI_HIP_TRY(hipMemcpy(m->ln_offs.ptr, offs.data(), offs.size() * 8, hipMemcpyHostToDevice));
+  }
+  if (m->ln_rows < (size_t)R) {
+    FMI_HIP_TRY(hipStreamSynchronize(s));
+    m->ln_c.reset(), m->ln_ops.reset(), m->ln_rows = 0;
+    if (m->ln_c.alloc((size_t)2 * R * cols * 4) != hipSuccess || m->ln_ops.alloc((size_t)nlin * 2 * R * D * 2) != hipSuccess) {
+      m->ln_c.reset(), m->ln_ops.reset();
+      return fail(FMI_ERR_NOMEM, "flux: hipMalloc of the folded LayerNorms' column vectors (" + std::to_string((size_t)2 * R * cols * 4) + " bytes) failed");
+    }
+    m->ln_rows = R;
+  }
+  PhaseTimer pt(m, s, PH_MOD);
+  bf16_t* ops = m->ln_ops.as<bf16_t>();
+  FMI_TRY(launch_ln_fold_operand(mod, m->n_mod, R, m->ln_offs.as<int64_t>(), nlin, D, ops, s));
+  float* c1 = m->ln_c.as<float>();
+  float* c2 = c1 + m->ln_rows * cols;
+  GemmProblem p[8];
+  int np = 0;
+  for (int l = 0; l < nlin; ++l) {
+    const int i = l < 4 * nl ? l / 4 : l - 4 * nl, mlp = (l / 2) & 1, st = l & 1;
+    const Dense& d = l < 4 * nl ? (mlp ? m->dbl[i].mlp1[st] : m->dbl[i].qkv[st]) : m->sgl[i].w1;
+    const int64_t col = l < 4 * nl ? ln_dbl_col(m, i, mlp, st) : ln_sgl_col(m, i);
+    p[np] = make_problem(d, ops + (size_t)(2 * l) * R * D, D, R, c1 + col, (int)cols, EPI_STORE_F32);
+    p[np++].bias = nullptr;
+    p[np++] = make_problem(d, ops + (size_t)(2 * l + 1) * R * D, D, R, c2 + col, (int)cols, EPI_STORE_F32);
+    if (np == 8 || l == nlin - 1) {
+      FMI_TRY(launch_gemm(p, np, s));
+      np = 0;
+    }
+  }
   return FMI_OK;
 }
 
@@ -970,6 +1034,66 @@
   }
   const float* const mod = mod_pre ? mod_pre : w.mod;
 
+  const bool fold = ln_fold_enabled(m);
+  const int NT = D / 256, BL = B * L;
+  const int64_t lcols = fold ? ln_cols(m) : 0;
+  const float *lc1 = nullptr, *lc2 = nullptr;
+  if (fold) {
+    size_t r0 = 0;
+    if (mod_pre) r0 = (size_t)((mod_pre - m->mod_steps.as<float>()) / nmod);
+    else FMI_TRY(ln_fold_precompute(m, w.mod, B, s));
+    if (r0 + B > m->ln_rows) return fail(FMI_ERR_STATE, "flux: the folded LayerNorms' column vectors were not computed for this step");
+    lc1 = m->ln_c.as<float>() + r0 * lcols, lc2 = lc1 + m->ln_rows * lcols;
+  }
+  int ln_cur = 0, ln_tiles = 0;
+  bool ln_have = false;
+  const auto ln_consume = [&](GemmProblem& q, int cur, int row0, int64_t col) {
+    q.ln_stats = w.ln_part[cur] + 2 * (size_t)row0, q.ln_tiles = NT, q.ln_ld = BL;
+    q.ln_c1 = lc1 + col, q.ln_c2 = lc2 + col, q.bias = nullptr;
+  };
+  const auto ln_produce = [&](GemmProblem& q, int cur, int tiles, int row0, bf16_t* a, const float* next_scale) {
+    q.ln_a = a, q.ln_lda = D, q.ln_scale = next_scale, q.ln_ld = BL;
+    q.ln_m0_prev = w.ln_m0[cur] + row0, q.ln_part_prev = w.ln_part[cur] + 2 * (size_t)row0, q.ln_prev_tiles = tiles;
+    q.ln_m0 = w.ln_m0[cur ^ 1] + row0, q.ln_part = w.ln_part[cur ^ 1] + 2 * (size_t)row0;
+  };
+  const auto ln_gemm = [&](GemmProblem* q, Dense* const* dn, int n, const int* rpb, hipStream_t st) -> int {
+    if (B == 1 || !q[0].ln_stats) return gemm2(m, q, dn, n, st);
+    GemmProblem e[8];
+    int ne = 0;
+    for (int i = 0; i < n; ++i)
+      for (int b = 0; b < B; ++b) {
+        GemmProblem x = q[i];
+        const size_t r = rpb[i];
+        x.M = rpb[i], x.A += b * r * x.lda, x.out = reinterpret_cast<bf16_t*>(x.out) + b * r * x.ldo;
+        x.ln_stats += 2 * b * r, x.ln_c1 += b * lcols, x.ln_c2 += b * lcols;
+        if (x.qk_qh) {
+          const size_t hl = (size_t)b * x.qk_H * x.qk_Ltot * 128 * (x.qk_q8 > 0.f ? 1 : 2);
+          x.qk_qh = reinterpret_cast<bf16_t*>(reinterpret_cast<char*>(x.qk_qh) + hl), x.qk_kh = reinterpret_cast<bf16_t*>(reinterpret_cast<char*>(x.qk_kh) + hl);
+          x.qk_vt += (size_t)b * x.qk_H * 128 * x.qk_Lpad, x.qk_pe += b * x.qk_pe_bstride;
+        }
+        e[ne++] = x;
+        if (ne == 8) {
+          FMI_TRY(launch_gemm(e, ne, st));
+          ne = 0;
+        }
+      }
+    return ne ? launch_gemm(e, ne, st) : FMI_OK;
+  };
+  const int rpb_st[2] = {S, T};
+  const bool ln_join = fold && B > 1 && c.num_single_layers > 0;
+  const auto ln_join_problems = [&](const GemmProblem& q, int st, int cur, int tiles, GemmProblem* e, int& ne) {
+    for (int b = 0; b < B; ++b) {
+      GemmProblem x = q;
+      const size_t r = st ? T : S, row_in = (st ? 0 : BT) + b * r, row_out = (size_t)b * L + (st ? 0 : T);
+      x.M = (int)r, x.A += b * r * x.lda, x.out = reinterpret_cast<float*>(x.out) + b * r * x.ldo;
+      x.gate += (size_t)b * x.gate_bstride, x.rows_per_batch = 0;
+      x.ln_a = w.xm + row_out * D, x.ln_lda = D, x.ln_scale = mod + m->sgl[0].mod_off + D + (size_t)b * nmod, x.ln_ld = BL;
+      x.ln_m0_prev = w.ln_m0[cur] + row_in, x.ln_part_prev = w.ln_part[cur] + 2 * row_in, x.ln_prev_tiles = tiles;
+      x.ln_m0 = w.ln_m0[cur ^ 1] + row_out, x.ln_part = w.ln_part[cur ^ 1] + 2 * row_out;
+      e[ne++] = x;
+    }
+  };
+
   bool reuse = false;
   for (int i = 0; i < c.num_layers; ++i) {
     if (sc && i == 1) {
@@ -983,13 +1107,20 @@
     bf16_t* xm_img = w.xm + (size_t)B * T * D;
     bool fused_img = false, fused_txt = false, qk8 = false;
     const bool q_qkv = fp8 && bw.qkv[0].w8, q_out = fp8 && bw.proj[0].w8, q_m1 = fp8 && bw.mlp1[0].w8, q_m2 = fp8 && bw.mlp2[0].w8;
-    {
+    const bool f1 = fold && ln_have;
+    const float* nxt[2] = {nullptr, nullptr};
+    if (fold && i + 1 < c.num_layers) nxt[0] = mod + m->dbl[i + 1].mod_off[0] + D, nxt[1] = mod + m->dbl[i + 1].mod_off[1] + D;
+    else if (fold && B == 1 && c.num_single_layers > 0) nxt[0] = nxt[1] = mod + m->sgl[0].mod_off + D;
+    const bool join = ln_join && i + 1 == c.num_layers;
+    if (!f1) {
       PhaseTimer pt(m, s, PH_LN);
       if (q_qkv) {
         FMI_TRY(launch_layernorm_mod_fp8_2(w.x_img, mi + D, mi, nmod, S, w.a8 + (size_t)BT * D, w.a8s + BT, B * S, w.x_txt, mt + D, mt, T, w.a8, w.a8s,
                                            B * T, D, 1e-6f, s, qk, bw.qkv[0].sm_inv, bw.qkv[1].sm_inv));
       } else {
-        FMI_TRY(launch_layernorm_mod2(w.x_img, mi + D, mi, nmod, S, xm_img, B * S, w.x_txt, mt + D, mt, T, xm_txt, B * T, D, 1e-6f, s));
+        FMI_TRY(launch_layernorm_mod2(w.x_img, mi + D, mi, nmod, S, xm_img, B * S, w.x_txt, mt + D, mt, T, xm_txt, B * T, D, 1e-6f, s,
+                                      fold ? w.ln_m0[ln_cur ^ 1] + BT : nullptr, fold ? w.ln_m0[ln_cur ^ 1] : nullptr));
+        if (fold) ln_cur ^= 1, ln_tiles = 0;
         FMI_TRY(calib_rec(m, bw.qkv[0], xm_img, D, B * S, s));
         FMI_TRY(calib_rec(m, bw.qkv[1], xm_txt, D, B * T, s));
       }
@@ -1005,8 +1136,9 @@
       const float q8 = qk8 ? m->q8_dbl[i] : 0.f, k8 = qk8 ? m->k8_dbl[i] : 0.f;
       fused_img = !ipj && with_qkv_relayout(m, p[0], bw.nq[0], bw.nk[0], pe_bs, S, T, L, q8, k8);
       fused_txt = with_qkv_relayout(m, p[1], bw.nq[1], bw.nk[1], pe_bs, T, 0, L, q8, k8);
+      if (f1) ln_consume(p[0], ln_cur, BT, ln_dbl_col(m, i, 0, 0)), ln_consume(p[1], ln_cur, 0, ln_dbl_col(m, i, 0, 1));
       Dense* dn[2] = {&bw.qkv[0], &bw.qkv[1]};
-      FMI_TRY(gemm2(m, p, dn, 2, s));
+      FMI_TRY(ln_gemm(p, dn, 2, rpb_st, s));
     }
     if (!(fused_img && fused_txt)) {
       PhaseTimer pt(m, s, PH_RELAYOUT);
@@ -1041,20 +1173,36 @@
         float* x = st ? w.x_txt : w.x_img;
         bf16_t* xm_ = st ? xm_txt : xm_img;
         bf16_t* hid_ = st ? hid_txt : hid_img;
+        const int row0 = st ? 0 : BT;
         GemmProblem p = make_problem(bw.proj[st], st ? w.attn_txt : w.attn_img, D, rows, x, D, EPI_RESID_GATE_F32);
         with_gate(p, mo + 2 * D, rpb, nmod);
+        if (fold) ln_produce(p, ln_cur, ln_tiles, row0, xm_, mo + 4 * D);
         FMI_TRY(gemm1(m, p, bw.proj[st], q));
-        FMI_TRY(launch_layernorm_mod(x, mo + 4 * D, mo + 3 * D, nmod, rpb, xm_, rows, D, 1e-6f, q));
+        if (!fold) FMI_TRY(launch_layernorm_mod(x, mo + 4 * D, mo + 3 * D, nmod, rpb, xm_, rows, D, 1e-6f, q));
         p = make_problem(bw.mlp1[st], xm_, D, rows, hid_, Mh, EPI_GELU_BF16);
-        FMI_TRY(gemm1(m, p, bw.mlp1[st], q));
+        if (fold) ln_consume(p, ln_cur ^ 1, row0, ln_dbl_col(m, i, 1, st));
+        Dense* dn1[1] = {&bw.mlp1[st]};
+        FMI_TRY(ln_gemm(&p, dn1, 1, &rpb_st[st], q));
         p = make_problem(bw.mlp2[st], hid_, Mh, rows, x, D, EPI_RESID_GATE_F32);
         with_gate(p, mo + 5 * D, rpb, nmod);
-        FMI_TRY(gemm1(m, p, bw.mlp2[st], q));
+        if (nxt[st]) ln_produce(p, ln_cur ^ 1, NT, row0, xm_, nxt[st]);
+        if (join) {
+          GemmProblem e[8];
+          int ne = 0;
+          ln_join_problems(p, st, ln_cur ^ 1, NT, e, ne);
+          FMI_TRY(launch_gemm(e, ne, q));
+        } else {
+          FMI_TRY(gemm1(m, p, bw.mlp2[st], q));
+        }
       }
       FMI_HIP_TRY(hipEventRecord(m->ev_join, m->side));
       FMI_HIP_TRY(hipStreamWaitEvent(s, m->ev_join, 0));
       FMI_TRY(ip_hook(i));
       FMI_TRY(cn_hook(false, i, w.x_img, (int64_t)S * D));
+      if (fold) {
+        ln_tiles = NT, ln_have = (nxt[0] != nullptr || join) && !ipj && !inj;
+        if (!nxt[0] && !join) ln_cur ^= 1;
+      }
       continue;
     }
     {
@@ -1073,10 +1221,14 @@
       p[1] = q_out ? make_problem_fp8(m, bw.proj[1], 0, B * T, w.x_txt, D, EPI_RESID_GATE_F32)
                    : make_problem(bw.proj[1], w.attn_txt, D, B * T, w.x_txt, D, EPI_RESID_GATE_F32);
       with_gate(p[1], mt + 2 * D, T, nmod);
+      if (fold) {
+        ln_produce(p[0], ln_cur, ln_tiles, BT, xm_img, mi + 4 * D), ln_produce(p[1], ln_cur, ln_tiles, 0, xm_txt, mt + 4 * D);
+        ln_cur ^= 1, ln_tiles = NT;
+      }
       Dense* dn[2] = {&bw.proj[0], &bw.proj[1]};
       FMI_TRY(gemm2(m, p, dn, 2, s));
     }
-    {
+    if (!fold) {
       PhaseTimer pt(m, s, PH_LN);
       if (q_m1) {
         FMI_TRY(launch_layernorm_mod_fp8_2(w.x_img, mi + 4 * D, mi + 3 * D, nmod, S, w.a8 + (size_t)BT * D, w.a8s + BT, B * S, w.x_txt, mt + 4 * D,
@@ -1095,8 +1247,9 @@
       GemmProblem p[2];
       p[0] = q_m1 ? make_problem_fp8(m, bw.mlp1[0], BT, B * S, hid_img, Mh, EPI_GELU_BF16) : make_problem(bw.mlp1[0], xm_img, D, B * S, hid_img, Mh, EPI_GELU_BF16);
       p[1] = q_m1 ? make_problem_fp8(m, bw.mlp1[1], 0, B * T, hid_txt, Mh, EPI_GELU_BF16) : make_problem(bw.mlp1[1], xm_txt, D, B * T, hid_txt, Mh, EPI_GELU_BF16);
+      if (fold) ln_consume(p[0], ln_cur, BT, ln_dbl_col(m, i, 1, 0)), ln_consume(p[1], ln_cur, 0, ln_dbl_col(m, i, 1, 1));
       Dense* dn1[2] = {&bw.mlp1[0], &bw.mlp1[1]};
-      FMI_TRY(gemm2(m, p, dn1, 2, s));
+      FMI_TRY(ln_gemm(p, dn1, 2, rpb_st, s));
       if (q_m2) {
         if (bw.mlp2[0].sm_inv || bw.mlp2[1].sm_inv) {
           FMI_TRY(quantize_act(m, bw.mlp2[1], hid_txt, Mh, B * T, 0, s));
@@ -1114,11 +1267,27 @@
       p[1] = q_m2 ? make_problem_fp8(m, bw.mlp2[1], 0, B * T, w.x_txt, D, EPI_RESID_GATE_F32)
                   : make_problem(bw.mlp2[1], hid_txt, Mh, B * T, w.x_txt, D, EPI_RESID_GATE_F32);
       with_gate(p[1], mt + 5 * D, T, nmod);
+      ln_have = false;
+      if (nxt[0]) {
+        ln_produce(p[0], ln_cur, ln_tiles, BT, xm_img, nxt[0]), ln_produce(p[1], ln_cur, ln_tiles, 0, xm_txt, nxt[1]);
+        ln_cur ^= 1, ln_tiles = NT, ln_have = true;
+      }
       Dense* dn2[2] = {&bw.mlp2[0], &bw.mlp2[1]};
-      FMI_TRY(gemm2(m, p, dn2, 2, s));
+      if (join) {
+        GemmProblem e[8];
+        for (int st = 0; st < 2; ++st) {
+          int ne = 0;
+          ln_join_problems(p[st], st, ln_cur, ln_tiles, e, ne);
+          FMI_TRY(launch_gemm(e, ne, s));
+        }
+        ln_cur ^= 1, ln_tiles = NT, ln_have = true;
+      } else {
+        FMI_TRY(gemm2(m, p, dn2, 2, s));
+      }
     }
     FMI_TRY(ip_hook(i));
     FMI_TRY(cn_hook(false, i, w.x_img, (int64_t)S * D));
+    if (ipj || inj) ln_have = false;
   }
 
   if (sc && c.num_layers == 1) FMI_TRY(step_cache_decide(m, sc, B, S, T, s, &reuse));
@@ -1133,12 +1302,14 @@
     bool fused = false;
     const bool q_w1 = fp8 && bw.w1.w8, q_w2 = fp8 && bw.w2.w8;
     const bool qk8 = ((q_w1 && m->fp8_attn) || (qk8_any && !bw.w1.q_type)) && can_fuse_relayout(m, B * L, L, 0);
-    {
+    const bool f1 = fold && ln_have;
+    if (!f1) {
       PhaseTimer pt(m, s, PH_LN);
       if (q_w1) {
         FMI_TRY(launch_layernorm_mod_fp8(w.x, mo + D, mo, nmod, L, w.a8, w.a8s, B * L, D, 1e-6f, s, qk, bw.w1.sm_inv));
       } else {
-        FMI_TRY(launch_layernorm_mod(w.x, mo + D, mo, nmod, L, w.xm, B * L, D, 1e-6f, s));
+        FMI_TRY(launch_layernorm_mod(w.x, mo + D, mo, nmod, L, w.xm, B * L, D, 1e-6f, s, fold ? w.ln_m0[ln_cur ^ 1] : nullptr));
+        if (fold) ln_cur ^= 1, ln_tiles = 0;
         FMI_TRY(calib_rec(m, bw.w1, w.xm, D, B * L, s));
       }
     }
@@ -1148,7 +1319,9 @@
                            : make_problem(bw.w1, w.xm, D, B * L, w.big, ldbig, EPI_GELU_FROM_COL);
       p.gelu_from = 3 * D;
       fused = with_qkv_relayout(m, p, bw.nq, bw.nk, pe_bs, L, 0, L, qk8 ? m->q8_sgl[i] : 0.f, qk8 ? m->k8_sgl[i] : 0.f);
-      FMI_TRY(gemm1(m, p, bw.w1, s));
+      if (f1) ln_consume(p, ln_cur, 0, ln_sgl_col(m, i));
+      Dense* dn1[1] = {&bw.w1};
+      FMI_TRY(ln_gemm(&p, dn1, 1, &L, s));
     }
     if (!fused) {
       PhaseTimer pt(m, s, PH_RELAYOUT);
@@ -1171,9 +1344,15 @@
       GemmProblem p = q_w2 ? make_problem_fp8(m, bw.w2, 0, B * L, w.x, D, EPI_RESID_GATE_F32)
                            : make_problem(bw.w2, w.big + 2 * D, ldbig, B * L, w.x, D, EPI_RESID_GATE_F32);
       with_gate(p, mo + 2 * D, L, nmod);
+      ln_have = false;
+      if (fold && i + 1 < c.num_single_layers) {
+        ln_produce(p, ln_cur, ln_tiles, 0, w.xm, mod + m->sgl[i + 1].mod_off + D);
+        ln_cur ^= 1, ln_tiles = NT, ln_have = true;
+      }
       FMI_TRY(gemm1(m, p, bw.w2, s));
     }
     FMI_TRY(cn_hook(true, i, w.x + (size_t)T * D, (int64_t)L * D));
+    if (inj) ln_have = false;
   }
   if (m->is_cn) return FMI_OK;
   if (sc) {
@@ -1733,6 +1912,7 @@
       }
     }
     *mod_steps = m->mod_steps.as<float>();
+    if (ln_fold_enabled(m)) FMI_TRY(ln_fold_precompute(m, m->mod_steps.as<float>(), (int)R, s));
   }
   *txt_pre = nullptr;
   if (n_steps > 1) {
diff --git a/diffusion-rs_amd/csrc/gemm_bf16.hip b/diffusion-rs_amd/csrc/gemm_bf16.hip
--- a/diffusion-rs_amd/csrc/gemm_bf16.hip
+++ b/diffusion-rs_amd/csrc/gemm_bf16.hip
@@ -296,7 +296,27 @@
   qkv_relayout_emit(P, smem, m0, n0, wave, lane);
 }
 
-template <int NJ, int WN, int ACT, class ACC>
+constexpr int LN_LDS_OFF = 8 * 16384;
+__device__ __forceinline__ float* ln_m0_lds(char* smem) { return reinterpret_cast<float*>(smem + LN_LDS_OFF); }
+__device__ __forceinline__ float2* ln_wavepart_lds(char* smem) { return reinterpret_cast<float2*>(smem + LN_LDS_OFF + 1024); }
+__device__ __forceinline__ void ln_centres(const GemmProblem& P, char* smem, int m0, int n0, int tid, int nthr) {
+  for (int t = tid; t < BM; t += nthr) {
+    const int mr = min(m0 + t, P.M - 1);
+    float c = P.ln_m0_prev[mr], sd = 0.f;
+    for (int k = 0; k < P.ln_prev_tiles; ++k) sd += P.ln_part_prev[((int64_t)k * P.ln_ld + mr) * 2];
+    if (P.ln_prev_tiles > 0) c += sd / (float)P.N;
+    ln_m0_lds(smem)[t] = c;
+    if (n0 == 0 && m0 + t < P.M) P.ln_m0[mr] = c;
+  }
+}
+__device__ __forceinline__ void ln_store_partials(const GemmProblem& P, char* smem, int m0, int n0, int tid, int nthr) {
+  const float2* wp = ln_wavepart_lds(smem);
+  for (int t = tid; t < BM && m0 + t < P.M; t += nthr) {
+    const float2 p0 = wp[t], p1 = wp[256 + t], p2 = wp[512 + t], p3 = wp[768 + t];
+    reinterpret_cast<float2*>(P.ln_part)[(int64_t)(n0 / 256) * P.ln_ld + m0 + t] = make_float2((p0.x + p1.x) + (p2.x + p3.x), (p0.y + p1.y) + (p2.y + p3.y));
+  }
+}
+template <int NJ, int WN, int ACT, int LN = 0, class ACC>
 __device__ __forceinline__ void gemm_epilogue_impl(const GemmProblem& P, const ACC& acc, char* smem, int m0, int n0, int wave, int lane) {
   constexpr int BN = WN * 32 * NJ;
   const int wm = wave / WN, wn = wave % WN;
@@ -404,6 +424,14 @@
       constexpr int NS16 = 8 * NJ;
       constexpr int LPR = RBF / 16, RPI = 64 / LPR;
       float* of = reinterpret_cast<float*>(P.out);
+      static_assert(LN == 0 || NJ == 2, "the next-operand arrays sit behind eight 16 KiB staging regions");
+      constexpr bool ln = LN != 0;
+      if constexpr (LN == 1) {
+        ln_centres(P, smem, m0, n0, wave * 64 + lane, GEMM_THREADS);
+        __syncthreads();
+      }
+      const float* ln_m0s = ln_m0_lds(smem);
+      float2* ln_wp = ln_wavepart_lds(smem);
       auto f32_pass = [&](auto pass_tag) {
         constexpr int pass = decltype(pass_tag)::value;
         asm volatile("s_waitcnt lgkmcnt(0)" ::: "memory");
@@ -419,27 +447,43 @@
           constexpr int GRP = NIT < 8 ? NIT : 8;
 #pragma unroll
           for (int g0 = 0; g0 < NIT; g0 += GRP) {
-            float4 xr[GRP], gg[GRP];
+            float4 xr[GRP], gg[GRP], sc0;
+            int bo[GRP];
 #pragma unroll
             for (int u = 0; u < GRP; ++u) {
               const int r = (g0 + u) * RPI + lane / LPR;
               const int m = min(m0 + wm * 128 + pass * 64 + r, P.M - 1);
-              const float* gate = P.gate + (P.rows_per_batch > 0 ? (int64_t)(m / P.rows_per_batch) * P.gate_bstride : 0);
-              gg[u] = *reinterpret_cast<const float4*>(gate + n);
+              const int64_t boff = P.rows_per_batch > 0 ? (int64_t)(m / P.rows_per_batch) * P.gate_bstride : 0;
+              gg[u] = *reinterpret_cast<const float4*>(P.gate + boff + n);
               xr[u] = *reinterpret_cast<const float4*>(of + (int64_t)m * P.ldo + n);
+              if constexpr (ln) {
+                bo[u] = (int)boff;
+                if (u == 0) sc0 = *reinterpret_cast<const float4*>(P.ln_scale + boff + n);
+              }
             }
 #pragma unroll
             for (int u = 0; u < GRP; ++u) {
               const int r = (g0 + u) * RPI + lane / LPR;
               const int m = m0 + wm * 128 + pass * 64 + r;
               const float4 v = *reinterpret_cast<const float4*>(cw + r * RBF + ((ch ^ (r & (NS16 - 1))) << 4));
-              if (m < P.M) {
-                float4 x = xr[u];
-                x.x += gg[u].x * v.x;
-                x.y += gg[u].y * v.y;
-                x.z += gg[u].z * v.z;
-                x.w += gg[u].w * v.w;
-                *reinterpret_cast<float4*>(of + (int64_t)m * P.ldo + n) = x;
+              float4 x = xr[u];
+              x.x += gg[u].x * v.x;
+              x.y += gg[u].y * v.y;
+              x.z += gg[u].z * v.z;
+              x.w += gg[u].w * v.w;
+              if (m < P.M) *reinterpret_cast<float4*>(of + (int64_t)m * P.ldo + n) = x;
+              if constexpr (ln) {
+                const int rt = wm * 128 + pass * 64 + r;
+                const float c = ln_m0s[rt];
+                const float d0 = x.x - c, d1 = x.y - c, d2 = x.z - c, d3 = x.w - c;
+                float4 sc = sc0;
+                if (bo[u] != bo[0]) sc = *reinterpret_cast<const float4*>(P.ln_scale + bo[u] + n);
+                if (m < P.M)
+                  *reinterpret_cast<uint2*>(P.ln_a + (int64_t)m * P.ln_lda + n) =
+                      make_uint2(pack_bf16x2(d0 * (sc.x + 1.0f), d1 * (sc.y + 1.0f)), pack_bf16x2(d2 * (sc.z + 1.0f), d3 * (sc.w + 1.0f)));
+                const float sd = row16_sum((d0 + d1) + (d2 + d3));
+                const float sd2 = row16_sum((d0 * d0 + d1 * d1) + (d2 * d2 + d3 * d3));
+                if (lane % LPR == 0) ln_wp[wn * 256 + rt] = make_float2(sd, sd2);
               }
             }
           }
@@ -455,6 +499,10 @@
       };
       f32_pass(std::integral_constant<int, 0>{});
       f32_pass(std::integral_constant<int, 1>{});
+      if constexpr (LN == 1) {
+        __syncthreads();
+        ln_store_partials(P, smem, m0, n0, wave * 64 + lane, GEMM_THREADS);
+      }
     }
     return;
   }
@@ -483,7 +531,7 @@
   });
 }
 
-template <int NJ, int WN = 4, int ACT = -1, class ACC>
+template <int NJ, int WN = 4, int ACT = -1, int LN = 0, class ACC>
 __device__ __forceinline__ void gemm_epilogue(const GemmProblem& P, const ACC& acc, char* smem, int m0, int n0, int wave, int lane) {
   if constexpr (NJ == 2 && WN == 4) {
     if (P.qk_qh != nullptr && n0 < 3 * P.qk_D) {
@@ -491,13 +539,16 @@
       return;
     }
   }
-  gemm_epilogue_impl<NJ, WN, ACT>(P, acc, smem, m0, n0, wave, lane);
+  gemm_epilogue_impl<NJ, WN, ACT, LN>(P, acc, smem, m0, n0, wave, lane);
 }
 inline int epilogue_kind(const GemmProblem* p, int n) {
-  auto kind = [](int epi) { return (epi == EPI_STORE_BF16 || epi == EPI_RESID_GATE_F32) ? 0 : epi == EPI_GELU_BF16 ? 1 : epi == EPI_GELU_FROM_COL ? 2 : 3; };
-  const int k = kind(p[0].epi);
+  auto kind = [](const GemmProblem& q) {
+    if (q.epi == EPI_RESID_GATE_F32 && q.ln_a) return 4;
+    return (q.epi == EPI_STORE_BF16 || q.epi == EPI_RESID_GATE_F32) ? 0 : q.epi == EPI_GELU_BF16 ? 1 : q.epi == EPI_GELU_FROM_COL ? 2 : 3;
+  };
+  const int k = kind(p[0]);
   for (int i = 1; i < n; ++i)
-    if (kind(p[i].epi) != k) return -1;
+    if (kind(p[i]) != k) return -1;
   return k;
 }
 
@@ -856,13 +907,57 @@
   }
   int lane_e = lane;
   asm volatile("" : "+v"(lane_e));
+  if constexpr (!FP8 && ACT < 3) {
+    if (P.ln_stats) {
+      float2* rowst = reinterpret_cast<float2*>(smem + LN_LDS_OFF);
+      const int tid_e = wave * 64 + lane_e;
+      const int l15 = lane_e & 15, l4 = lane_e >> 4;
+      float4 c1v[2 * NJ], c2v[2 * NJ];
+#pragma unroll
+      for (int j = 0; j < 2 * NJ; ++j) {
+        const int n = min(n0 + wn * 64 + j * 16 + 4 * l4, P.N - 4);
+        c1v[j] = *reinterpret_cast<const float4*>(P.ln_c1 + n);
+        c2v[j] = *reinterpret_cast<const float4*>(P.ln_c2 + n);
+      }
+      float2 st = make_float2(0.f, 0.f);
+      if (tid_e < BM) {
+        const int mr = min(m0 + tid_e, P.M - 1);
+        const float2* part = reinterpret_cast<const float2*>(P.ln_stats) + mr;
+        float sd = 0.f, sd2 = 0.f;
+#pragma unroll 4
+        for (int t = 0; t < P.ln_tiles; ++t) {
+          const float2 v = part[(int64_t)t * P.ln_ld];
+          sd += v.x, sd2 += v.y;
+        }
+        const float dm = sd / (float)P.K;
+        const float var = sd2 / (float)P.K - dm * dm;
+        const float r = 1.0f / sqrtf(var + 1e-6f);
+        st = make_float2(r, r * dm);
+      }
+      __syncthreads();
+      if (tid_e < BM) rowst[tid_e] = st;
+      __syncthreads();
+#pragma unroll
+      for (int i = 0; i < 8; ++i) {
+        const float2 s = rowst[g * 128 + i * 16 + l15];
+#pragma unroll
+        for (int j = 0; j < 2 * NJ; ++j) {
+          acc16[i][j][0] = __builtin_fmaf(s.x, acc16[i][j][0], __builtin_fmaf(-s.y, c1v[j].x, c2v[j].x));
+          acc16[i][j][1] = __builtin_fmaf(s.x, acc16[i][j][1], __builtin_fmaf(-s.y, c1v[j].y, c2v[j].y));
+          acc16[i][j][2] = __builtin_fmaf(s.x, acc16[i][j][2], __builtin_fmaf(-s.y, c1v[j].z, c2v[j].z));
+          acc16[i][j][3] = __builtin_fmaf(s.x, acc16[i][j][3], __builtin_fmaf(-s.y, c1v[j].w, c2v[j].w));
+        }
+      }
+      asm volatile("" : "+v"(lane_e));
+    }
+  }
   if constexpr (FP8) gemm_epilogue<NJ, 4, ACT>(P, Acc32<NJ>{acc, lane_e}, smem, m0, n0, wave, lane_e);
-  else gemm_epilogue<NJ, 4, ACT>(P, Acc16<NJ>{acc16, lane_e}, smem, m0, n0, wave, lane_e);
+  else gemm_epilogue<NJ, 4, ACT, ACT == 4 ? 1 : 0>(P, Acc16<NJ>{acc16, lane_e}, smem, m0, n0, wave, lane_e);
 }
 
 
 constexpr int W4_THREADS = 256;
-template <int ACT, class V, int I, int J>
+template <int ACT, bool LN = false, class V, int I, int J>
 __device__ __forceinline__ void w4_epilogue(const GemmProblem& P, V (&acc)[I][J], char* smem, int m0, int n0, int wave, int wm, int wn, int lane) {
   using View = std::conditional_t<std::is_same<V, f32x16>::value, Acc32<2>, Acc16<2>>;
   constexpr int H = J / 2;
@@ -894,6 +989,10 @@
     }
     return;
   }
+  if constexpr (LN) {
+    __syncthreads();
+    ln_centres(P, smem, m0, n0, wave * 64 + lane_e, W4_THREADS);
+  }
   V hacc[I][H];
 #pragma unroll
   for (int i = 0; i < I; ++i)
@@ -901,12 +1000,16 @@
     for (int j = 0; j < H; ++j) hacc[i][j] = acc[i][j];
 #pragma clang loop unroll(disable)
   for (int r = 0; r < 2; ++r) {
-    gemm_epilogue_impl<2, 4, ACT>(P, View{hacc, lane_e}, smem, m0, n0, wm * 4 + wn * 2 + r, lane_e);
+    gemm_epilogue_impl<2, 4, ACT, LN ? 2 : 0>(P, View{hacc, lane_e}, smem, m0, n0, wm * 4 + wn * 2 + r, lane_e);
 #pragma unroll
     for (int i = 0; i < I; ++i)
 #pragma unroll
       for (int j = 0; j < H; ++j) hacc[i][j] = acc[i][H + j];
     asm volatile("" : "+v"(lane_e));
+  }
+  if constexpr (LN) {
+    __syncthreads();
+    ln_store_partials(P, smem, m0, n0, wave * 64 + lane_e, W4_THREADS);
   }
 }
 
@@ -1040,7 +1143,7 @@
     for (int j = 0; j < 8; ++j) asm volatile("" : "+a"(acc[i][j]));
 #undef FMI_W4_RD
 #undef FMI_W4_WAIT
-  w4_epilogue<ACT>(P, acc, smem, m0, n0, wave, wm, wn, lane);
+  w4_epilogue<ACT, ACT == 4>(P, acc, smem, m0, n0, wave, wm, wn, lane);
 }
 
 #endif
@@ -1060,6 +1163,7 @@
 void set_gemm_w4q_min_rows(int rows) { g_w4q_min_rows = rows; }
 void set_gemm_w4(bool on) { g_w4 = on; }
 void set_gemm_pingpong(bool on) { g_pingpong = on; }
+bool gemm_ln_fold_available(int K) { return g_pingpong && !(g_w4 && (K >= 8192 || g_w4_qkv_min_n < (1 << 30))); }
 
 static int pick_tile_band(int tiles_m) {
   static const int pinned = [] {
@@ -1139,6 +1243,24 @@
     }
   }
   if (epilogue_kind(probs, nprob) < 0) return fail(FMI_ERR_INVALID, "launch_gemm: the problems of a grouped launch must share the activation kind");
+  for (int i = 0; i < nprob; ++i) {
+    const GemmProblem& p = probs[i];
+    if (!p.ln_a && !p.ln_stats) continue;
+    auto al = [](const void* q, uintptr_t a) { return (reinterpret_cast<uintptr_t>(q) & (a - 1)) == 0; };
+    if (quant || conv || fp8 || bn != 256 || p.ln_ld < p.M) return fail(FMI_ERR_INVALID, "launch_gemm: the LayerNorm fold needs a dense bf16 problem wider than 128 and a stats slab of at least M rows");
+    if (p.ln_a) {
+      if (p.epi != EPI_RESID_GATE_F32 || p.N % 256 || p.ldo % 8 || !al(p.out, 16) || (p.bias && !al(p.bias, 8)))
+        return fail(FMI_ERR_INVALID, "launch_gemm: the next-operand output belongs to the gated residual epilogue with N % 256 == 0, ldo % 8 == 0 and a 16-byte aligned out");
+      if (!p.ln_scale || !p.ln_m0_prev || !p.ln_m0 || !p.ln_part || p.ln_prev_tiles < 0 || (p.ln_prev_tiles > 0 && !p.ln_part_prev) || !al(p.ln_scale, 16) || !al(p.ln_part, 8) ||
+          !al(p.ln_part_prev, 8) || !al(p.ln_a, 8) || p.ln_lda % 4 || p.ln_lda < p.N)
+        return fail(FMI_ERR_INVALID, "launch_gemm: bad next-operand descriptor (scale, both m0, part; scale 16-byte, a 8-byte aligned; ln_lda % 4 == 0 and >= N)");
+    }
+    if (p.ln_stats) {
+      if (epilogue_kind(&p, 1) >= 3 || p.bias || !p.ln_c1 || !p.ln_c2 || p.ln_tiles <= 0 || p.N % 4 || !al(p.ln_stats, 8) || !al(p.ln_c1, 16) ||
+          !al(p.ln_c2, 16))
+        return fail(FMI_ERR_INVALID, "launch_gemm: bad row-affine descriptor (store / GELU / GELU-from-column kinds, no bias, c1 and c2 16-byte aligned, N % 4 == 0)");
+    }
+  }
   return FMI_OK;
 }
 
@@ -1187,6 +1309,7 @@
     case 0: return launch(std::integral_constant<int, 0>{});
     case 1: return launch(std::integral_constant<int, 1>{});
     case 2: return launch(std::integral_constant<int, 2>{});
+    case 4: return launch(std::integral_constant<int, 4>{});
     default: return launch(std::integral_constant<int, 3>{});
   }
 }
@@ -1201,6 +1324,9 @@
                      gemm_w4_pays(probs, nprob, sw.w4_qkv_min_n), gemm_w4q_ok(probs, nprob, sw.w4q_min_rows)};
   const GemmChoice c = select_gemm_kernel(t, sw, FMI_ALT_KERNELS != 0);
   if (c.err != FMI_OK) return fail(c.err, c.msg);
+  for (int i = 0; i < nprob; ++i)
+    if ((probs[i].ln_stats && c.kernel != GK_PP) || (probs[i].ln_a && c.kernel != GK_PP && c.kernel != GK_W4))
+      return fail(FMI_ERR_UNSUPPORTED, "launch_gemm: the LayerNorm fold's epilogues live in the ping-pong kernel (the next-operand output also in the dense 4-wave kernel)");
   GemmBatch b;
   b.nprob = nprob;
   int total = 0;
@@ -1215,17 +1341,18 @@
   const bool wide = bn == 256;
   return with_act(epilogue_kind(probs, nprob), [&](auto act) -> int {
     constexpr int ACT = decltype(act)::value;
+    constexpr int ACTQ = ACT == 4 ? 0 : ACT;
     auto launch = [&](auto kernel, int threads) { hipLaunchKernelGGL(kernel, dim3(total), dim3(threads), 0, stream, b); };
     switch (c.kernel) {
       case GK_DB128: launch(gemm_bf16_kernel<0, 1>, GEMM_THREADS); break;
       case GK_Q4_DB: wide ? launch(gemm_bf16_kernel<1, 2>, GEMM_THREADS) : launch(gemm_bf16_kernel<1, 1>, GEMM_THREADS); break;
       case GK_CONV: wide ? launch(gemm_bf16_kernel<2, 2>, GEMM_THREADS) : launch(gemm_bf16_kernel<2, 1>, GEMM_THREADS); break;
       case GK_PP: launch(gemm_pp_kernel<0, ACT>, GEMM_THREADS); break;
-      case GK_PP_E4M3: launch(gemm_pp_kernel<1, ACT>, GEMM_THREADS); break;
-      case GK_PP_I8: launch(gemm_pp_kernel<2, ACT>, GEMM_THREADS); break;
+      case GK_PP_E4M3: launch(gemm_pp_kernel<1, ACTQ>, GEMM_THREADS); break;
+      case GK_PP_I8: launch(gemm_pp_kernel<2, ACTQ>, GEMM_THREADS); break;
       case GK_W4Q:
-        FMI_LDS_GUARD((gemm_w4q_kernel<ACT>), W4Q_LUT_BYTES + 4 * A_TILE_BYTES);
-        launch(gemm_w4q_kernel<ACT>, W4_THREADS);
+        FMI_LDS_GUARD((gemm_w4q_kernel<ACTQ>), W4Q_LUT_BYTES + 4 * A_TILE_BYTES);
+        launch(gemm_w4q_kernel<ACTQ>, W4_THREADS);
         break;
 #if FMI_ALT_KERNELS
       case GK_DB256: launch(gemm_bf16_kernel<0, 2>, GEMM_THREADS); break;
diff --git a/diffusion-rs_amd/csrc/norm_rope.hip b/diffusion-rs_amd/csrc/norm_rope.hip
--- a/diffusion-rs_amd/csrc/norm_rope.hip
+++ b/diffusion-rs_amd/csrc/norm_rope.hip
@@ -7,7 +7,7 @@
                                                             const float* __restrict shift1, int mod_bstride, int rows_per_batch1,
                                                             bf16_t* __restrict out1, int D, float eps, int rows1, const float* __restrict x2,
                                                             const float* __restrict scale2, const float* __restrict shift2, int rows_per_batch2,
-                                                            bf16_t* __restrict out2) {
+                                                            bf16_t* __restrict out2, float* __restrict mean1, float* __restrict mean2) {
   __shared__ float red[2][4];
   const bool second = (int)blockIdx.x >= rows1;
   const int row = second ? blockIdx.x - rows1 : blockIdx.x;
@@ -55,6 +55,7 @@
   s = (red[0][0] + red[0][1]) + (red[0][2] + red[0][3]);
   s2 = (red[1][0] + red[1][1]) + (red[1][2] + red[1][3]);
   const float mean = s / (float)D;
+  if (float* mo = second ? mean2 : mean1; mo && threadIdx.x == 0) mo[row] = mean;
   const float var = s2 / (float)D - mean * mean;
   const float inv_std = 1.0f / sqrtf(var + eps);
   uint2* o = reinterpret_cast<uint2*>(out + (int64_t)row * D);
@@ -90,21 +91,38 @@
 
 int launch_layernorm_mod2(const float* x, const float* scale, const float* shift, int mod_bstride, int rows_per_batch, bf16_t* out, int rows,
                           const float* x2, const float* scale2, const float* shift2, int rows_per_batch2, bf16_t* out2, int rows2, int D, float eps,
-                          hipStream_t stream) {
+                          hipStream_t stream, float* mean, float* mean2) {
   if (rows + rows2 <= 0) return FMI_OK;
   if (D % 4) return fail(FMI_ERR_INVALID, "layernorm_mod: D must be a multiple of 4");
   if (D <= 4096)
     hipLaunchKernelGGL(layernorm_mod_kernel<true>, dim3(rows + rows2), dim3(256), 0, stream, x, scale, shift, mod_bstride, rows_per_batch, out, D, eps, rows,
-                       x2, scale2, shift2, rows_per_batch2, out2);
+                       x2, scale2, shift2, rows_per_batch2, out2, mean, mean2);
   else
     hipLaunchKernelGGL(layernorm_mod_kernel<false>, dim3(rows + rows2), dim3(256), 0, stream, x, scale, shift, mod_bstride, rows_per_batch, out, D, eps, rows,
-                       x2, scale2, shift2, rows_per_batch2, out2);
+                       x2, scale2, shift2, rows_per_batch2, out2, mean, mean2);
   FMI_LAUNCH_CHECK();
   return FMI_OK;
 }
 int launch_layernorm_mod(const float* x, const float* scale, const float* shift, int mod_bstride, int rows_per_batch, bf16_t* out,
-                         int rows, int D, float eps, hipStream_t stream) {
-  return launch_layernorm_mod2(x, scale, shift, mod_bstride, rows_per_batch, out, rows, nullptr, nullptr, nullptr, 0, nullptr, 0, D, eps, stream);
+                         int rows, int D, float eps, hipStream_t stream, float* mean) {
+  return launch_layernorm_mod2(x, scale, shift, mod_bstride, rows_per_batch, out, rows, nullptr, nullptr, nullptr, 0, nullptr, 0, D, eps, stream, mean, nullptr);
+}
+
+__global__ __launch_bounds__(256) void ln_fold_operand_kernel(const float* __restrict mod, int64_t nmod, int R, const int64_t* __restrict offs, int D, bf16_t* __restrict out) {
+  const int l = blockIdx.z, r = blockIdx.y, k = (blockIdx.x * 256 + threadIdx.x) * 4;
+  if (k >= D) return;
+  const float* row = mod + (int64_t)r * nmod;
+  const float4 sh = *reinterpret_cast<const float4*>(row + offs[2 * l] + k), sc = *reinterpret_cast<const float4*>(row + offs[2 * l + 1] + k);
+  bf16_t* o1 = out + ((int64_t)(2 * l) * R + r) * D + k;
+  *reinterpret_cast<uint2*>(o1) = make_uint2(pack_bf16x2(sc.x + 1.0f, sc.y + 1.0f), pack_bf16x2(sc.z + 1.0f, sc.w + 1.0f));
+  *reinterpret_cast<uint2*>(o1 + (int64_t)R * D) = make_uint2(pack_bf16x2(sh.x, sh.y), pack_bf16x2(sh.z, sh.w));
+}
+int launch_ln_fold_operand(const float* mod, int64_t nmod, int R, const int64_t* offs_dev, int nlin, int D, bf16_t* out, hipStream_t stream) {
+  if (R <= 0 || nlin <= 0) return FMI_OK;
+  if (D % 4 || nmod % 4) return fail(FMI_ERR_INVALID, "ln_fold_operand: D and the modulation row length must be multiples of 4");
+  hipLaunchKernelGGL(ln_fold_operand_kernel, dim3(cdiv(D, 1024), R, nlin), dim3(256), 0, stream, mod, nmod, R, offs_dev, D, out);
+  FMI_LAUNCH_CHECK();
+  return FMI_OK;
 }
 
 template <bool F32OUT>
diff --git a/include/flux_mi355x.h b/include/flux_mi355x.h
--- a/include/flux_mi355x.h
+++ b/include/flux_mi355x.h
@@ -382,6 +382,23 @@
   const float* w_sum;
 } fmi_gemm_desc;
 int fmi_gemm_group(const fmi_gemm_desc* probs, int nprob, void* stream);
+typedef struct fmi_gemm_ln_desc {
+  const float* scale;
+  const float* m0_prev;
+  const float* part_prev;
+  float* m0;
+  float* part;
+  void* a;
+  const float* stats;
+  const float* c1;
+  const float* c2;
+  int prev_tiles, lda, ld, tiles;
+  void *qh, *kh, *vt;
+  const void *wq, *wk;
+  const float* pe;
+  int qk_H, qk_rows, qk_row_off, qk_Ltot, qk_Lpad;
+} fmi_gemm_ln_desc;
+int fmi_gemm_ln(const fmi_gemm_desc* prob, const fmi_gemm_ln_desc* ln, void* stream);
 int fmi_splitk_resid_gate(const float* parts, int S, const void* bias, const float* gate, int rows_per_batch, int gate_bstride, float* out, int ldo,
                           int M, int N, void* stream);
 int fmi_set_gemm_kernel(int pingpong, int w4);
```

Result: no change. 0.3209 images/s (-0.9%).
